# endernewton/tf-faster-rcnn

Hardware: AMD Instinct MI355X
Metric: images/sec (600×1000) ResNet-101 Faster R-CNN at 1/2/4/8 MI355X (higher is better)
Workload: dtype f32 (operands, accumulators, results; GEMMs with Cin, Cout % 128 == 0 form each f32 product from two-piece fp16 operands with an exact power-of-two scale per 128-k block on the fp16 matrix pipe -- 3 MFMAs / product, dropped terms <= 3 * 2^-22, measured error vs float64 below the f32-MFMA kernel's; o

## Files before the change

### include/frcnn_hip.h

```cpp
#ifndef FRCNN_HIP_H_
#define FRCNN_HIP_H_
#include <stddef.h>
#include <stdint.h>

#ifdef __cplusplus
extern "C" {
#endif

#define FRCNN_OK 0
#define FRCNN_E_ARG (-1)
#define FRCNN_E_WS (-2)
#define FRCNN_E_UNSUPPORTED (-3)
#define FRCNN_E_HIP(e) (-(1000 + (int)(e)))

#define FRCNN_NMS_RULE_CPU 0
#define FRCNN_NMS_RULE_GPU 1

#define FRCNN_ACT_NONE 0
#define FRCNN_ACT_RELU 1
#define FRCNN_ACT_RELU6 2

#define FRCNN_ABI_VERSION 6
int frcnn_abi_version(void);
const char* frcnn_build_info(void);
// ... 61 lines not shown
                      int* out_count_d, int max_out, void* ws, size_t ws_bytes, void* stream);
size_t frcnn_detect_post_batched_workspace_bytes(int B, int R, int C);
int frcnn_detect_post_batched(const float* cls_prob_d, const float* bbox_pred_d, const float* rois_d, const int* num_rois_d,
                              int B, int R, int C, double im_scale, int im_h, int im_w, double nms_thresh, int rule,
                              float score_thresh, int max_per_image, float* out_dets_d, int* out_count_d, int max_out,
                              long long out_stride, void* ws, size_t ws_bytes, void* stream);

int frcnn_im_detect_boxes(const float* rois_d, const float* bbox_pred_d, int R, int C, double im_scale,
                          int im_h, int im_w, float* boxes_d, void* stream);

int frcnn_bbox_transform_inv(const float* boxes_d, const float* deltas_d, int N, int k, float* out_d, void* stream);
int frcnn_clip_boxes(float* boxes_d, int N, int k, float im_h, float im_w, void* stream);
int frcnn_bbox_transform(const float* ex_rois_d, const float* gt_rois_d, int N, float* targets_d, void* stream);

int frcnn_bbox_overlaps(const double* boxes_d, int n, const double* query_d, int k, double* out_d, void* stream);

size_t frcnn_coco_match_workspace_bytes(int n_groups, long long n_det, long long n_gt, long long n_pairs);
int frcnn_coco_match(const double* det_xywh_d, const long long* det_off_d, const double* gt_xywh_d, const double* gt_area_d,
                     const unsigned char* gt_crowd_d, const long long* gt_off_d, int n_groups, const double* iou_thrs_d, int T,
                     const double* area_rng_d, int A, unsigned char* det_matched_d, unsigned char* det_ignored_d,
                     unsigned char* gt_ignored_d, double* iou_out_d, void* ws, size_t ws_bytes, void* stream);

int frcnn_conv2d_nhwc(const float* x_d, int N, int H, int W, int Cin, const float* w_d, const float* bias_d,
                      const float* residual_d, int RH, int RW, int res_stride, float* y_d, int OH, int OW,
                      int Cout, int KH, int KW, int stride, int pad_top, int pad_left, int act, int fold_w,
                      void* stream);
size_t frcnn_conv2d_workspace_bytes(int N, int OH, int OW, int Cout, int KH, int KW, int Cin, int fold_w);
int frcnn_conv2d_nhwc_ws(const float* x_d, int N, int H, int W, int Cin, const float* w_d, const float* bias_d,
                         const float* residual_d, int RH, int RW, int res_stride, float* y_d, int OH, int OW, int Cout, int KH,
                         int KW, int stride, int pad_top, int pad_left, int act, int fold_w, void* ws, size_t ws_bytes,
                         void* stream);

int frcnn_set_tuning(int key, int value);
unsigned int frcnn_crc32c(const void* data, size_t n, unsigned int crc);

long long frcnn_snappy_uncompress(const unsigned char* src, size_t n, unsigned char* dst, size_t cap);

int frcnn_prep_image_shape(int h, int w, int target_size, int max_size, double* im_scale, int* out_h, int* out_w);
int frcnn_prep_image(const void* src_d, int src_is_float, int h, int w, const double* pixel_means, double im_scale, float* out_d,
                     int OH, int OW, int out_c, void* stream);
int frcnn_prep_image_batched(const void* src_d, int src_is_float, int B, int h, int w, const double* pixel_means, double im_scale,
                             float* out_d, int OH, int OW, int out_c, void* stream);
int frcnn_prep_train_image(const void* src_d, int src_is_float, int h, int w, int flipped, const double* pixel_means, double im_scale,
                           float* out_d, int OH, int OW, int out_c, const unsigned short* boxes_d, const int* classes_d, int G,
                           float* gt_d, void* stream);

int frcnn_jpeg_info(const unsigned char* data, size_t n, int* out8);
size_t frcnn_jpeg_coef_bytes(int width, int height, int ncomp, int hs, int vs);
int frcnn_jpeg_entropy_decode(const unsigned char* data, size_t n, void* coef_h, size_t coef_bytes);
int frcnn_jpeg_pixels_host(const void* coef_h, int width, int height, int ncomp, int hs, int vs, unsigned char* bgr_h);
size_t frcnn_jpeg_workspace_bytes(int width, int height, int ncomp, int hs, int vs);
int frcnn_jpeg_pixels(const void* coef_d, int width, int height, int ncomp, int hs, int vs, unsigned char* bgr_d, void* ws,
                      size_t ws_bytes, void* stream);

int frcnn_gemm_batched_nt(const float* x_d, const float* w_d, float* y_d, int G, int M, int N, int K, void* stream);
size_t frcnn_gemm_x3_pack_bytes(int G, int N, int K);
int frcnn_gemm_x3_pack(const float* w_d, int G, int N, int K, void* planes_d, void* stream);
int frcnn_gemm_x3(const float* x_d, const void* planes_d, const float* bias_d, const float* res_d, float* y_d, int G, int M, int N,
                  int K, int act, int cfg, int terms, void* stream);
size_t frcnn_h2_planes_bytes(long long rows, int K);
int frcnn_h2_pack_w(const float* w_d, int G, int N, int K, void* planes_d, float* w_inv_d, void* stream);
int frcnn_h2_split(const float* x_d, long long M, int K, void* planes_d, float* inv_d, void* stream);
int frcnn_gemm_h2(const void* x_planes_d, const float* x_inv_d, const void* w_planes_d, const float* w_inv_d, const float* bias_d,
                  const float* res_d, const void* res_planes_d, const float* res_inv_d, float* y_d, void* y_planes_d, float* y_inv_d,
                  int G, int M, int N, int K, int act, int cfg, void* stream);
size_t frcnn_gemm_h2_mean_workspace_bytes(int G, int M, int N);
int frcnn_gemm_h2_mean(const void* x_planes_d, const float* x_inv_d, const void* w_planes_d, const float* w_inv_d, const float* bias_d,
                       const float* res_d, const void* res_planes_d, const float* res_inv_d, int G, int M, int N, int K, int act, int rows,
                       float* mean_out_d, void* ws, size_t ws_bytes, int cfg, void* stream);
int frcnn_winograd_filter_transform(const float* w_hwio, int Cin, int Cout, const float* scale, int m, float* u_out);
int frcnn_winograd_filter_transform_device(const float* w_packed_d, int Cout, int Cin, int m, int transpose_flip, float* u_d,
                                           void* stream);
int frcnn_winograd_input_transform(const float* x_d, int N, int H, int W, int C, int m, float* v_d, void* stream);
int frcnn_winograd_output_transform(const float* m_d, int N, int H, int W, int C, int m, const float* bias_d, int act, float* y_d,
                                    void* stream);
int frcnn_winograd7_filter_transform(const float* w_hwio, int Cin, int Cout, const float* scale, float* u_out);
int frcnn_winograd7_filter_transform_device(const float* w_packed_d, int Cout, int Cin, int transpose_flip, float* u_d, void* stream);
int frcnn_winograd7_input_transform(const float* x_d, int R, int C, float* v_d, void* stream);
int frcnn_winograd7_output_transform(const float* m_d, int R, int C, const float* bias_d, int act, float* y_d, void* stream);
int frcnn_winograd_input_transform_h2(const float* x_d, int N, int H, int W, int C, int m, void* v_planes_d, float* v_inv_d, void* stream);
int frcnn_winograd_output_transform_h2(const float* m_d, int N, int H, int W, int C, int m, const float* bias_d, int act, float* y_d,
                                       void* y_planes_d, float* y_inv_d, void* stream);
int frcnn_winograd7_input_transform_h2(const float* x_d, int R, int C, void* v_planes_d, float* v_inv_d, void* stream);
int frcnn_winograd7_output_transform_h2(const float* m_d, int R, int C, const float* bias_d, int act, float* y_d, void* y_planes_d,
                                        float* y_inv_d, void* stream);
int frcnn_pack_filter_hwio(const float* w_hwio, int KH, int KW, int Cin, int Cout, const float* scale, float* out);
int frcnn_maxpool_nhwc(const float* x_d, int N, int H, int W, int C, int k, int stride, int pad_top,
                       int pad_left, float* y_d, int OH, int OW, void* stream);
int frcnn_dwconv3x3_nhwc(const float* x_d, int N, int H, int W, int C, const float* w_d, const float* bias_d,
                         float* y_d, int OH, int OW, int stride, int pad_top, int pad_left, int act, void* stream);
int frcnn_dwconv3x3_nhwc_h2(const float* x_d, int N, int H, int W, int C, const float* w_d, const float* bias_d, float* y_d,
                            void* y_planes_d, float* y_inv_d, int OH, int OW, int stride, int pad_top, int pad_left, int act, void* stream);
int frcnn_spatial_mean(const float* x_d, int N, int HW, int C, float* y_d, void* stream);
int frcnn_softmax_rows(const float* x_d, int R, int C, int ld, float* y_d, void* stream);
int frcnn_rpn_softmax(const float* score_d, int HW, int A, int ld, float* prob_d, void* stream);
int frcnn_copy_cols(const float* src_d, int R, int ld_src, int col0, int cols, float* dst_d, int ld_dst, void* stream);

size_t frcnn_anchor_target_workspace_bytes(int H, int W, int A, int max_gt);
int frcnn_anchor_target_layer(const float* gt_boxes_d, int G, float im_h, float im_w, int H, int W, int A,
                              int feat_stride, const double* base_d, int rpn_batchsize, double fg_fraction,
                              double pos_overlap, double neg_overlap, long long seed, const double* opts, float* labels_d,
                              float* bbox_targets_d, float* inside_w_d, float* outside_w_d, void* ws,
                              size_t ws_bytes, void* stream);
int frcnn_anchor_target_layer_inject(const float* gt_boxes_d, int G, float im_h, float im_w, int H, int W, int A, int feat_stride,
                                     const double* base_d, int rpn_batchsize, double fg_fraction, double pos_overlap,
                                     double neg_overlap, const int* disable_d, int n_disable, const double* opts, float* labels_d,
                                     float* bbox_targets_d, float* inside_w_d, float* outside_w_d, void* ws, size_t ws_bytes,
                                     void* stream);
int frcnn_proposal_target_layer(const float* rpn_rois_d, const float* rpn_scores_d, int N, const float* gt_boxes_d,
                                int G, int num_classes, int batch_size, double fg_fraction, double fg_thresh,
                                double bg_thresh_hi, double bg_thresh_lo, const double* means4, const double* stds4,
                                long long seed, const double* opts, float* rois_d, float* roi_scores_d, float* labels_d,
                                float* bbox_targets_d, float* inside_w_d, float* outside_w_d, int* counts_d,
                                void* stream);
int frcnn_proposal_target_layer_dn(const float* rpn_rois_d, const float* rpn_scores_d, int max_rois, const int* num_rois_d,
                                   const float* gt_boxes_d, int G, int num_classes, int batch_size, double fg_fraction,
                                   double fg_thresh, double bg_thresh_hi, double bg_thresh_lo, const double* means4,
                                   const double* stds4, long long seed, const double* opts, float* rois_d, float* roi_scores_d,
                                   float* labels_d, float* bbox_targets_d, float* inside_w_d, float* outside_w_d, int* counts_d,
                                   void* stream);
int frcnn_proposal_target_layer_inject(const float* rpn_rois_d, const float* rpn_scores_d, int N, const float* gt_boxes_d, int G,
                                       int num_classes, int batch_size, const int* keep_inds_d, int n_fg, const double* means4,
                                       const double* stds4, const double* opts, float* rois_d, float* roi_scores_d, float* labels_d,
                                       float* bbox_targets_d, float* inside_w_d, float* outside_w_d, void* stream);
size_t frcnn_loss_workspace_bytes(long long elements);
int frcnn_softmax_ce_loss(const float* logits_d, const float* labels_d, int R, int C, int rpn_A, int rpn_H, int rpn_W,
                          float* loss_d, float* dlogits_d, void* ws, size_t ws_bytes, void* stream);
int frcnn_smooth_l1_loss(const float* pred_d, const float* targets_d, const float* inside_w_d, const float* outside_w_d,
                         long long n, float sigma, float mean_divisor, float* loss_d, float* dpred_d, void* ws,
                         size_t ws_bytes, void* stream);

int frcnn_transpose_pad(const float* in_d, int M, int C, float* out_d, int Mp, void* stream);
int frcnn_im2col_t(const float* x_d, int N, int H, int W, int Cin, int OH, int OW, int KH, int KW, int stride,
                   int pad_top, int pad_left, float* out_d, int Mp, void* stream);
int frcnn_flip_transpose_filter(const float* w_d, int Cout, int KH, int KW, int Cin, float* out_d, void* stream);
int frcnn_conv2d_dgrad_strided(const float* dy_d, int N, int OH, int OW, int Cout, const float* w_d, int KH, int KW,
                               int Cin, int stride, int pad_top, int pad_left, float* dx_d, int H, int W,
                               int accumulate, void* stream);
int frcnn_conv2d_wgrad_supported(int Cin, int Cout);
size_t frcnn_conv2d_wgrad_workspace_bytes(int N, int OH, int OW, int Cin, int Cout, int KH, int KW);
int frcnn_conv2d_wgrad(const float* dy_d, const float* x_d, int N, int H, int W, int Cin, int OH, int OW, int Cout, int KH, int KW,
                       int stride, int pad_top, int pad_left, float* dw_d, void* ws, size_t ws_bytes, void* stream);
void frcnn_conv2d_wgrad_set_plan(int tile, int min_workgroups);
size_t frcnn_conv2d_wgrad_h2_workspace_bytes(int N, int OH, int OW, int Cin, int Cout, int KH, int KW);
int frcnn_conv2d_wgrad_h2(const float* dy_d, const float* x_d, int N, int H, int W, int Cin, int OH, int OW, int Cout, int KH, int KW,
                          int stride, int pad_top, int pad_left, float* dw_d, void* ws, size_t ws_bytes, void* stream);
void frcnn_conv2d_wgrad_h2_set_plan(int tile, int min_workgroups);
int frcnn_relu_bwd(float* grad_d, const float* y_d, long long n, void* stream);
int frcnn_conv2d_nhwc_masked_ws(const float* x_d, int N, int H, int W, int Cin, const float* w_d, const float* bias_d,
                                const float* residual_d, int RH, int RW, int res_stride, float* y_d, int OH, int OW,
                                int Cout, int KH, int KW, int stride, int pad_top, int pad_left, int act, const float* mask_d,
                                void* ws, size_t ws_bytes, void* stream);
int frcnn_gemm_h2_masked(const void* x_planes_d, const float* x_inv_d, const void* w_planes_d, const float* w_inv_d, const float* bias_d,
                         const float* res_d, const float* mask_d, float* y_d, void* y_planes_d, float* y_inv_d, int G, int M, int N, int K,
                         int act, int cfg, void* stream);
int frcnn_winograd_output_transform_masked(const float* m_d, int N, int H, int W, int C, int m, const float* mask_d, float* y_d,
                                           void* y_planes_d, float* y_inv_d, void* stream);
int frcnn_winograd7_output_transform_masked(const float* m_d, int R, int C, const float* mask_d, float* y_d, void* y_planes_d,
                                            float* y_inv_d, void* stream);
int frcnn_relu6_bwd(float* grad_d, const float* y_d, long long n, void* stream);
int frcnn_maxpool_bwd(const float* x_d, int N, int H, int W, int C, int k, int stride, const float* y_d, const float* dy_d,
                      int OH, int OW, float* dx_d, void* stream);
int frcnn_dropout(const float* x_d, long long n, unsigned long long seed, float keep_prob, float* y_d, void* stream);
int frcnn_dwconv3x3_dgrad(const float* g_d, int N, int OH, int OW, int C, const float* w_d, float* dx_d, int H, int W, int stride,
                          int pad_top, int pad_left, int accumulate, void* stream);
size_t frcnn_dwconv3x3_wgrad_workspace_bytes(int N, int OH, int OW, int C);
// ... 30 lines not shown
```

### scratch/wino_bench.py

```python
import os, sys
ROOT = os.path.dirname(os.path.dirname(os.path.abspath(__file__)))
sys.path[:0] = [os.path.join(ROOT, "tf-faster-rcnn_amd")]
import numpy as np, torch
import frcnn_hip
from frcnn_hip import ops
dev = torch.device("cuda:0")
ths = [int(a) for a in (sys.argv[1] if (len(sys.argv) > 1 and "=" not in sys.argv[1]) else "256,100000000").split(",")]
shapes = {
    "block3 conv2 x8": (8, 38, 63, 256, 4),
    "block3 conv2 x1": (1, 38, 63, 256, 4),
    "rpn 3x3 x8": (8, 38, 63, 1024, 4),
    "block2 conv2 x8 (F2)": (8, 75, 125, 128, 2),
    "tail conv2 7x7 x8": (2400, 7, 7, 512, 7),
}
single = [a for a in sys.argv[1:] if a.startswith("single=")]
if single:
    nm, which, n = single[0][7:].split(":")
    N, H, W, C, m = shapes[nm]
    x = torch.randn(N, H, W, C, device=dev).clamp(min=0)
    G, T = ops.winograd_points(m), ops.winograd_tiles(N, H, W, m)
    mm = torch.randn(G, T, C, device=dev)
    bias = torch.randn(C, device=dev)
    v, yp = ops.H2.empty(G * T, C, dev), ops.H2.empty(N * H * W, C, dev)
    for _ in range(int(n)):
        if which == "input":
            ops.winograd_input_transform_h2(x, v, m)
        else:
            ops.winograd_output_transform_h2(mm, bias, 1, (N, H, W, C), m, yp)
    torch.cuda.synchronize()
    print("algorithmic bytes per launch: %d" % (4 * (N * H * W * C + G * T * C)))
    sys.exit(0)
print("%-24s %-10s %-6s %9s %9s %8s  %s" % ("shape", "transform", "rows<", "med_us", "min_us", "GB/s", "bits vs first"))
for name, (N, H, W, C, m) in shapes.items():
    torch.manual_seed(1)
    x = torch.randn(N, H, W, C, device=dev).clamp(min=0)
    G, T = ops.winograd_points(m), ops.winograd_tiles(N, H, W, m)
    mm = torch.randn(G, T, C, device=dev)
    bias = torch.randn(C, device=dev)
    for which in ("input", "output"):
        ref = None
        for th in ths:
            frcnn_hip.lib().frcnn_set_tuning(9, th)
            v = ops.H2.empty(G * T, C, dev)
            yp = ops.H2.empty(N * H * W, C, dev)
            v.planes.zero_(); v.inv.zero_(); yp.planes.zero_(); yp.inv.zero_()

            def run():
                if which == "input":
                    ops.winograd_input_transform_h2(x, v, m)
                else:
                    ops.winograd_output_transform_h2(mm, bias, 1, (N, H, W, C), m, yp)
            run(); torch.cuda.synchronize()
            o = v if which == "input" else yp
            pv = o.planes.view(torch.int16).to(torch.int64).view(-1)
            dig = (int(pv.sum()), int((pv * (torch.arange(pv.numel(), device=dev) % 8191 + 1)).sum()), int(o.inv.view(torch.int32).to(torch.int64).sum()))
            del pv
            ref = dig if ref is None else ref
            ts = []
            for r in range(6):
                e0, e1 = torch.cuda.Event(enable_timing=True), torch.cuda.Event(enable_timing=True)
                e0.record()
                for _ in range(10): run()
                e1.record(); torch.cuda.synchronize()
                if r: ts.append(e0.elapsed_time(e1) * 100)
            nbytes = 4.0 * (N * H * W * C + G * T * C)
            print("%-24s %-10s %-6s %9.1f %9.1f %8.0f  %s" % (name, which, th if th < 10**8 else "all", float(np.median(ts)), min(ts), nbytes / np.median(ts) / 1e3,
                                                             "identical" if dig == ref else "DIFFERENT"), flush=True)
            if m != 4:
                break
frcnn_hip.lib().frcnn_set_tuning(9, 0)
```

### tf-faster-rcnn_amd/csrc/conv_igemm.hip

```cpp
#include "common.h"
#include "mfma_f32.h"
#include <mutex>
#include <type_traits>

__device__ float4 g_zero_page[4];

struct ConvParams {
  const float* x; const float* w; const float* bias; const float* res; float* y;
  const float* mask;
  int N, H, W, Cin, OH, OW, Cout, KH, KW, stride, pad_top, pad_left, act;
  int RH, RW, res_stride;
  int M, Ktot, nsteps;
  int mtiles, ntiles;
  int batch;
  long long gx, gw, gy;
  int reserved;
  int splits, kchunk;
  long long gz;
  int stagger, stagger_slots;
};

__device__ __forceinline__ size_t res_offset_strided(int m, int n, int Cout, int res_stride, int ohow, int OW, int RH, int RW) {
  const int img = m / ohow, rem = m % ohow, oh = rem / OW, ow = rem % OW;
  return ((size_t)(img * RH + oh * res_stride) * RW + ow * res_stride) * Cout + n;
// ... 448 lines not shown
    int next = tile;
    if (last) {
      next = __builtin_amdgcn_readfirstlane(tile + W8);
      set_tile(next < t_end ? next : tile);
      prefetch_res();
    }
    slab_body(cur);
    cur ^= 1;
    if (!last) { ++step; continue; }
    if (p.res) finish(std::true_type{}); else finish(std::false_type{});
    if (next >= t_end) break;
    zero_acc();
    step = 0; tile = next; c_bm0 = i_bm0; c_bn0 = i_bn0; c_g = i_g;
  }
  wait_vmcnt<0>();
}

template <int BM, int BN, int WM, int WN, bool ILV, bool RF, bool RESPF>
static int launch_stream(const ConvParams& c, hipStream_t st) {
  constexpr int NT = (BM / WM) * (BN / WN) * 64;
  constexpr size_t lds = sizeof(float) * 2 * (BM + BN) * 32;
  auto kern = k_gemm_stream<BM, BN, WM, WN, ILV, RF, RESPF>;
  static KernelOnce once;
  int slots = 0;
  HIP_TRY(kernel_once(once, (const void*)kern, NT, lds, &slots));
  const bool plain = c.KH == 1 && c.KW == 1 && c.stride == 1 && c.pad_top == 0 && c.pad_left == 0 && c.OH == c.H && c.OW == c.W;
  if (slots < 8 || !plain || c.mask || c.Cout % BN || c.splits != 1 || (c.res && c.res_stride != 1) || (long long)c.M * c.Cout >= (1ll << 31) ||
      (long long)c.M * c.Cin >= (1ll << 31) || (long long)c.Cout * c.Cin >= (1ll << 31))
    return FRCNN_E_UNSUPPORTED;
  GemmParams p;
  p.x = c.x; p.w = c.w; p.bias = c.bias; p.res = c.res; p.y = c.y;
  p.mtiles = cdiv(c.M, BM); p.M = c.M; p.N = c.Cout; p.K = c.Cin; p.nsteps = c.Cin / 32;
  p.ntiles = c.Cout / BN; p.batch = c.batch; p.act = c.act;
  p.gx = c.gx; p.gw = c.gw; p.gy = c.gy;
  const long long T = (long long)p.mtiles * p.ntiles * p.batch;
  if (T >= (1ll << 30)) return FRCNN_E_UNSUPPORTED;
  const int grid = (int)min((long long)(slots / 8) * 8, ((T + 7) / 8) * 8);
  hipLaunchKernelGGL(kern, dim3(grid), dim3(NT), lds, st, p);
  LAUNCH_CHECK();
  return FRCNN_OK;
}

enum : int {
  IGEMM_64x32_NS4 = 4,
  IGEMM_64x64_ILV = 15,
  IGEMM_128_RF = 20,
  IGEMM_128_8W_RF = 21,
  STREAM_64x64 = 100, STREAM_64x64_RESPF = 101,
  STREAM_128_RF = 102,
  STREAM_128_8W_RF = 104, STREAM_128_8W_RF_RESPF = 105,
  STREAM_128x64 = 106, STREAM_128x64_RESPF = 107,
  STREAM_64x128 = 108, STREAM_64x128_RESPF = 109,
  STREAM_128x64_4W_RESPF = 110, STREAM_64x128_4W_RESPF = 111,
  STREAM_32x64 = 112,
  STREAM_32x128 = 114,
};

static int launch_cfg(int id, const ConvParams& p, hipStream_t st) {
  switch (id) {
    case IGEMM_64x32_NS4: return launch_conv<64, 32, 32, 32, 4, false>(p, st);
    case IGEMM_64x64_ILV: return launch_conv<64, 64, 32, 32, 2, false, true>(p, st);
    case IGEMM_128_RF: return launch_conv<128, 128, 64, 64, 2, false, false, true>(p, st);
    case IGEMM_128_8W_RF: return launch_conv<128, 128, 32, 64, 2, false, false, true>(p, st);
    case STREAM_64x64: return launch_stream<64, 64, 32, 32, true, false, false>(p, st);
    case STREAM_64x64_RESPF: return launch_stream<64, 64, 32, 32, true, false, true>(p, st);
    case STREAM_128_RF: return launch_stream<128, 128, 64, 64, false, true, false>(p, st);
    case STREAM_128_8W_RF: return launch_stream<128, 128, 32, 64, false, true, false>(p, st);
    case STREAM_128_8W_RF_RESPF: return launch_stream<128, 128, 32, 64, false, true, true>(p, st);
    case STREAM_128x64: return launch_stream<128, 64, 32, 32, true, false, false>(p, st);
    case STREAM_128x64_RESPF: return launch_stream<128, 64, 32, 32, true, false, true>(p, st);
    case STREAM_64x128: return launch_stream<64, 128, 32, 32, true, false, false>(p, st);
    case STREAM_64x128_RESPF: return launch_stream<64, 128, 32, 32, true, false, true>(p, st);
    case STREAM_128x64_4W_RESPF: return launch_stream<128, 64, 64, 32, false, true, true>(p, st);
    case STREAM_64x128_4W_RESPF: return launch_stream<64, 128, 32, 64, false, true, true>(p, st);
    case STREAM_32x64: return launch_stream<32, 64, 32, 32, true, false, false>(p, st);
    case STREAM_32x128: return launch_stream<32, 128, 32, 32, true, false, false>(p, st);
    default: return FRCNN_E_ARG;
  }
}

static thread_local int g_force_cfg = -1, g_stagger = 0, g_stream = 1, g_split_target = 640;
static thread_local int g_plan_images = 0;
static constexpr int PLAN_IMAGES = 4;
extern thread_local int g_wino_rows_below;
extern "C" int frcnn_set_tuning(int key, int value) {
  if (key == 9) { g_wino_rows_below = value > 0 ? value : 256; return FRCNN_OK; }
  if (key == 0) { g_force_cfg = value; return FRCNN_OK; }
  if (key == 5) { g_stagger = value; return FRCNN_OK; }
  if (key == 6) { g_stream = value; return FRCNN_OK; }
  if (key == 7) { g_split_target = value > 0 ? value : 640; return FRCNN_OK; }
  if (key == 8) { g_plan_images = value > 0 ? value : 0; return FRCNN_OK; }
  return FRCNN_E_ARG;
}

static long long plan_rows(long long M) {
  return (g_plan_images > 0 && M % g_plan_images == 0) ? M / g_plan_images * PLAN_IMAGES : M;
}

static long long tiles_128(long long rows, int Cout, int groups) { return (rows + 127) / 128 * cdiv(Cout, 128) * groups; }

static int tile_cfg_64(int Cout) { return Cout > 32 ? IGEMM_64x64_ILV : IGEMM_64x32_NS4; }
static int tile_cfg(long long rows, int Cout, int nsteps, int groups) {
  if (Cout >= 96 && tiles_128(rows, Cout, groups) >= 384 && nsteps >= 8) return Cout >= 1024 ? IGEMM_128_8W_RF : IGEMM_128_RF;
  return tile_cfg_64(Cout);
}

static bool short_k_stream(long long rows, int Cout, int nsteps, int groups) {
  return g_stream && nsteps <= 8 && Cout % 128 == 0 && (rows + 63) / 64 * (Cout / 128) * groups >= 512;
}

static int plan_splits(int M, int Cout, int nsteps) {
  if (g_force_cfg >= 0) return 1;
  M = (int)min(plan_rows(M), (long long)0x7fffffff);
  if (tile_cfg(M, Cout, nsteps, 1) != tile_cfg_64(Cout)) return 1;
  const long long tiles = (long long)cdiv(M, 64) * cdiv(Cout, Cout > 32 ? 64 : 32);
  if (tiles >= 384 || nsteps < 16) return 1;
  int S = (int)min((long long)8, (g_split_target + tiles - 1) / tiles);
  S = min(S, nsteps / 8);
  if (S < 2) return 1;
  const int kchunk = cdiv(nsteps, S);
  return cdiv(nsteps, kchunk);
}

extern "C" size_t frcnn_conv2d_workspace_bytes(int N, int OH, int OW, int Cout, int KH, int KW, int Cin, int fold_w) {
  if (fold_w || N <= 0 || OH <= 0 || OW <= 0 || Cout <= 0 || KH <= 0 || KW <= 0 || Cin <= 0 || Cin % 32) return 0;
  const long long M = (long long)N * OH * OW;
  if (M >= (1ll << 29)) return 0;
  const int S = plan_splits((int)M, Cout, KH * KW * (Cin / 32));
  return S > 1 ? (size_t)S * (size_t)M * (size_t)Cout * sizeof(float) : 0;
}

__global__ void k_splitk_finish(const float* __restrict__ part, int S, int M, int Cout, const float* __restrict__ bias,
                                const float* res, int res_stride, int OH, int OW, int RH, int RW, int act, const float* __restrict__ mask,
                                float* y) {
  const long long total = (long long)M * Cout;
  const int ohow = OH * OW;
  for (long long i = (long long)blockIdx.x * blockDim.x + threadIdx.x; i < total; i += (long long)gridDim.x * blockDim.x) {
    float v = part[i];
    for (int s = 1; s < S; ++s) v += part[(size_t)s * total + i];
    const int m = (int)(i / Cout), n = (int)(i - (long long)m * Cout);
    if (bias) v += bias[n];
    if (res) {
      size_t ro;
      if (res_stride == 1) ro = (size_t)i;
      else ro = res_offset_strided(m, n, Cout, res_stride, ohow, OW, RH, RW);
      v += res[ro];
    }
    if (act == FRCNN_ACT_RELU) v = act_relu(v);
    else if (act == FRCNN_ACT_RELU6) v = act_relu6(v);
    if (mask) v = mask[i] > 0.f ? v : 0.f;
    y[i] = v;
  }
}

static ConvParams conv_params() {
  ConvParams p = {};
  p.KH = p.KW = p.stride = p.res_stride = p.batch = p.splits = 1;
  p.act = FRCNN_ACT_NONE;
  return p;
}

static int conv2d_impl(const float* x_d, int N, int H, int W, int Cin, const float* w_d, const float* bias_d,
                       const float* residual_d, int RH, int RW, int res_stride, float* y_d, int OH, int OW, int Cout, int KH, int KW,
                       int stride, int pad_top, int pad_left, int act, int fold_w, void* ws, size_t ws_bytes, const float* mask_d,
                       void* stream) {
  if (!x_d || !w_d || !y_d) return FRCNN_E_ARG;
  if (N <= 0 || H <= 0 || W <= 0 || Cin <= 0 || OH <= 0 || OW <= 0 || Cout <= 0 || KH <= 0 || KW <= 0 || stride <= 0)
    return FRCNN_E_ARG;
  if (act < 0 || act > 2) return FRCNN_E_ARG;
// ... 110 lines not shown
```

### tf-faster-rcnn_amd/csrc/detect_kernels.hip

```cpp
#include "common.h"

extern "C" int frcnn_generate_anchors(int base_size, const double* ratios, int n_ratios, const double* scales,
                                      int n_scales, double* out_base) {
  if (!ratios || !scales || !out_base || n_ratios <= 0 || n_scales <= 0 || base_size <= 0) return FRCNN_E_ARG;
  const double w = (double)base_size, h = (double)base_size;
  const double cx = 0.5 * (w - 1), cy = 0.5 * (h - 1);
  for (int r = 0; r < n_ratios; ++r) {
    const double ws = nearbyint(sqrt(w * h / ratios[r]));
    const double hs = nearbyint(ws * ratios[r]);
    const double x1 = cx - 0.5 * (ws - 1), y1 = cy - 0.5 * (hs - 1);
    const double x2 = cx + 0.5 * (ws - 1), y2 = cy + 0.5 * (hs - 1);
    const double aw = x2 - x1 + 1, ah = y2 - y1 + 1;
    const double acx = x1 + 0.5 * (aw - 1), acy = y1 + 0.5 * (ah - 1);
    for (int s = 0; s < n_scales; ++s) {
      const double sw = aw * scales[s], sh = ah * scales[s];
      double* o = out_base + 4 * ((size_t)r * n_scales + s);
      o[0] = acx - 0.5 * (sw - 1);
      o[1] = acy - 0.5 * (sh - 1);
      o[2] = acx + 0.5 * (sw - 1);
      o[3] = acy + 0.5 * (sh - 1);
    }
  }
  return FRCNN_OK;
}

__device__ __forceinline__ float4 anchor_at(const double* __restrict__ base, int n, int A, int W, int stride) {
  const int a = n % A, pix = n / A;
  const double sx = (double)((pix % W) * stride), sy = (double)((pix / W) * stride);
  const double* b = base + 4 * a;
  return make_float4((float)(b[0] + sx), (float)(b[1] + sy), (float)(b[2] + sx), (float)(b[3] + sy));
}

__global__ void k_anchors(const double* __restrict__ base, int A, int W, int stride, int N, float4* __restrict__ out) {
  const int n = blockIdx.x * blockDim.x + threadIdx.x;
  if (n < N) out[n] = anchor_at(base, n, A, W, stride);
}

extern "C" int frcnn_generate_anchors_pre(int height, int width, int feat_stride, const double* base_d, int A,
                                          float* anchors_d, void* stream) {
  if (!base_d || !anchors_d || height <= 0 || width <= 0 || A <= 0) return FRCNN_E_ARG;
  const int N = height * width * A;
  hipLaunchKernelGGL(k_anchors, dim3(cdiv(N, 256)), dim3(256), 0, (hipStream_t)stream, base_d, A, width,
                     feat_stride, N, (float4*)anchors_d);
  LAUNCH_CHECK();
  return FRCNN_OK;
}

#define NMS_RULE_CPU FRCNN_NMS_RULE_CPU
#define NMS_RULE_GPU FRCNN_NMS_RULE_GPU
#define NMS_RULE_TF 2

__global__ void k_decode_clip_key(const float* __restrict__ prob, const float4* __restrict__ deltas,
                                  const double* __restrict__ base, int A, int W, int stride, int N, float hi_x,
                                  float hi_y, float4* __restrict__ boxes, u64* __restrict__ keys, size_t img) {
  const int n = blockIdx.x * blockDim.x + threadIdx.x;
  if (n >= N) return;
  const int b = blockIdx.y;
  prob += (size_t)b * 2 * N;
  deltas += (size_t)b * N;
  const int a = n % A, pix = n / A;
  const float score = prob[(size_t)pix * 2 * A + A + a];
  float4 bx = decode_box(anchor_at(base, n, A, W, stride), deltas[n]);
  bx.x = rmax(rmin(bx.x, hi_x), 0.0f);
  bx.y = rmax(rmin(bx.y, hi_y), 0.0f);
  bx.z = rmax(rmin(bx.z, hi_x), 0.0f);
  bx.w = rmax(rmin(bx.w, hi_y), 0.0f);
  img_ptr(boxes, img, b)[n] = bx;
  img_ptr(keys, img, b)[n] = make_key(score, (u32)n);
}

__global__ void k_dets_key(const float* __restrict__ dets, int k, float4* __restrict__ boxes, u64* __restrict__ keys) {
  const int n = blockIdx.x * blockDim.x + threadIdx.x;
  if (n >= k) return;
  const float* d = dets + 5 * (size_t)n;
  boxes[n] = make_float4(d[0], d[1], d[2], d[3]);
  keys[n] = make_key(d[4], (u32)n);
}

__global__ void k_boxes_scores_key(const float4* __restrict__ in_boxes, const float* __restrict__ in_scores, int k,
                                   float4* __restrict__ boxes, u64* __restrict__ keys) {
  const int n = blockIdx.x * blockDim.x + threadIdx.x;
  if (n >= k) return;
  boxes[n] = in_boxes[n];
// ... 652 lines not shown
  if (!rpn_cls_prob_d || !rpn_bbox_pred_d || !base_d || !rois_d || !scores_d || !ws) return FRCNN_E_ARG;
  if (H <= 0 || W <= 0 || A <= 0 || rpn_top_n <= 0) return FRCNN_E_ARG;
  const int N = H * W * A;
  if (N < rpn_top_n) return FRCNN_E_UNSUPPORTED;
  hipStream_t st = (hipStream_t)stream;
  SortWs s = carve(ws, N, rpn_top_n);
  if (s.bytes > ws_bytes) return FRCNN_E_WS;
  int rc = launch_decode(s, rpn_cls_prob_d, rpn_bbox_pred_d, 1, im_h, im_w, W, A, feat_stride, base_d, N, st);
  if (rc) return rc;
  rc = launch_topk_sort(s, N, rpn_top_n, 1, st);
  if (rc) return rc;
  hipLaunchKernelGGL(k_top_rois, dim3(cdiv(rpn_top_n, 256)), dim3(256), 0, st, s.sboxes, s.sscores, rpn_top_n, rois_d,
                     scores_d);
  LAUNCH_CHECK();
  return FRCNN_OK;
}

extern "C" int frcnn_proposal_top_layer_inds(const float* rpn_cls_prob_d, const float* rpn_bbox_pred_d, float im_h, float im_w,
                                             int H, int W, int A, int feat_stride, const double* base_d, const int* top_inds_d,
                                             int n_inds, float* rois_d, float* scores_d, void* stream) {
  if (!rpn_cls_prob_d || !rpn_bbox_pred_d || !base_d || !rois_d || !scores_d || !top_inds_d) return FRCNN_E_ARG;
  if (H <= 0 || W <= 0 || A <= 0 || n_inds <= 0) return FRCNN_E_ARG;
  hipLaunchKernelGGL(k_decode_gather, dim3(cdiv(n_inds, 256)), dim3(256), 0, (hipStream_t)stream, rpn_cls_prob_d,
                     (const float4*)rpn_bbox_pred_d, base_d, A, W, feat_stride, H * W * A, im_w - 1.0f, im_h - 1.0f, top_inds_d, n_inds,
                     rois_d, scores_d);
  LAUNCH_CHECK();
  return FRCNN_OK;
}

extern "C" int frcnn_non_max_suppression(const float* boxes_d, const float* scores_d, int k, int max_output_size,
                                         float iou_threshold, int* selected_d, int* num_d, void* ws, size_t ws_bytes,
                                         void* stream) {
  if (!num_d || k < 0 || max_output_size < 0) return FRCNN_E_ARG;
  hipStream_t st = (hipStream_t)stream;
  if (k == 0 || max_output_size == 0) {
    HIP_TRY(hipMemsetAsync(num_d, 0, sizeof(int), st));
    return FRCNN_OK;
  }
  if (!boxes_d || !scores_d || !selected_d || !ws) return FRCNN_E_ARG;
  if (k > NMS_MAX_BOXES) return FRCNN_E_UNSUPPORTED;
  SortWs s = carve(ws, k, k);
  if (s.bytes > ws_bytes) return FRCNN_E_WS;
  hipLaunchKernelGGL(k_boxes_scores_key, dim3(cdiv(k, 256)), dim3(256), 0, st, (const float4*)boxes_d, scores_d, k, s.boxes,
                     s.keys);
  LAUNCH_CHECK();
  int rc = launch_topk_sort(s, k, k, 1, st);
  if (rc) return rc;
  rc = launch_mask(s, k, 1, iou_threshold, NMS_RULE_TF, st);
  if (rc) return rc;
  ReduceOut o = {s.sboxes, s.sscores, s.sidx, nullptr, nullptr, selected_d, num_d, 0};
  return launch_reduce(s, k, 1, min(max_output_size, k), o, st);
}

extern "C" int frcnn_proposal_layer_tf_batched(const float* rpn_cls_prob_d, const float* rpn_bbox_pred_d, int B, float im_h,
                                               float im_w, int H, int W, int A, int feat_stride, const double* base_d,
                                               int post_nms_topn, float nms_thresh, float* rois_d, float* scores_d, int* num_d,
                                               void* ws, size_t ws_bytes, void* stream) {
  if (!rpn_cls_prob_d || !rpn_bbox_pred_d || !base_d || !rois_d || !scores_d || !num_d || !ws) return FRCNN_E_ARG;
  if (B <= 0 || H <= 0 || W <= 0 || A <= 0 || post_nms_topn <= 0) return FRCNN_E_ARG;
  const long long NN = (long long)H * W * A;
  if (NN > NMS_MAX_BOXES) return FRCNN_E_UNSUPPORTED;
  const int N = (int)NN;
  hipStream_t st = (hipStream_t)stream;
  SortWs s = carve(ws, N, N);
  if (s.bytes * (size_t)B > ws_bytes) return FRCNN_E_WS;
  int rc = launch_decode(s, rpn_cls_prob_d, rpn_bbox_pred_d, B, im_h, im_w, W, A, feat_stride, base_d, N, st);
  if (rc) return rc;
  rc = launch_topk_sort(s, N, N, B, st);
  if (rc) return rc;
  rc = launch_mask(s, N, B, nms_thresh, NMS_RULE_TF, st);
  if (rc) return rc;
  ReduceOut o = {s.sboxes, s.sscores, s.sidx, rois_d, scores_d, nullptr, num_d, 1};
  return launch_reduce(s, N, B, post_nms_topn, o, st);
}

extern "C" int frcnn_proposal_layer_tf(const float* rpn_cls_prob_d, const float* rpn_bbox_pred_d, float im_h, float im_w,
                                       int H, int W, int A, int feat_stride, const double* base_d, int post_nms_topn,
                                       float nms_thresh, float* rois_d, float* scores_d, int* num_d, void* ws,
                                       size_t ws_bytes, void* stream) {
  return frcnn_proposal_layer_tf_batched(rpn_cls_prob_d, rpn_bbox_pred_d, 1, im_h, im_w, H, W, A, feat_stride, base_d, post_nms_topn,
                                         nms_thresh, rois_d, scores_d, num_d, ws, ws_bytes, stream);
}

__device__ __forceinline__ float4 lerp4(const float4 a, const float4 b, float t) {
  return make_float4(a.x + (b.x - a.x) * t, a.y + (b.y - a.y) * t, a.z + (b.z - a.z) * t, a.w + (b.w - a.w) * t);
}
__device__ __forceinline__ float4 max4(const float4 a, const float4 b) {
  return make_float4(fmaxf(a.x, b.x), fmaxf(a.y, b.y), fmaxf(a.z, b.z), fmaxf(a.w, b.w));
}

__device__ __forceinline__ float4 crop_sample(const float4* __restrict__ feat, int H, int W, int C4, int c4, float y1,
                                              float x1, float hs, float ws, int gy, int gx) {
  const float in_y = y1 * (float)(H - 1) + (float)gy * hs;
  const float in_x = x1 * (float)(W - 1) + (float)gx * ws;
  if (in_y < 0 || in_y > (float)(H - 1) || in_x < 0 || in_x > (float)(W - 1)) return make_float4(0, 0, 0, 0);
  const int top = (int)floorf(in_y), bot = (int)ceilf(in_y);
  const int left = (int)floorf(in_x), right = (int)ceilf(in_x);
  const float ly = in_y - (float)top, lx = in_x - (float)left;
  const float4 tl = feat[((size_t)top * W + left) * C4 + c4], tr = feat[((size_t)top * W + right) * C4 + c4];
  const float4 bl = feat[((size_t)bot * W + left) * C4 + c4], br = feat[((size_t)bot * W + right) * C4 + c4];
  return lerp4(lerp4(tl, tr, lx), lerp4(bl, br, lx), ly);
}

template <bool MAX2>
__global__ __launch_bounds__(256) void k_crop_and_resize(const float4* __restrict__ feat_all, int NIMG, int H, int W, int C4,
                                                         int nslab, const float* __restrict__ rois, float stride, int pool,
                                                         const float4* __restrict__ bias, int act, float4* __restrict__ out) {
  const int slab = blockIdx.x % nslab, rp = blockIdx.x / nslab;
  const int r = rp / pool, py = rp % pool;
  const int SC4 = C4 / nslab, c40 = slab * SC4;
  const float height = ((float)H - 1.0f) * stride, width = ((float)W - 1.0f) * stride;
  const float* roi = rois + 5 * (size_t)r;
  const int img = (int)roi[0];
  float4* orow = out + ((size_t)r * pool + py) * pool * C4;
  if (img < 0 || img >= NIMG) {
    for (int t = threadIdx.x; t < pool * SC4; t += 256) orow[(size_t)(t / SC4) * C4 + c40 + t % SC4] = make_float4(0, 0, 0, 0);
    return;
  }
  const float4* feat = feat_all + (size_t)img * H * W * C4;
  const float x1 = roi[1] / width, y1 = roi[2] / height, x2 = roi[3] / width, y2 = roi[4] / height;
  const int P = MAX2 ? 2 * pool : pool;
  const float hs = (y2 - y1) * (float)(H - 1) / (float)(P - 1);
  const float ws = (x2 - x1) * (float)(W - 1) / (float)(P - 1);
  for (int t = threadIdx.x; t < pool * SC4; t += 256) {
    const int px = t / SC4, c4 = c40 + t % SC4;
    float4 v;
    if (MAX2) {
      v = crop_sample(feat, H, W, C4, c4, y1, x1, hs, ws, 2 * py, 2 * px);
      v = max4(v, crop_sample(feat, H, W, C4, c4, y1, x1, hs, ws, 2 * py, 2 * px + 1));
      v = max4(v, crop_sample(feat, H, W, C4, c4, y1, x1, hs, ws, 2 * py + 1, 2 * px));
      v = max4(v, crop_sample(feat, H, W, C4, c4, y1, x1, hs, ws, 2 * py + 1, 2 * px + 1));
    } else {
      v = crop_sample(feat, H, W, C4, c4, y1, x1, hs, ws, py, px);
    }
    if (bias) {
      const float4 bv = bias[c4];
      v.x += bv.x; v.y += bv.y; v.z += bv.z; v.w += bv.w;
    }
    if (act == FRCNN_ACT_RELU) v = act_relu(v);
    orow[(size_t)px * C4 + c4] = v;
  }
}

template <bool MAX2, int ITEMS>
__global__ __launch_bounds__(256) void k_crop_and_resize_roi(const float4* __restrict__ feat_all, int NIMG, int H, int W, int C4,
                                                             int nslab, const float* __restrict__ rois, float stride, int pool,
                                                             const float4* __restrict__ bias, int act, float4* __restrict__ out) {
  const int slab = blockIdx.x % nslab, r = blockIdx.x / nslab;
  const int SC4 = C4 / nslab, c40 = slab * SC4;
  const float height = ((float)H - 1.0f) * stride, width = ((float)W - 1.0f) * stride;
  const float* roi = rois + 5 * (size_t)r;
  const int img = (int)roi[0];
  float4* obase = out + (size_t)r * pool * pool * C4;
  const int total = pool * pool * SC4;
  if (img < 0 || img >= NIMG) {
    for (int t = threadIdx.x; t < total; t += 256) obase[(size_t)(t / SC4) * C4 + c40 + t % SC4] = make_float4(0, 0, 0, 0);
    return;
  }
  const float4* feat = feat_all + (size_t)img * H * W * C4;
  const float x1 = roi[1] / width, y1 = roi[2] / height, x2 = roi[3] / width, y2 = roi[4] / height;
  const int P = MAX2 ? 2 * pool : pool;
  const float hs = (y2 - y1) * (float)(H - 1) / (float)(P - 1);
  const float ws = (x2 - x1) * (float)(W - 1) / (float)(P - 1);
  for (int t0 = threadIdx.x; t0 < total; t0 += 256 * ITEMS) {
    float4 v[ITEMS];
#pragma unroll
    for (int k = 0; k < ITEMS; ++k) {
      const int t = t0 + k * 256;
      if (t >= total) { v[k] = make_float4(0, 0, 0, 0); continue; }
      const int pix = t / SC4, c4 = c40 + t % SC4;
      const int py = pix / pool, px = pix - py * pool;
      if (MAX2) {
        v[k] = crop_sample(feat, H, W, C4, c4, y1, x1, hs, ws, 2 * py, 2 * px);
        v[k] = max4(v[k], crop_sample(feat, H, W, C4, c4, y1, x1, hs, ws, 2 * py, 2 * px + 1));
        v[k] = max4(v[k], crop_sample(feat, H, W, C4, c4, y1, x1, hs, ws, 2 * py + 1, 2 * px));
        v[k] = max4(v[k], crop_sample(feat, H, W, C4, c4, y1, x1, hs, ws, 2 * py + 1, 2 * px + 1));
      } else {
        v[k] = crop_sample(feat, H, W, C4, c4, y1, x1, hs, ws, py, px);
      }
    }
#pragma unroll
    for (int k = 0; k < ITEMS; ++k) {
      const int t = t0 + k * 256;
      if (t >= total) continue;
      const int pix = t / SC4, c4 = c40 + t % SC4;
      float4 o = v[k];
      if (bias) {
        const float4 bv = bias[c4];
        o.x += bv.x; o.y += bv.y; o.z += bv.z; o.w += bv.w;
      }
      if (act == FRCNN_ACT_RELU) o = act_relu(o);
      obase[(size_t)pix * C4 + c4] = o;
    }
  }
}

static thread_local int g_crop_slabs = -1;
static thread_local int g_crop_form = 0;

static int launch_crop(const float* feat_d, int NIMG, int H, int W, int C, const float* rois_d, int R, float feat_stride, int pool,
                       int fuse_max2x2, const float* bias_d, int act, float* out_d, void* stream) {
  if (R == 0) return FRCNN_OK;
  if (!feat_d || !rois_d || !out_d || NIMG <= 0 || H < 2 || W < 2 || C <= 0 || R < 0 || pool < 2) return FRCNN_E_ARG;
  if (C % 4) return FRCNN_E_UNSUPPORTED;
  hipStream_t st = (hipStream_t)stream;
  const int C4 = C / 4;
  int nslab = (C4 % 8 == 0 && C4 / 8 >= 16) ? 8 : 1;
  if (g_crop_form == 0 && nslab == 8 && C4 / 8 < 32) nslab = 4;
  if (g_crop_slabs > 0 && C4 % g_crop_slabs == 0) nslab = g_crop_slabs;
  const long long blocks = (long long)R * pool * nslab;
  if (blocks >= (1ll << 31)) return FRCNN_E_UNSUPPORTED;
  if (g_crop_form == 0) {
    const unsigned grid = (unsigned)((long long)R * nslab);
    if (fuse_max2x2)
      hipLaunchKernelGGL((k_crop_and_resize_roi<true, 2>), dim3(grid), dim3(256), 0, st, (const float4*)feat_d, NIMG, H, W, C4, nslab, rois_d,
                         feat_stride, pool, (const float4*)bias_d, act, (float4*)out_d);
    else
      hipLaunchKernelGGL((k_crop_and_resize_roi<false, 4>), dim3(grid), dim3(256), 0, st, (const float4*)feat_d, NIMG, H, W, C4, nslab, rois_d,
                         feat_stride, pool, (const float4*)bias_d, act, (float4*)out_d);
    LAUNCH_CHECK();
    return FRCNN_OK;
  }
  if (fuse_max2x2)
    hipLaunchKernelGGL(k_crop_and_resize<true>, dim3((unsigned)blocks), dim3(256), 0, st, (const float4*)feat_d, NIMG, H, W, C4, nslab,
                       rois_d, feat_stride, pool, (const float4*)bias_d, act, (float4*)out_d);
  else
    hipLaunchKernelGGL(k_crop_and_resize<false>, dim3((unsigned)blocks), dim3(256), 0, st, (const float4*)feat_d, NIMG, H, W, C4, nslab,
                       rois_d, feat_stride, pool, (const float4*)bias_d, act, (float4*)out_d);
  LAUNCH_CHECK();
  return FRCNN_OK;
}

extern "C" int frcnn_detect_set_tuning(int key, int value) {
  if (key == 4) { g_crop_slabs = value; return FRCNN_OK; }
  if (key == 5) { g_crop_form = value; return FRCNN_OK; }
  return FRCNN_E_ARG;
}

extern "C" int frcnn_crop_and_resize(const float* feat_d, int H, int W, int C, const float* rois_d, int R,
                                     float feat_stride, int pool, int fuse_max2x2, float* out_d, void* stream) {
  return launch_crop(feat_d, 1, H, W, C, rois_d, R, feat_stride, pool, fuse_max2x2, nullptr, FRCNN_ACT_NONE, out_d, stream);
}

extern "C" int frcnn_crop_and_resize_batched(const float* feat_d, int N, int H, int W, int C, const float* rois_d, int R,
                                             float feat_stride, int pool, int fuse_max2x2, float* out_d, void* stream) {
  return launch_crop(feat_d, N, H, W, C, rois_d, R, feat_stride, pool, fuse_max2x2, nullptr, FRCNN_ACT_NONE, out_d, stream);
}

extern "C" int frcnn_crop_and_resize_bias_act(const float* feat_d, int N, int H, int W, int C, const float* rois_d, int R,
                                              float feat_stride, int pool, const float* bias_d, int act, float* out_d,
                                              void* stream) {
  if (act != FRCNN_ACT_NONE && act != FRCNN_ACT_RELU) return FRCNN_E_ARG;
  return launch_crop(feat_d, N, H, W, C, rois_d, R, feat_stride, pool, 0, bias_d, act, out_d, stream);
}

__global__ void k_bbox_transform_inv(const float4* __restrict__ boxes, const float4* __restrict__ deltas, int N, int k,
                                     float4* __restrict__ out) {
  const long long t = (long long)blockIdx.x * blockDim.x + threadIdx.x;
  if (t >= (long long)N * k) return;
  out[t] = decode_box(boxes[t / k], deltas[t]);
}
__global__ void k_clip_boxes(float4* __restrict__ boxes, long long n, float hi_x, float hi_y) {
  const long long t = (long long)blockIdx.x * blockDim.x + threadIdx.x;
  if (t >= n) return;
  float4 b = boxes[t];
  b.x = rmax(rmin(b.x, hi_x), 0.0f); b.y = rmax(rmin(b.y, hi_y), 0.0f);
  b.z = rmax(rmin(b.z, hi_x), 0.0f); b.w = rmax(rmin(b.w, hi_y), 0.0f);
  boxes[t] = b;
}
__global__ void k_bbox_transform(const float4* __restrict__ ex, const float4* __restrict__ gt, int N, float4* __restrict__ out) {
  const int t = blockIdx.x * blockDim.x + threadIdx.x;
  if (t >= N) return;
  const float4 e = ex[t], g = gt[t];
  const float ew = (e.z - e.x) + 1.0f, eh = (e.w - e.y) + 1.0f;
  const float ecx = e.x + 0.5f * ew, ecy = e.y + 0.5f * eh;
// ... 315 lines not shown
```

### tf-faster-rcnn_amd/csrc/gemm_h2.hip

```cpp
#include "h2_common.h"
#include <mutex>
#include <type_traits>

typedef float f32x16 __attribute__((ext_vector_type(16)));
typedef _Float16 h8 __attribute__((ext_vector_type(8)));

#define LDS_AS __attribute__((address_space(3)))

struct GemmH2Params {
  const unsigned short* x; const float* x_inv; const unsigned short* w; const float* w_inv;
  const float* bias; const float* res; const unsigned short* resp; const float* resp_inv; float* y; unsigned short* yp; float* y_inv;
  int M, N, K, batch, act, nsteps, mtiles, ntiles;
  long long Mtot;
  int wshare;
  const float* mask;
  float* mean_part; int mean_rows;
};

__device__ __forceinline__ void h2_glds16(unsigned voff, const void* sbase, unsigned lds_base) {
  unsigned keep;
  asm volatile(
      "s_mov_b32 %0, m0\n\t"
      "s_mov_b32 m0, %3\n\t"
      "s_nop 0\n\t"
// ... 1028 lines not shown
  return FRCNN_OK;
}

template <int MASK>
static int h2_dispatch(const GemmH2Params& p, int cfg, hipStream_t st) {
  switch (cfg) {
    case 9: return launch_h2<128, 128, 64, 64, 2, 2, H2_SCALES_ONCE + MASK>(p, st);
    case 12: return launch_h2<64, 128, 32, 64, 2, 2, MASK>(p, st);
    case 21: return launch_h2<256, 128, 64, 64, 3, 2, H2_SCALES_ONCE + H2_PINGPONG + MASK>(p, st);
    case 30: return launch_h2<128, 128, 64, 64, 2, 2, H2_SCALES_ONCE + H2_LIGHT_BOUNDARY + MASK>(p, st);
    case 31: return launch_h2<128, 128, 64, 64, 2, 2, H2_SCALES_ONCE + H2_LIGHT_BOUNDARY + H2_STORE16 + MASK>(p, st);
    case 32: return launch_h2<128, 128, 64, 64, 2, 2, H2_SCALES_ONCE + H2_STORE16 + MASK>(p, st);
    case 33: return launch_h2<64, 128, 32, 64, 2, 2, H2_LIGHT_BOUNDARY + H2_STORE16 + MASK>(p, st);
    case 34: return launch_h2<256, 128, 64, 64, 3, 2, H2_SCALES_ONCE + H2_PINGPONG + H2_STORE16 + MASK>(p, st);
    case 40: return launch_h2<128, 128, 64, 64, 2, 2, H2_SCALES_ONCE + H2_LIGHT_BOUNDARY + H2_STORE16 + H2_DEFERRED + MASK>(p, st);
    case 41: return launch_h2<64, 128, 32, 64, 2, 2, H2_LIGHT_BOUNDARY + H2_STORE16 + H2_DEFERRED + MASK>(p, st);
  }
#ifdef FRCNN_ABLATION
  constexpr int CFG31 = H2_SCALES_ONCE + H2_LIGHT_BOUNDARY + H2_STORE16;
  if constexpr (MASK == 0) switch (cfg) {
    case 50: return launch_h2<128, 128, 64, 64, 2, 2, CFG31 + H2_NO_MFMA>(p, st);
    case 51: return launch_h2<128, 128, 64, 64, 2, 2, CFG31 + H2_NO_FRAG>(p, st);
    case 52: return launch_h2<128, 128, 64, 64, 2, 2, CFG31 + H2_NO_LOAD>(p, st);
    case 53: return launch_h2<128, 128, 64, 64, 2, 2, CFG31 + H2_NO_MFMA + H2_NO_FRAG>(p, st);
    case 54: return launch_h2<128, 128, 64, 64, 2, 2, CFG31 + H2_NO_FRAG + H2_NO_LOAD>(p, st);
    case 55: return launch_h2<128, 128, 64, 64, 2, 2, CFG31 + H2_NO_MFMA + H2_NO_FRAG + H2_NO_LOAD>(p, st);
  }
#endif
  return FRCNN_E_ARG;
}

static int run_h2(GemmH2Params& p, int cfg, hipStream_t st);

static GemmH2Params h2_params(const void* x_planes_d, const float* x_inv_d, const void* w_planes_d, const float* w_inv_d, const float* bias_d,
                              const float* res_d, const void* res_planes_d, const float* res_inv_d, float* y_d, void* y_planes_d, float* y_inv_d,
                              int G, int M, int N, int K, int act) {
  GemmH2Params p;
  p.x = (const unsigned short*)x_planes_d; p.x_inv = x_inv_d; p.w = (const unsigned short*)w_planes_d; p.w_inv = w_inv_d;
  p.bias = bias_d; p.res = res_d; p.resp = (const unsigned short*)res_planes_d; p.resp_inv = res_inv_d; p.y = y_d; p.yp = (unsigned short*)y_planes_d; p.y_inv = y_inv_d;
  p.M = M; p.N = N; p.K = K; p.batch = G; p.act = act; p.Mtot = (long long)G * M;
  p.nsteps = p.mtiles = p.ntiles = 0;
  p.mean_part = nullptr; p.mean_rows = 0; p.wshare = 0; p.mask = nullptr;
  return p;
}

extern "C" int frcnn_gemm_h2(const void* x_planes_d, const float* x_inv_d, const void* w_planes_d, const float* w_inv_d, const float* bias_d,
                             const float* res_d, const void* res_planes_d, const float* res_inv_d, float* y_d, void* y_planes_d, float* y_inv_d,
                             int G, int M, int N, int K, int act, int cfg, void* stream) {
  if (!x_planes_d || !x_inv_d || !w_planes_d || !w_inv_d || (!y_d && !y_planes_d) || (y_planes_d && !y_inv_d) || G <= 0 || M <= 0 || N <= 0 ||
      K <= 0 || act < 0 || act > 2 || (res_d && res_planes_d) || (res_planes_d && !res_inv_d))
    return FRCNN_E_ARG;
  const long long Mtot = (long long)G * M;
  if (K % H2_KB || N % 128 || 4ll * Mtot * K >= (1ll << 32) || 4ll * N * K >= (1ll << 32) ||
      (long long)M * N >= (1ll << 29))
    return FRCNN_E_UNSUPPORTED;
  GemmH2Params p = h2_params(x_planes_d, x_inv_d, w_planes_d, w_inv_d, bias_d, res_d, res_planes_d, res_inv_d, y_d, y_planes_d, y_inv_d, G, M, N, K, act);
  return run_h2(p, cfg, (hipStream_t)stream);
}

extern "C" int frcnn_gemm_h2_masked(const void* x_planes_d, const float* x_inv_d, const void* w_planes_d, const float* w_inv_d, const float* bias_d,
                                    const float* res_d, const float* mask_d, float* y_d, void* y_planes_d, float* y_inv_d, int G, int M, int N, int K,
                                    int act, int cfg, void* stream) {
  if (!x_planes_d || !x_inv_d || !w_planes_d || !w_inv_d || !mask_d || (!y_d && !y_planes_d) || (y_planes_d && !y_inv_d) || G <= 0 || M <= 0 ||
      N <= 0 || K <= 0 || act < 0 || act > 2)
    return FRCNN_E_ARG;
  const long long Mtot = (long long)G * M;
  if (K % H2_KB || N % 128 || 4ll * Mtot * K >= (1ll << 32) || 4ll * N * K >= (1ll << 32) || (long long)M * N >= (1ll << 29)) return FRCNN_E_UNSUPPORTED;
  GemmH2Params p = h2_params(x_planes_d, x_inv_d, w_planes_d, w_inv_d, bias_d, res_d, nullptr, nullptr, y_d, y_planes_d, y_inv_d, G, M, N, K, act);
  p.mask = mask_d;
  return run_h2(p, cfg, (hipStream_t)stream);
}

static int run_h2(GemmH2Params& p, int cfg, hipStream_t st) {
  const int G = p.batch, M = p.M, N = p.N, K = p.K;
  if (cfg < 0) {
    const long long mt256 = (M + 255) / 256;
#ifndef FRCNN_H2_PP_MIN_K
#define FRCNN_H2_PP_MIN_K 1024
#endif
    const int pp_min_k = ((cfg == -4 || cfg == -5 || cfg == -6) && !p.mean_part) ? 512 : FRCNN_H2_PP_MIN_K;
    const int pp_cfg = (cfg == -3 || cfg == -4 || (cfg == -6 && K < FRCNN_H2_PP_MIN_K)) ? 34 : 21;
    const bool pp = K >= pp_min_k && mt256 * 256 * 100 <= (long long)M * 104 && mt256 * (N / 128) * G >= 256;
    const bool tiny = (long long)((M + 127) / 128) * (N / 128) * G < 150;
    const bool de = cfg != -2 && cfg != -7 && !p.mean_part && !p.mask && ((p.resp && p.yp && !p.y) || cfg == -8);
    cfg = pp ? pp_cfg : tiny ? (cfg == -2 ? 12 : (de && cfg == -8) ? 41 : 33) : (cfg == -2 ? 9 : de ? 40 : 31);
  }
  if (p.mean_part && (cfg == 40 || cfg == 41)) cfg = cfg == 40 ? 31 : 33;
  return p.mask ? h2_dispatch<H2_MASKED>(p, cfg, st) : h2_dispatch<0>(p, cfg, st);
}

__global__ __launch_bounds__(256) void k_h2_mean_finish(const float* __restrict__ part, int G, int M, int N4, int rows, float4* __restrict__ out) {
  const long long t = (long long)blockIdx.x * blockDim.x + threadIdx.x;
  const int per = M / rows;
  if (t >= (long long)G * per * N4) return;
  const int n4 = (int)(t % N4);
  const long long gr = t / N4;
  const int g = (int)(gr / per), r = (int)(gr % per);
  const int nblk = (M + 31) >> 5;
  const int row0 = r * rows, row1 = row0 + rows - 1;
  float4 s = make_float4(0.f, 0.f, 0.f, 0.f);
  for (int b = row0 >> 5; b <= (row1 >> 5); ++b) {
    const int which = ((b << 5) / rows == r) ? 0 : 1;
    const float4 v = *(const float4*)(part + (((size_t)g * nblk + b) * 2 + which) * (size_t)N4 * 4 + (size_t)n4 * 4);
    s.x += v.x; s.y += v.y; s.z += v.z; s.w += v.w;
  }
  const float inv = 1.0f / (float)rows;
  out[t] = make_float4(s.x * inv, s.y * inv, s.z * inv, s.w * inv);
}

extern "C" size_t frcnn_gemm_h2_mean_workspace_bytes(int G, int M, int N) {
  if (G <= 0 || M <= 0 || N <= 0) return 256;
  return (size_t)G * (size_t)((M + 31) / 32) * 2 * (size_t)N * sizeof(float);
}

extern "C" int frcnn_gemm_h2_mean(const void* x_planes_d, const float* x_inv_d, const void* w_planes_d, const float* w_inv_d, const float* bias_d,
                                  const float* res_d, const void* res_planes_d, const float* res_inv_d, int G, int M, int N, int K, int act, int rows,
                                  float* mean_out_d, void* ws, size_t ws_bytes, int cfg, void* stream) {
  if (!x_planes_d || !x_inv_d || !w_planes_d || !w_inv_d || !mean_out_d || !ws || G <= 0 || M <= 0 || N <= 0 || K <= 0 || act < 0 || act > 2 ||
      rows <= 0 || (res_d && res_planes_d) || (res_planes_d && !res_inv_d))
    return FRCNN_E_ARG;
  const long long Mtot = (long long)G * M;
  if (K % H2_KB || N % 128 || M % rows || rows < 32 || 4ll * Mtot * K >= (1ll << 32) || 4ll * N * K >= (1ll << 32) || (long long)M * N >= (1ll << 29))
    return FRCNN_E_UNSUPPORTED;
  if (frcnn_gemm_h2_mean_workspace_bytes(G, M, N) > ws_bytes) return FRCNN_E_WS;
  GemmH2Params p = h2_params(x_planes_d, x_inv_d, w_planes_d, w_inv_d, bias_d, res_d, res_planes_d, res_inv_d, nullptr, nullptr, nullptr, G, M, N, K, act);
  p.mean_part = (float*)ws; p.mean_rows = rows; p.wshare = 1;
  hipStream_t st = (hipStream_t)stream;
  const int rc = run_h2(p, cfg, st);
  if (rc) return rc;
  const long long tot = (long long)G * (M / rows) * (N / 4);
  hipLaunchKernelGGL(k_h2_mean_finish, dim3((unsigned)((tot + 255) / 256)), dim3(256), 0, st, (const float*)ws, G, M, N / 4, rows, (float4*)mean_out_d);
  LAUNCH_CHECK();
  return FRCNN_OK;
}
```

### tf-faster-rcnn_amd/csrc/winograd.hip

```cpp
#include "h2_common.h"


extern "C" int frcnn_winograd_filter_transform(const float* w_hwio, int Cin, int Cout, const float* scale, int m, float* u_out) {
  if (!w_hwio || !u_out || Cin <= 0 || Cout <= 0) return FRCNN_E_ARG;
  if (m != 2 && m != 4) return FRCNN_E_UNSUPPORTED;
  static const double G2[4][3] = {{1, 0, 0}, {0.5, 0.5, 0.5}, {0.5, -0.5, 0.5}, {0, 0, 1}};
  static const double G4[6][3] = {{1.0 / 4, 0, 0},           {-1.0 / 6, -1.0 / 6, -1.0 / 6}, {-1.0 / 6, 1.0 / 6, -1.0 / 6},
                                  {1.0 / 24, 1.0 / 12, 1.0 / 6}, {1.0 / 24, -1.0 / 12, 1.0 / 6}, {0, 0, 1}};
  const int a = m + 2;
  const double(*G)[3] = m == 2 ? G2 : G4;
  for (int c = 0; c < Cin; ++c)
    for (int o = 0; o < Cout; ++o) {
      double g[3][3], t[6][3];
      const double sc = scale ? (double)scale[o] : 1.0;
      for (int i = 0; i < 3; ++i)
        for (int j = 0; j < 3; ++j) g[i][j] = (double)w_hwio[((size_t)(i * 3 + j) * Cin + c) * Cout + o] * sc;
      for (int i = 0; i < a; ++i)
        for (int j = 0; j < 3; ++j) t[i][j] = G[i][0] * g[0][j] + G[i][1] * g[1][j] + G[i][2] * g[2][j];
      for (int i = 0; i < a; ++i)
        for (int j = 0; j < a; ++j) {
          const double u = t[i][0] * G[j][0] + t[i][1] * G[j][1] + t[i][2] * G[j][2];
          u_out[((size_t)(i * a + j) * Cout + o) * Cin + c] = (float)u;
        }
    }
// ... 196 lines not shown
    if (oh >= H) continue;
    float4 o[4];
    WINO4_AT(s[a][0], s[a][1], s[a][2], s[a][3], s[a][4], s[a][5], o[0], o[1], o[2], o[3]);
    const size_t row = (size_t)(img * H + oh) * W;
    size_t r[4];
    unsigned valid = 0;
#pragma unroll
    for (int b = 0; b < 4; ++b) {
      const int ow = 4 * tx + b;
      r[b] = row + ow;
      valid |= (ow < W ? 1u : 0u) << b;
      float4 v = f4add(o[b], bv);
      if (act == FRCNN_ACT_RELU) v = act_relu(v);
      if (MASK && ow < W) {
        const float4 k = mask[r[b] * C4 + c4];
        v.x = k.x > 0.f ? v.x : 0.f; v.y = k.y > 0.f ? v.y : 0.f; v.z = k.z > 0.f ? v.z : 0.f; v.w = k.w > 0.f ? v.w : 0.f;
      }
      o[b] = v;
    }
    y.template putn<4>(r, o, valid, c4, C4);
  }
}

template <int A, bool H2, bool MASK>
__device__ __forceinline__ void wino4_output_row(const float4* __restrict__ in, size_t plane, int H, int W, int C4, int img, int ty, int tx, int c4,
                                                 const float4* __restrict__ bias, int act, const float4* __restrict__ mask,
                                                 const WinoSink<H2>& y) {
  const int oh = 4 * ty + A;
  if (oh >= H) return;
  float4 sa[6];
#pragma unroll
  for (int j = 0; j < 6; ++j) {
    const float4 z = make_float4(0.f, 0.f, 0.f, 0.f);
    const float4 m0 = A == 0 ? in[(size_t)(0 * 6 + j) * plane] : z, m1 = in[(size_t)(1 * 6 + j) * plane], m2 = in[(size_t)(2 * 6 + j) * plane];
    const float4 m3 = in[(size_t)(3 * 6 + j) * plane], m4 = in[(size_t)(4 * 6 + j) * plane], m5 = A == 3 ? in[(size_t)(5 * 6 + j) * plane] : z;
    float4 sv[4];
    WINO4_AT(m0, m1, m2, m3, m4, m5, sv[0], sv[1], sv[2], sv[3]);
    sa[j] = sv[A];
  }
  const float4 bv = bias ? bias[c4] : make_float4(0.f, 0.f, 0.f, 0.f);
  float4 o[4];
  WINO4_AT(sa[0], sa[1], sa[2], sa[3], sa[4], sa[5], o[0], o[1], o[2], o[3]);
  const size_t row = (size_t)(img * H + oh) * W;
  size_t r[4];
  unsigned valid = 0;
#pragma unroll
  for (int b = 0; b < 4; ++b) {
    const int ow = 4 * tx + b;
    r[b] = row + ow;
    valid |= (ow < W ? 1u : 0u) << b;
    float4 v = f4add(o[b], bv);
    if (act == FRCNN_ACT_RELU) v = act_relu(v);
    if (MASK && ow < W) {
      const float4 k = mask[r[b] * C4 + c4];
      v.x = k.x > 0.f ? v.x : 0.f; v.y = k.y > 0.f ? v.y : 0.f; v.z = k.z > 0.f ? v.z : 0.f; v.w = k.w > 0.f ? v.w : 0.f;
    }
    o[b] = v;
  }
  y.template putn<4>(r, o, valid, c4, C4);
}

template <bool H2, bool MASK = false>
__global__ void __launch_bounds__(256) k_wino4_output_rows(const float4* __restrict__ Mx, int N, int H, int W, int C4, int TH, int TW,
                                                            const float4* __restrict__ bias, int act, const float4* __restrict__ mask,
                                                            const WinoSink<H2> y) {
  const long long id = (long long)blockIdx.x * blockDim.x + threadIdx.x;
  const long long T = (long long)N * TH * TW;
  if (id >= T * C4 * 4) return;
  const int c4 = (int)(id % C4);
  const int a = (int)((id / C4) & 3);
  const long long t = id / ((long long)C4 * 4);
  const int tx = (int)(t % TW), ty = (int)((t / TW) % TH), img = (int)(t / ((long long)TW * TH));
  const size_t plane = (size_t)T * C4;
  const float4* in = Mx + (size_t)t * C4 + c4;
  switch (a) {
    case 0: wino4_output_row<0, H2, MASK>(in, plane, H, W, C4, img, ty, tx, c4, bias, act, mask, y); break;
    case 1: wino4_output_row<1, H2, MASK>(in, plane, H, W, C4, img, ty, tx, c4, bias, act, mask, y); break;
    case 2: wino4_output_row<2, H2, MASK>(in, plane, H, W, C4, img, ty, tx, c4, bias, act, mask, y); break;
    default: wino4_output_row<3, H2, MASK>(in, plane, H, W, C4, img, ty, tx, c4, bias, act, mask, y); break;
  }
}

thread_local int g_wino_rows_below = 256;
#define WINO_ROWS_BELOW g_wino_rows_below

template <bool H2>
static int wino_input_launch(const float* x_d, int N, int H, int W, int C, int m, const WinoSink<H2>& sink, hipStream_t st) {
  const int TH = (H + m - 1) / m, TW = (W + m - 1) / m;
  const long long tot = (long long)N * TH * TW * (C / 4);
  if (m == 4 && (tot + 255) / 256 < WINO_ROWS_BELOW)
    hipLaunchKernelGGL(k_wino4_input_rows<H2>, dim3((unsigned)((tot * 6 + 255) / 256)), dim3(256), 0, st, (const float4*)x_d, N, H, W, C / 4, TH, TW,
                       sink);
  else if (m == 4)
    hipLaunchKernelGGL(k_wino4_input<H2>, dim3((unsigned)((tot + 255) / 256)), dim3(256), 0, st, (const float4*)x_d, N, H, W, C / 4, TH, TW, sink);
  else
    hipLaunchKernelGGL(k_wino_input<H2>, dim3((unsigned)((tot + 255) / 256)), dim3(256), 0, st, (const float4*)x_d, N, H, W, C / 4, TH, TW, sink);
  LAUNCH_CHECK();
  return FRCNN_OK;
}

extern "C" int frcnn_winograd_input_transform(const float* x_d, int N, int H, int W, int C, int m, float* v_d, void* stream) {
  if (!x_d || !v_d || N <= 0 || H <= 0 || W <= 0 || C <= 0) return FRCNN_E_ARG;
  if (C % 4 || (m != 2 && m != 4)) return FRCNN_E_UNSUPPORTED;
  const WinoSink<false> sink{(float4*)v_d, nullptr, nullptr, 0};
  return wino_input_launch<false>(x_d, N, H, W, C, m, sink, (hipStream_t)stream);
}

extern "C" int frcnn_winograd_input_transform_h2(const float* x_d, int N, int H, int W, int C, int m, void* v_planes_d, float* v_inv_d,
                                                 void* stream) {
  if (!x_d || !v_planes_d || !v_inv_d || N <= 0 || H <= 0 || W <= 0 || C <= 0) return FRCNN_E_ARG;
  if (C % H2_KB || (m != 2 && m != 4)) return FRCNN_E_UNSUPPORTED;
  const int TH = (H + m - 1) / m, TW = (W + m - 1) / m;
  const WinoSink<true> sink{nullptr, (unsigned short*)v_planes_d, v_inv_d, (size_t)(m + 2) * (m + 2) * N * TH * TW};
  return wino_input_launch<true>(x_d, N, H, W, C, m, sink, (hipStream_t)stream);
}

template <bool H2>
__global__ void k_wino_output(const float4* __restrict__ Mx, int N, int H, int W, int C4, int TH, int TW,
                              const float4* __restrict__ bias, int act, const WinoSink<H2> y) {
  const long long id = (long long)blockIdx.x * blockDim.x + threadIdx.x;
  const long long T = (long long)N * TH * TW;
  if (id >= T * C4) return;
  const int c4 = (int)(id % C4);
  const long long t = id / C4;
  const int tx = (int)(t % TW), ty = (int)((t / TW) % TH), img = (int)(t / ((long long)TW * TH));
  const size_t plane = (size_t)T * C4;
  const float4* in = Mx + (size_t)t * C4 + c4;
  float4 m[4][4];
#pragma unroll
  for (int i = 0; i < 4; ++i)
#pragma unroll
    for (int j = 0; j < 4; ++j) m[i][j] = in[(size_t)(i * 4 + j) * plane];
  float4 s[2][4];
#pragma unroll
  for (int j = 0; j < 4; ++j) {
    s[0][j] = f4add(f4add(m[0][j], m[1][j]), m[2][j]);
    s[1][j] = f4sub(f4sub(m[1][j], m[2][j]), m[3][j]);
  }
  const float4 bv = bias ? bias[c4] : make_float4(0.f, 0.f, 0.f, 0.f);
#pragma unroll
  for (int a = 0; a < 2; ++a) {
    const int oh = 2 * ty + a;
    if (oh >= H) continue;
    float4 o0 = f4add(f4add(f4add(s[a][0], s[a][1]), s[a][2]), bv);
    float4 o1 = f4add(f4sub(f4sub(s[a][1], s[a][2]), s[a][3]), bv);
    if (act == FRCNN_ACT_RELU) {
      o0 = act_relu(o0);
      o1 = act_relu(o1);
    }
    const size_t row = (size_t)(img * H + oh) * W;
    const float4 o[2] = {o0, o1};
    const size_t r[2] = {row + 2 * tx, row + 2 * tx + 1};
    y.template putn<2>(r, o, (2 * tx < W ? 1u : 0u) | (2 * tx + 1 < W ? 2u : 0u), c4, C4);
  }
}

template <bool H2>
static int wino_output_launch(const float* m_d, int N, int H, int W, int C, int m, const float* bias_d, int act, const WinoSink<H2>& sink,
                              hipStream_t st, const float* mask_d = nullptr) {
  const int TH = (H + m - 1) / m, TW = (W + m - 1) / m;
  const long long tot = (long long)N * TH * TW * (C / 4);
  const bool rows = (tot + 255) / 256 < WINO_ROWS_BELOW;
  if (m == 4 && mask_d && rows)
    hipLaunchKernelGGL((k_wino4_output_rows<H2, true>), dim3((unsigned)((tot * 4 + 255) / 256)), dim3(256), 0, st, (const float4*)m_d, N, H, W,
                       C / 4, TH, TW, (const float4*)bias_d, act, (const float4*)mask_d, sink);
  else if (m == 4 && mask_d)
    hipLaunchKernelGGL((k_wino4_output<H2, true>), dim3((unsigned)((tot + 255) / 256)), dim3(256), 0, st, (const float4*)m_d, N, H, W, C / 4, TH,
                       TW, (const float4*)bias_d, act, (const float4*)mask_d, sink);
  else if (mask_d)
    return FRCNN_E_UNSUPPORTED;
  else if (m == 4 && rows)
    hipLaunchKernelGGL((k_wino4_output_rows<H2, false>), dim3((unsigned)((tot * 4 + 255) / 256)), dim3(256), 0, st, (const float4*)m_d, N, H, W,
                       C / 4, TH, TW, (const float4*)bias_d, act, (const float4*)nullptr, sink);
  else if (m == 4)
    hipLaunchKernelGGL((k_wino4_output<H2, false>), dim3((unsigned)((tot + 255) / 256)), dim3(256), 0, st, (const float4*)m_d, N, H, W, C / 4, TH,
                       TW, (const float4*)bias_d, act, (const float4*)nullptr, sink);
  else
    hipLaunchKernelGGL(k_wino_output<H2>, dim3((unsigned)((tot + 255) / 256)), dim3(256), 0, st, (const float4*)m_d, N, H, W, C / 4, TH, TW,
                       (const float4*)bias_d, act, sink);
  LAUNCH_CHECK();
  return FRCNN_OK;
}

extern "C" int frcnn_winograd_output_transform(const float* m_d, int N, int H, int W, int C, int m, const float* bias_d, int act,
                                               float* y_d, void* stream) {
  if (!m_d || !y_d || N <= 0 || H <= 0 || W <= 0 || C <= 0) return FRCNN_E_ARG;
  if (C % 4 || (m != 2 && m != 4) || (act != FRCNN_ACT_NONE && act != FRCNN_ACT_RELU)) return FRCNN_E_UNSUPPORTED;
  const WinoSink<false> sink{(float4*)y_d, nullptr, nullptr, 0};
  return wino_output_launch<false>(m_d, N, H, W, C, m, bias_d, act, sink, (hipStream_t)stream);
}

extern "C" int frcnn_winograd_output_transform_h2(const float* m_d, int N, int H, int W, int C, int m, const float* bias_d, int act,
                                                  float* y_d, void* y_planes_d, float* y_inv_d, void* stream) {
  if (!m_d || !y_planes_d || !y_inv_d || N <= 0 || H <= 0 || W <= 0 || C <= 0) return FRCNN_E_ARG;
  if (C % H2_KB || (m != 2 && m != 4) || (act != FRCNN_ACT_NONE && act != FRCNN_ACT_RELU)) return FRCNN_E_UNSUPPORTED;
  const WinoSink<true> sink{(float4*)y_d, (unsigned short*)y_planes_d, y_inv_d, (size_t)N * H * W};
  return wino_output_launch<true>(m_d, N, H, W, C, m, bias_d, act, sink, (hipStream_t)stream);
}

extern "C" int frcnn_winograd_output_transform_masked(const float* m_d, int N, int H, int W, int C, int m, const float* mask_d, float* y_d,
                                                      void* y_planes_d, float* y_inv_d, void* stream) {
  if (!m_d || !mask_d || (!y_d && !y_planes_d) || (y_planes_d && !y_inv_d) || N <= 0 || H <= 0 || W <= 0 || C <= 0) return FRCNN_E_ARG;
  if (C % 4 || m != 4 || (y_planes_d && C % H2_KB)) return FRCNN_E_UNSUPPORTED;
  if (y_planes_d) {
    const WinoSink<true> sink{(float4*)y_d, (unsigned short*)y_planes_d, y_inv_d, (size_t)N * H * W};
    return wino_output_launch<true>(m_d, N, H, W, C, m, nullptr, FRCNN_ACT_NONE, sink, (hipStream_t)stream, mask_d);
  }
  const WinoSink<false> sink{(float4*)y_d, nullptr, nullptr, 0};
  return wino_output_launch<false>(m_d, N, H, W, C, m, nullptr, FRCNN_ACT_NONE, sink, (hipStream_t)stream, mask_d);
}

template <int M>
__global__ void k_wino_filter(const float* __restrict__ w, int O, int C, int transpose_flip, float* __restrict__ U) {
  const long long id = (long long)blockIdx.x * blockDim.x + threadIdx.x;
  if (id >= (long long)O * C) return;
  int o, c;
  if (transpose_flip) { o = (int)(id % O); c = (int)(id / O); }
  else { c = (int)(id % C); o = (int)(id / C); }
  float g[3][3];
#pragma unroll
  for (int i = 0; i < 3; ++i)
#pragma unroll
    for (int j = 0; j < 3; ++j) {
      const int kh = transpose_flip ? 2 - i : i, kw = transpose_flip ? 2 - j : j;
      g[i][j] = w[(((size_t)o * 3 + kh) * 3 + kw) * C + c];
    }
  constexpr int A = M + 2;
  float t[A][3];
#pragma unroll
  for (int j = 0; j < 3; ++j) {
    const float g0 = g[0][j], g1 = g[1][j], g2 = g[2][j];
    if (M == 2) {
      t[0][j] = g0;
      t[1][j] = 0.5f * (g0 + g1 + g2);
      t[2][j] = 0.5f * (g0 - g1 + g2);
      t[3][j] = g2;
    } else {
      t[0][j] = 0.25f * g0;
      t[1][j] = (-1.0f / 6.0f) * (g0 + g1 + g2);
      t[2][j] = (-1.0f / 6.0f) * (g0 - g1 + g2);
      t[3][j] = (1.0f / 24.0f) * g0 + (1.0f / 12.0f) * g1 + (1.0f / 6.0f) * g2;
      t[4][j] = (1.0f / 24.0f) * g0 - (1.0f / 12.0f) * g1 + (1.0f / 6.0f) * g2;
      t[A - 1][j] = g2;
    }
  }
// ... 33 lines not shown
```

### tf-faster-rcnn_amd/csrc/winograd7.hip

```cpp
#include "h2_common.h"

namespace w7 {
constexpr float BT[11][9] = {
    {4.f, 0.f, -5.f, 0.f, 1.f, 0.f, 0.f, 0.f, 0.f},  {0.f, -4.f, -4.f, 1.f, 1.f, 0.f, 0.f, 0.f, 0.f}, {0.f, 4.f, -4.f, -1.f, 1.f, 0.f, 0.f, 0.f, 0.f},
    {0.f, -2.f, -1.f, 2.f, 1.f, 0.f, 0.f, 0.f, 0.f}, {0.f, 2.f, -1.f, -2.f, 1.f, 0.f, 0.f, 0.f, 0.f}, {0.f, 4.f, 0.f, -5.f, 0.f, 1.f, 0.f, 0.f, 0.f},
    {0.f, 0.f, 0.f, 0.f, 2.f, -1.f, -2.f, 1.f, 0.f}, {0.f, 0.f, 0.f, 0.f, 0.f, -2.f, -1.f, 1.f, 0.f}, {0.f, 0.f, 0.f, 0.f, 0.f, 2.f, -3.f, 1.f, 0.f},
    {0.f, 0.f, 0.f, 0.f, 0.f, -1.f, 0.f, 1.f, 0.f},  {0.f, 0.f, 0.f, 0.f, 0.f, 2.f, -1.f, -2.f, 1.f}};
constexpr float AT[7][11] = {
    {1.f, 1.f, 1.f, 1.f, 1.f, 0.f, 0.f, 0.f, 0.f, 0.f, 0.f},  {0.f, 1.f, -1.f, 2.f, -2.f, 0.f, 0.f, 0.f, 0.f, 0.f, 0.f},
    {0.f, 1.f, 1.f, 4.f, 4.f, 0.f, 0.f, 0.f, 0.f, 0.f, 0.f},  {0.f, 1.f, -1.f, 8.f, -8.f, 1.f, 0.f, 0.f, 0.f, 0.f, 0.f},
    {0.f, 0.f, 0.f, 0.f, 0.f, 0.f, 1.f, 1.f, 1.f, 1.f, 0.f},  {0.f, 0.f, 0.f, 0.f, 0.f, 0.f, 0.f, 1.f, -1.f, 2.f, 0.f},
    {0.f, 0.f, 0.f, 0.f, 0.f, 0.f, 0.f, 1.f, 1.f, 4.f, 1.f}};
constexpr double G[11][3] = {{1.0 / 4, 0, 0},          {-1.0 / 6, -1.0 / 6, -1.0 / 6}, {-1.0 / 6, 1.0 / 6, -1.0 / 6}, {1.0 / 24, 1.0 / 12, 1.0 / 6},
                             {1.0 / 24, -1.0 / 12, 1.0 / 6}, {0, 0, 1},                {1.0 / 2, 0, 0},               {-1.0 / 2, -1.0 / 2, -1.0 / 2},
                             {-1.0 / 6, 1.0 / 6, -1.0 / 6},  {1.0 / 6, 1.0 / 3, 2.0 / 3}, {0, 0, 1}};
}

__device__ __forceinline__ float2 f2mad(float a, float2 x, float2 y) { return make_float2(a * x.x + y.x, a * x.y + y.y); }

__device__ __forceinline__ void acc_term(float2& acc, bool& first, float coef, const float2 x) {
  if (coef == 0.f) return;
  if (first) {
    acc = coef == 1.f ? x : (coef == -1.f ? make_float2(-x.x, -x.y) : make_float2(coef * x.x, coef * x.y));
    first = false;
  } else if (coef == 1.f) {
    acc = make_float2(acc.x + x.x, acc.y + x.y);
  } else if (coef == -1.f) {
    acc = make_float2(acc.x - x.x, acc.y - x.y);
  } else {
    acc = f2mad(coef, x, acc);
  }
}

template <bool H2>
struct Wino7Sink {
  float2* f; unsigned short* planes; float* inv; size_t rows;
  template <int NR>
  __device__ __forceinline__ void putn(const size_t* row, const float2* v, int c2, int C2) const {
    if (!H2 || f) {
#pragma unroll
      for (int n = 0; n < NR; ++n) f[row[n] * C2 + c2] = v[n];
    }
    if (H2) {
      size_t e[NR];
      float* slot[NR];
#pragma unroll
      for (int n = 0; n < NR; ++n) {
        e[n] = (row[n] * C2 + c2) * 2;
        slot[n] = inv + (size_t)(c2 >> 6) * rows + row[n];
      }
      h2_emit_rows64<NR>(v, e, slot, (1u << NR) - 1u, planes, rows * (size_t)C2 * 2, c2 & 63);
    }
  }
};

template <bool H2>
__global__ void __launch_bounds__(256) k_wino7_input(const float2* __restrict__ x, int R, int C2, const Wino7Sink<H2> V) {
  const long long id = (long long)blockIdx.x * blockDim.x + threadIdx.x;
  if (id >= (long long)R * C2) return;
  const int c2 = (int)(id % C2);
  const int r = (int)(id / C2);
  float2 d[7][7];
  const float2* src = x + (size_t)r * 49 * C2 + c2;
#pragma unroll
  for (int i = 0; i < 7; ++i)
#pragma unroll
    for (int j = 0; j < 7; ++j) d[i][j] = src[(size_t)(i * 7 + j) * C2];
#pragma unroll
  for (int xi = 0; xi < 11; ++xi) {
    float2 t[7];
#pragma unroll
    for (int j = 0; j < 7; ++j) {
      bool first = true;
      t[j] = make_float2(0.f, 0.f);
#pragma unroll
      for (int i = 0; i < 7; ++i) acc_term(t[j], first, w7::BT[xi][i + 1], d[i][j]);
    }
    float2 o[11];
    size_t rw[11];
#pragma unroll
    for (int nu = 0; nu < 11; ++nu) {
      bool first = true;
      float2 v = make_float2(0.f, 0.f);
#pragma unroll
      for (int j = 0; j < 7; ++j) acc_term(v, first, w7::BT[nu][j + 1], t[j]);
      o[nu] = v;
      rw[nu] = (size_t)(xi * 11 + nu) * R + r;
    }
    V.template putn<11>(rw, o, c2, C2);
  }
}

template <int XI0, int NXI, int I0, int NI, bool H2, bool MASK>
__device__ __forceinline__ void wino7_out_segment(const float2* __restrict__ in, size_t plane, float2 bv, int act, const Wino7Sink<H2>& y,
                                                  size_t row0, int c2, int C2, const float2* __restrict__ mask) {
  float2 m[NXI][11];
#pragma unroll
  for (int a = 0; a < NXI; ++a)
#pragma unroll
    for (int nu = 0; nu < 11; ++nu) m[a][nu] = in[(size_t)((XI0 + a) * 11 + nu) * plane];
#pragma unroll
  for (int i = 0; i < NI; ++i) {
    float2 s[11];
#pragma unroll
    for (int nu = 0; nu < 11; ++nu) {
      bool first = true;
      s[nu] = make_float2(0.f, 0.f);
#pragma unroll
      for (int a = 0; a < NXI; ++a) acc_term(s[nu], first, w7::AT[I0 + i][XI0 + a], m[a][nu]);
    }
    float2 o[7];
    size_t rw[7];
#pragma unroll
    for (int j = 0; j < 7; ++j) {
      bool first = true;
      float2 v = make_float2(0.f, 0.f);
#pragma unroll
      for (int nu = 0; nu < 11; ++nu) acc_term(v, first, w7::AT[j][nu], s[nu]);
      v = make_float2(v.x + bv.x, v.y + bv.y);
      if (act == FRCNN_ACT_RELU) v = act_relu(v);
      rw[j] = row0 + (I0 + i) * 7 + j;
      if (MASK) {
        const float2 k = mask[rw[j] * C2 + c2];
        v.x = k.x > 0.f ? v.x : 0.f; v.y = k.y > 0.f ? v.y : 0.f;
      }
      o[j] = v;
    }
    y.template putn<7>(rw, o, c2, C2);
  }
}

template <bool H2, bool MASK = false>
__global__ void __launch_bounds__(256) k_wino7_output(const float2* __restrict__ Mx, int R, int C2, const float2* __restrict__ bias, int act,
                                                       const float2* __restrict__ mask, const Wino7Sink<H2> y) {
  const long long id = (long long)blockIdx.x * blockDim.x + threadIdx.x;
  if (id >= (long long)R * C2) return;
  const int c2 = (int)(id % C2);
  const int r = (int)(id / C2);
  const size_t plane = (size_t)R * C2;
  const float2* in = Mx + (size_t)r * C2 + c2;
  const float2 bv = bias ? bias[c2] : make_float2(0.f, 0.f);
  wino7_out_segment<0, 6, 0, 4, H2, MASK>(in, plane, bv, act, y, (size_t)r * 49, c2, C2, mask);
  wino7_out_segment<6, 5, 4, 3, H2, MASK>(in, plane, bv, act, y, (size_t)r * 49, c2, C2, mask);
}

__global__ void k_wino7_filter(const float* __restrict__ w, int O, int C, int transpose_flip, float* __restrict__ U) {
  const long long id = (long long)blockIdx.x * blockDim.x + threadIdx.x;
  if (id >= (long long)O * C) return;
  int o, c;
  if (transpose_flip) { o = (int)(id % O); c = (int)(id / O); }
  else { c = (int)(id % C); o = (int)(id / C); }
  float g[3][3];
#pragma unroll
  for (int i = 0; i < 3; ++i)
#pragma unroll
    for (int j = 0; j < 3; ++j) {
      const int kh = transpose_flip ? 2 - i : i, kw = transpose_flip ? 2 - j : j;
      g[i][j] = w[(((size_t)o * 3 + kh) * 3 + kw) * C + c];
    }
  float t[11][3];
#pragma unroll
  for (int a = 0; a < 11; ++a)
#pragma unroll
    for (int j = 0; j < 3; ++j) t[a][j] = (float)w7::G[a][0] * g[0][j] + (float)w7::G[a][1] * g[1][j] + (float)w7::G[a][2] * g[2][j];
  const size_t plane = (size_t)O * C;
  float* out = U + (transpose_flip ? (size_t)c * O + o : (size_t)o * C + c);
#pragma unroll
  for (int a = 0; a < 11; ++a)
#pragma unroll
    for (int b = 0; b < 11; ++b)
      out[(size_t)(a * 11 + b) * plane] = t[a][0] * (float)w7::G[b][0] + t[a][1] * (float)w7::G[b][1] + t[a][2] * (float)w7::G[b][2];
}

extern "C" int frcnn_winograd7_filter_transform(const float* w_hwio, int Cin, int Cout, const float* scale, float* u_out) {
  if (!w_hwio || !u_out || Cin <= 0 || Cout <= 0) return FRCNN_E_ARG;
  for (int c = 0; c < Cin; ++c)
    for (int o = 0; o < Cout; ++o) {
      double g[3][3], t[11][3];
      const double sc = scale ? (double)scale[o] : 1.0;
      for (int i = 0; i < 3; ++i)
        for (int j = 0; j < 3; ++j) g[i][j] = (double)w_hwio[((size_t)(i * 3 + j) * Cin + c) * Cout + o] * sc;
      for (int a = 0; a < 11; ++a)
        for (int j = 0; j < 3; ++j) t[a][j] = w7::G[a][0] * g[0][j] + w7::G[a][1] * g[1][j] + w7::G[a][2] * g[2][j];
      for (int a = 0; a < 11; ++a)
        for (int b = 0; b < 11; ++b)
          u_out[((size_t)(a * 11 + b) * Cout + o) * Cin + c] = (float)(t[a][0] * w7::G[b][0] + t[a][1] * w7::G[b][1] + t[a][2] * w7::G[b][2]);
    }
  return FRCNN_OK;
}

extern "C" int frcnn_winograd7_filter_transform_device(const float* w_packed_d, int Cout, int Cin, int transpose_flip, float* u_d,
                                                       void* stream) {
  if (!w_packed_d || !u_d || Cout <= 0 || Cin <= 0) return FRCNN_E_ARG;
  const long long tot = (long long)Cout * Cin;
  hipLaunchKernelGGL(k_wino7_filter, dim3((unsigned)((tot + 255) / 256)), dim3(256), 0, (hipStream_t)stream, w_packed_d, Cout, Cin,
                     transpose_flip ? 1 : 0, u_d);
  LAUNCH_CHECK();
  return FRCNN_OK;
}

extern "C" int frcnn_winograd7_input_transform(const float* x_d, int R, int C, float* v_d, void* stream) {
  if (!x_d || !v_d || R <= 0 || C <= 0) return FRCNN_E_ARG;
  if (C % 2) return FRCNN_E_UNSUPPORTED;
  const long long tot = (long long)R * (C / 2);
  const Wino7Sink<false> sink{(float2*)v_d, nullptr, nullptr, 0};
  hipLaunchKernelGGL(k_wino7_input<false>, dim3((unsigned)((tot + 255) / 256)), dim3(256), 0, (hipStream_t)stream, (const float2*)x_d, R, C / 2, sink);
  LAUNCH_CHECK();
  return FRCNN_OK;
}

extern "C" int frcnn_winograd7_input_transform_h2(const float* x_d, int R, int C, void* v_planes_d, float* v_inv_d, void* stream) {
  if (!x_d || !v_planes_d || !v_inv_d || R <= 0 || C <= 0) return FRCNN_E_ARG;
  if (C % H2_KB) return FRCNN_E_UNSUPPORTED;
  const long long tot = (long long)R * (C / 2);
  const Wino7Sink<true> sink{nullptr, (unsigned short*)v_planes_d, v_inv_d, (size_t)121 * R};
  hipLaunchKernelGGL(k_wino7_input<true>, dim3((unsigned)((tot + 255) / 256)), dim3(256), 0, (hipStream_t)stream, (const float2*)x_d, R, C / 2, sink);
  LAUNCH_CHECK();
  return FRCNN_OK;
}

extern "C" int frcnn_winograd7_output_transform(const float* m_d, int R, int C, const float* bias_d, int act, float* y_d, void* stream) {
  if (!m_d || !y_d || R <= 0 || C <= 0) return FRCNN_E_ARG;
  if (C % 2 || (act != FRCNN_ACT_NONE && act != FRCNN_ACT_RELU)) return FRCNN_E_UNSUPPORTED;
  const long long tot = (long long)R * (C / 2);
  const Wino7Sink<false> sink{(float2*)y_d, nullptr, nullptr, 0};
  hipLaunchKernelGGL((k_wino7_output<false, false>), dim3((unsigned)((tot + 255) / 256)), dim3(256), 0, (hipStream_t)stream, (const float2*)m_d, R,
                     C / 2, (const float2*)bias_d, act, (const float2*)nullptr, sink);
  LAUNCH_CHECK();
  return FRCNN_OK;
}

extern "C" int frcnn_winograd7_output_transform_h2(const float* m_d, int R, int C, const float* bias_d, int act, float* y_d, void* y_planes_d,
                                                   float* y_inv_d, void* stream) {
  if (!m_d || !y_planes_d || !y_inv_d || R <= 0 || C <= 0) return FRCNN_E_ARG;
  if (C % H2_KB || (act != FRCNN_ACT_NONE && act != FRCNN_ACT_RELU)) return FRCNN_E_UNSUPPORTED;
  const long long tot = (long long)R * (C / 2);
  const Wino7Sink<true> sink{(float2*)y_d, (unsigned short*)y_planes_d, y_inv_d, (size_t)R * 49};
  hipLaunchKernelGGL((k_wino7_output<true, false>), dim3((unsigned)((tot + 255) / 256)), dim3(256), 0, (hipStream_t)stream, (const float2*)m_d, R,
                     C / 2, (const float2*)bias_d, act, (const float2*)nullptr, sink);
  LAUNCH_CHECK();
  return FRCNN_OK;
}

extern "C" int frcnn_winograd7_output_transform_masked(const float* m_d, int R, int C, const float* mask_d, float* y_d, void* y_planes_d,
                                                       float* y_inv_d, void* stream) {
  if (!m_d || !mask_d || (!y_d && !y_planes_d) || (y_planes_d && !y_inv_d) || R <= 0 || C <= 0) return FRCNN_E_ARG;
  if (C % 2 || (y_planes_d && C % H2_KB)) return FRCNN_E_UNSUPPORTED;
  const long long tot = (long long)R * (C / 2);
  if (y_planes_d) {
    const Wino7Sink<true> sink{(float2*)y_d, (unsigned short*)y_planes_d, y_inv_d, (size_t)R * 49};
    hipLaunchKernelGGL((k_wino7_output<true, true>), dim3((unsigned)((tot + 255) / 256)), dim3(256), 0, (hipStream_t)stream, (const float2*)m_d, R,
                       C / 2, (const float2*)nullptr, FRCNN_ACT_NONE, (const float2*)mask_d, sink);
  } else {
    const Wino7Sink<false> sink{(float2*)y_d, nullptr, nullptr, 0};
    hipLaunchKernelGGL((k_wino7_output<false, true>), dim3((unsigned)((tot + 255) / 256)), dim3(256), 0, (hipStream_t)stream, (const float2*)m_d, R,
                       C / 2, (const float2*)nullptr, FRCNN_ACT_NONE, (const float2*)mask_d, sink);
  }
  LAUNCH_CHECK();
  return FRCNN_OK;
}
```

### tf-faster-rcnn_amd/frcnn_hip/__init__.py

```python
import ctypes
import os
from ctypes import c_double, c_float, c_int, c_longlong, c_size_t, c_ulonglong, c_void_p

_PKG = os.path.dirname(os.path.abspath(__file__))
LIB_PATH = os.path.join(_PKG, "libfrcnn_hip.so")
_lib = None

ABI_VERSION = 6
ACT_NONE, ACT_RELU, ACT_RELU6 = 0, 1, 2
NMS_RULE_CPU, NMS_RULE_GPU = 0, 1

_P = c_void_p
SIGNATURES = {
    "frcnn_abi_version": (c_int, []),
    "frcnn_build_info": (ctypes.c_char_p, []),
    "_nms": (None, [_P, _P, _P, c_int, c_int, c_float, c_int]),
    "frcnn_nms_workspace_bytes": (c_size_t, [c_int]),
    "frcnn_nms": (c_int, [_P, c_int, c_double, c_int, _P, _P, _P, c_size_t, _P]),
    "frcnn_nms_sorted": (c_int, [_P, c_int, c_int, c_double, c_int, _P, _P, _P, c_size_t, _P]),
    "frcnn_nms_rule": (c_int, [_P, c_int, c_double, c_int, c_int, _P, _P, _P, c_size_t, _P]),
    "frcnn_nms_sorted_rule": (c_int, [_P, c_int, c_int, c_double, c_int, c_int, _P, _P, _P, c_size_t, _P]),
    "frcnn_generate_anchors": (c_int, [c_int, _P, c_int, _P, c_int, _P]),
    "frcnn_generate_anchors_pre": (c_int, [c_int, c_int, c_int, _P, c_int, _P, _P]),
    "frcnn_proposal_workspace_bytes": (c_size_t, [c_int, c_int, c_int, c_int]),
    "frcnn_proposal_layer": (c_int, [_P, _P, c_float, c_float, c_int, c_int, c_int, c_int, _P, c_int, c_int, c_double,
                                     _P, _P, _P, _P, c_size_t, _P]),
    "frcnn_proposal_batched_workspace_bytes": (c_size_t, [c_int, c_int, c_int, c_int, c_int]),
    "frcnn_proposal_layer_batched": (c_int, [_P, _P, c_int, c_float, c_float, c_int, c_int, c_int, c_int, _P, c_int, c_int, c_double,
                                             c_int, _P, _P, _P, _P, c_size_t, _P]),
    "frcnn_proposal_top_layer_inds": (c_int, [_P, _P, c_float, c_float, c_int, c_int, c_int, c_int, _P, _P, c_int, _P, _P, _P]),
    "frcnn_proposal_layer_tf_batched": (c_int, [_P, _P, c_int, c_float, c_float, c_int, c_int, c_int, c_int, _P, c_int, c_float, _P, _P,
                                                _P, _P, c_size_t, _P]),
    "frcnn_proposal_top_layer": (c_int, [_P, _P, c_float, c_float, c_int, c_int, c_int, c_int, _P, c_int, _P, _P, _P,
                                         c_size_t, _P]),
    "frcnn_non_max_suppression": (c_int, [_P, _P, c_int, c_int, c_float, _P, _P, _P, c_size_t, _P]),
    "frcnn_proposal_layer_tf": (c_int, [_P, _P, c_float, c_float, c_int, c_int, c_int, c_int, _P, c_int, c_float, _P, _P, _P,
                                        _P, c_size_t, _P]),
    "frcnn_crop_and_resize": (c_int, [_P, c_int, c_int, c_int, _P, c_int, c_float, c_int, c_int, _P, _P]),
    "frcnn_crop_and_resize_batched": (c_int, [_P, c_int, c_int, c_int, c_int, _P, c_int, c_float, c_int, c_int, _P, _P]),
    "frcnn_crop_and_resize_bias_act": (c_int, [_P, c_int, c_int, c_int, c_int, _P, c_int, c_float, c_int, _P, c_int, _P, _P]),
    "frcnn_detect_set_tuning": (c_int, [c_int, c_int]),
    "frcnn_detect_post_batched_workspace_bytes": (c_size_t, [c_int, c_int, c_int]),
    "frcnn_detect_post_batched": (c_int, [_P, _P, _P, _P, c_int, c_int, c_int, c_double, c_int, c_int, c_double, c_int, c_float, c_int,
                                          _P, _P, c_int, c_longlong, _P, c_size_t, _P]),
    "frcnn_detect_post_workspace_bytes": (c_size_t, [c_int, c_int]),
    "frcnn_detect_post": (c_int, [_P, _P, _P, _P, c_int, c_int, c_double, c_int, c_int, c_double, c_float, c_int, _P, _P,
                                  c_int, _P, c_size_t, _P]),
    "frcnn_im_detect_boxes": (c_int, [_P, _P, c_int, c_int, c_double, c_int, c_int, _P, _P]),
    "frcnn_bbox_overlaps": (c_int, [_P, c_int, _P, c_int, _P, _P]),
    "frcnn_coco_match_workspace_bytes": (c_size_t, [c_int, c_longlong, c_longlong, c_longlong]),
    "frcnn_coco_match": (c_int, [_P, _P, _P, _P, _P, _P, c_int, _P, c_int, _P, c_int, _P, _P, _P, _P, _P, c_size_t, _P]),
    "frcnn_bbox_transform_inv": (c_int, [_P, _P, c_int, c_int, _P, _P]),
    "frcnn_clip_boxes": (c_int, [_P, c_int, c_int, c_float, c_float, _P]),
    "frcnn_bbox_transform": (c_int, [_P, _P, c_int, _P, _P]),
    "frcnn_conv2d_nhwc": (c_int, [_P, c_int, c_int, c_int, c_int, _P, _P, _P, c_int, c_int, c_int, _P, c_int, c_int,
                                  c_int, c_int, c_int, c_int, c_int, c_int, c_int, c_int, _P]),
    "frcnn_conv2d_workspace_bytes": (c_size_t, [c_int, c_int, c_int, c_int, c_int, c_int, c_int, c_int]),
    "frcnn_conv2d_nhwc_ws": (c_int, [_P, c_int, c_int, c_int, c_int, _P, _P, _P, c_int, c_int, c_int, _P, c_int, c_int,
                                     c_int, c_int, c_int, c_int, c_int, c_int, c_int, c_int, _P, c_size_t, _P]),
    "frcnn_conv2d_nhwc_masked_ws": (c_int, [_P, c_int, c_int, c_int, c_int, _P, _P, _P, c_int, c_int, c_int, _P, c_int, c_int,
                                            c_int, c_int, c_int, c_int, c_int, c_int, c_int, _P, _P, c_size_t, _P]),
    "frcnn_gemm_h2_masked": (c_int, [_P, _P, _P, _P, _P, _P, _P, _P, _P, _P, c_int, c_int, c_int, c_int, c_int, c_int, _P]),
    "frcnn_winograd_output_transform_masked": (c_int, [_P, c_int, c_int, c_int, c_int, c_int, _P, _P, _P, _P, _P]),
    "frcnn_winograd7_output_transform_masked": (c_int, [_P, c_int, c_int, _P, _P, _P, _P, _P]),
    "frcnn_crc32c": (ctypes.c_uint32, [_P, c_size_t, ctypes.c_uint32]),
    "frcnn_snappy_uncompress": (c_longlong, [_P, c_size_t, _P, c_size_t]),
    "frcnn_prep_image_shape": (c_int, [c_int, c_int, c_int, c_int, _P, _P, _P]),
    "frcnn_prep_image": (c_int, [_P, c_int, c_int, c_int, _P, c_double, _P, c_int, c_int, c_int, _P]),
    "frcnn_prep_image_batched": (c_int, [_P, c_int, c_int, c_int, c_int, _P, c_double, _P, c_int, c_int, c_int, _P]),
    "frcnn_prep_train_image": (c_int, [_P, c_int, c_int, c_int, c_int, _P, c_double, _P, c_int, c_int, c_int, _P, _P, c_int, _P, _P]),
    "frcnn_jpeg_info": (c_int, [_P, c_size_t, _P]),
    "frcnn_jpeg_coef_bytes": (c_size_t, [c_int, c_int, c_int, c_int, c_int]),
    "frcnn_jpeg_entropy_decode": (c_int, [_P, c_size_t, _P, c_size_t]),
    "frcnn_jpeg_pixels_host": (c_int, [_P, c_int, c_int, c_int, c_int, c_int, _P]),
    "frcnn_jpeg_workspace_bytes": (c_size_t, [c_int, c_int, c_int, c_int, c_int]),
    "frcnn_jpeg_pixels": (c_int, [_P, c_int, c_int, c_int, c_int, c_int, _P, _P, c_size_t, _P]),
    "frcnn_gemm_batched_nt": (c_int, [_P, _P, _P, c_int, c_int, c_int, c_int, _P]),
    "frcnn_winograd_filter_transform": (c_int, [_P, c_int, c_int, _P, c_int, _P]),
    "frcnn_winograd_filter_transform_device": (c_int, [_P, c_int, c_int, c_int, c_int, _P, _P]),
    "frcnn_winograd_input_transform": (c_int, [_P, c_int, c_int, c_int, c_int, c_int, _P, _P]),
    "frcnn_winograd_output_transform": (c_int, [_P, c_int, c_int, c_int, c_int, c_int, _P, c_int, _P, _P]),
    "frcnn_winograd7_filter_transform": (c_int, [_P, c_int, c_int, _P, _P]),
    "frcnn_winograd7_filter_transform_device": (c_int, [_P, c_int, c_int, c_int, _P, _P]),
    "frcnn_winograd7_input_transform": (c_int, [_P, c_int, c_int, _P, _P]),
    "frcnn_winograd7_output_transform": (c_int, [_P, c_int, c_int, _P, c_int, _P, _P]),
    "frcnn_winograd_input_transform_h2": (c_int, [_P, c_int, c_int, c_int, c_int, c_int, _P, _P, _P]),
    "frcnn_winograd_output_transform_h2": (c_int, [_P, c_int, c_int, c_int, c_int, c_int, _P, c_int, _P, _P, _P, _P]),
    "frcnn_winograd7_input_transform_h2": (c_int, [_P, c_int, c_int, _P, _P, _P]),
    "frcnn_winograd7_output_transform_h2": (c_int, [_P, c_int, c_int, _P, c_int, _P, _P, _P, _P]),
    "frcnn_set_tuning": (c_int, [c_int, c_int]),
    "frcnn_pack_filter_hwio": (c_int, [_P, c_int, c_int, c_int, c_int, _P, _P]),
    "frcnn_maxpool_nhwc": (c_int, [_P, c_int, c_int, c_int, c_int, c_int, c_int, c_int, c_int, _P, c_int, c_int, _P]),
    "frcnn_dwconv3x3_nhwc": (c_int, [_P, c_int, c_int, c_int, c_int, _P, _P, _P, c_int, c_int, c_int, c_int, c_int, c_int, _P]),
    "frcnn_dwconv3x3_nhwc_h2": (c_int, [_P, c_int, c_int, c_int, c_int, _P, _P, _P, _P, _P, c_int, c_int, c_int, c_int, c_int, c_int, _P]),
    "frcnn_spatial_mean": (c_int, [_P, c_int, c_int, c_int, _P, _P]),
    "frcnn_softmax_rows": (c_int, [_P, c_int, c_int, c_int, _P, _P]),
    "frcnn_rpn_softmax": (c_int, [_P, c_int, c_int, c_int, _P, _P]),
    "frcnn_copy_cols": (c_int, [_P, c_int, c_int, c_int, c_int, _P, c_int, _P]),
    "frcnn_anchor_target_workspace_bytes": (c_size_t, [c_int, c_int, c_int, c_int]),
    "frcnn_anchor_target_layer": (c_int, [_P, c_int, c_float, c_float, c_int, c_int, c_int, c_int, _P, c_int, c_double, c_double,
                                          c_double, c_longlong, _P, _P, _P, _P, _P, _P, c_size_t, _P]),
    "frcnn_anchor_target_layer_inject": (c_int, [_P, c_int, c_float, c_float, c_int, c_int, c_int, c_int, _P, c_int, c_double, c_double,
                                                 c_double, _P, c_int, _P, _P, _P, _P, _P, _P, c_size_t, _P]),
    "frcnn_proposal_target_layer_inject": (c_int, [_P, _P, c_int, _P, c_int, c_int, c_int, _P, c_int, _P, _P, _P, _P, _P, _P, _P, _P, _P, _P]),
    "frcnn_proposal_target_layer": (c_int, [_P, _P, c_int, _P, c_int, c_int, c_int, c_double, c_double, c_double, c_double, _P, _P,
                                            c_longlong, _P, _P, _P, _P, _P, _P, _P, _P, _P]),
    "frcnn_proposal_target_layer_dn": (c_int, [_P, _P, c_int, _P, _P, c_int, c_int, c_int, c_double, c_double, c_double, c_double, _P, _P,
                                               c_longlong, _P, _P, _P, _P, _P, _P, _P, _P, _P]),
    "frcnn_loss_workspace_bytes": (c_size_t, [c_longlong]),
    "frcnn_softmax_ce_loss": (c_int, [_P, _P, c_int, c_int, c_int, c_int, c_int, _P, _P, _P, c_size_t, _P]),
    "frcnn_smooth_l1_loss": (c_int, [_P, _P, _P, _P, c_longlong, c_float, c_float, _P, _P, _P, c_size_t, _P]),
    "frcnn_transpose_pad": (c_int, [_P, c_int, c_int, _P, c_int, _P]),
    "frcnn_im2col_t": (c_int, [_P, c_int, c_int, c_int, c_int, c_int, c_int, c_int, c_int, c_int, c_int, c_int, _P, c_int, _P]),
    "frcnn_flip_transpose_filter": (c_int, [_P, c_int, c_int, c_int, c_int, _P, _P]),
    "frcnn_conv2d_dgrad_strided": (c_int, [_P, c_int, c_int, c_int, c_int, _P, c_int, c_int, c_int, c_int, c_int, c_int, _P, c_int,
                                           c_int, c_int, _P]),
    "frcnn_conv2d_wgrad_supported": (c_int, [c_int, c_int]),
    "frcnn_conv2d_wgrad_workspace_bytes": (c_size_t, [c_int, c_int, c_int, c_int, c_int, c_int, c_int]),
    "frcnn_conv2d_wgrad": (c_int, [_P, _P, c_int, c_int, c_int, c_int, c_int, c_int, c_int, c_int, c_int, c_int, c_int, c_int, _P, _P,
                                   c_size_t, _P]),
    "frcnn_conv2d_wgrad_set_plan": (None, [c_int, c_int]),
    "frcnn_conv2d_wgrad_h2_workspace_bytes": (c_size_t, [c_int, c_int, c_int, c_int, c_int, c_int, c_int]),
    "frcnn_conv2d_wgrad_h2": (c_int, [_P, _P, c_int, c_int, c_int, c_int, c_int, c_int, c_int, c_int, c_int, c_int, c_int, c_int, _P, _P,
                                      c_size_t, _P]),
    "frcnn_conv2d_wgrad_h2_set_plan": (None, [c_int, c_int]),
    "frcnn_relu_bwd": (c_int, [_P, _P, c_longlong, _P]),
    "frcnn_gemm_x3_pack_bytes": (c_size_t, [c_int, c_int, c_int]),
    "frcnn_gemm_x3_pack": (c_int, [_P, c_int, c_int, c_int, _P, _P]),
    "frcnn_gemm_x3": (c_int, [_P, _P, _P, _P, _P, c_int, c_int, c_int, c_int, c_int, c_int, c_int, _P]),
    "frcnn_h2_planes_bytes": (c_size_t, [c_longlong, c_int]),
    "frcnn_h2_pack_w": (c_int, [_P, c_int, c_int, c_int, _P, _P, _P]),
    "frcnn_h2_split": (c_int, [_P, c_longlong, c_int, _P, _P, _P]),
    "frcnn_gemm_h2": (c_int, [_P, _P, _P, _P, _P, _P, _P, _P, _P, _P, _P, c_int, c_int, c_int, c_int, c_int, c_int, _P]),
    "frcnn_gemm_h2_mean_workspace_bytes": (c_size_t, [c_int, c_int, c_int]),
    "frcnn_gemm_h2_mean": (c_int, [_P, _P, _P, _P, _P, _P, _P, _P, c_int, c_int, c_int, c_int, c_int, c_int, _P, _P, c_size_t, c_int, _P]),
    "frcnn_relu6_bwd": (c_int, [_P, _P, c_longlong, _P]),
    "frcnn_maxpool_bwd": (c_int, [_P, c_int, c_int, c_int, c_int, c_int, c_int, _P, _P, c_int, c_int, _P, _P]),
    "frcnn_dropout": (c_int, [_P, c_longlong, c_ulonglong, c_float, _P, _P]),
    "frcnn_dwconv3x3_dgrad": (c_int, [_P, c_int, c_int, c_int, c_int, _P, _P, c_int, c_int, c_int, c_int, c_int, c_int, _P]),
    "frcnn_dwconv3x3_wgrad_workspace_bytes": (c_size_t, [c_int, c_int, c_int, c_int]),
    "frcnn_dwconv3x3_wgrad": (c_int, [_P, _P, c_int, c_int, c_int, c_int, c_int, c_int, c_int, c_int, c_int, _P, _P, _P, c_size_t, _P]),
    "frcnn_dwconv3x3_refold": (c_int, [_P, _P, c_int, _P, _P]),
    "frcnn_add_strided": (c_int, [_P, c_int, c_int, c_int, c_int, _P, c_int, c_int, c_int, c_int, _P]),
    "frcnn_spatial_mean_bwd": (c_int, [_P, c_int, c_int, c_int, _P, _P]),
    "frcnn_colsum": (c_int, [_P, c_int, c_int, _P, _P]),
    "frcnn_crop_and_resize_bwd": (c_int, [_P, c_int, c_int, c_int, _P, c_int, c_float, c_int, _P, _P]),
    "frcnn_crop_and_resize_bwd_plan": (c_int, [_P, c_int, c_int, c_int, _P, c_int, c_float, c_int, _P, c_size_t, _P]),
    "frcnn_sgd_momentum": (c_int, [_P, _P, _P, _P, _P, c_longlong, c_int, c_float, c_float, c_float, c_float, _P]),
    "frcnn_sgd_desc_bytes": (c_size_t, []),
    "frcnn_sgd_momentum_multi": (c_int, [_P, c_int, c_float, c_float, c_float, _P]),
    "frcnn_sgd_momentum_range": (c_int, [_P, c_int, c_int, c_float, c_float, c_float, _P]),
    "frcnn_sumsq": (c_int, [_P, c_longlong, c_double, _P, c_int, _P, c_size_t, _P]),
    "frcnn_sumsq_multi": (c_int, [_P, _P, c_int, c_double, _P, c_int, _P, c_size_t, _P]),
    "frcnn_graph_begin": (c_int, [_P]),
    "frcnn_graph_end": (c_int, [_P, ctypes.POINTER(c_void_p)]),
    "frcnn_graph_launch": (c_int, [_P, _P]),
    "frcnn_graph_destroy": (c_int, [_P]),
}


class FrcnnHipError(RuntimeError):
    pass


def lib():
    global _lib
    if _lib is None:
        if not os.path.exists(LIB_PATH):
            raise ImportError("libfrcnn_hip.so not built: run `python -c 'import __graft_entry__ as g; g.build()'` "
                              "(or python tf-faster-rcnn_amd/frcnn_hip/build.py); there is no CPU fallback")
        L = ctypes.CDLL(LIB_PATH)
# ... 28 lines not shown
```

### tf-faster-rcnn_amd/frcnn_hip/ops.py

```python
import ctypes

import numpy as np
import torch

import frcnn_hip as _binding
from . import ACT_NONE, NMS_RULE_CPU, call, lib

_ws_cache = {}
ws_scope = "default"

_scope_stack = [(None, None, None)]


def active_store(owner, default=None):
    o, _, store = _scope_stack[-1]
    return store if store is not None and (owner is None or o is owner) else default


def scope_depth():
    return len(_scope_stack) - 1


class unscoped(object):

# ... 897 lines not shown
    __slots__ = ("planes", "inv", "rows", "K")

    def __init__(self, planes, inv, rows, K):
        self.planes, self.inv, self.rows, self.K = planes, inv, int(rows), int(K)

    @staticmethod
    def empty(rows, K, device):
        assert K % 128 == 0
        return H2(torch.empty(lib().frcnn_h2_planes_bytes(int(rows), int(K)), dtype=torch.uint8, device=device),
                  torch.empty((K // 128, rows), dtype=torch.float32, device=device), rows, K)

    def to_float(self):
        hl = self.planes.view(torch.float16).view(2, self.rows, self.K).float()
        inv = self.inv.t().repeat_interleave(128, dim=1)
        return (hl[0] + hl[1]) * inv


def h2_split(x, out=None):
    _chk(x)
    K = x.shape[-1]
    rows = x.numel() // K
    out = H2.empty(rows, K, x.device) if out is None else out
    assert out.rows == rows and out.K == K
    call("frcnn_h2_split", _ptr(x), rows, K, _ptr(out.planes), _ptr(out.inv), _stream())
    return out


def h2_pack_w(w, out=None):
    _chk(w)
    G, N, K = (w.shape[0], w.shape[1], w.shape[2]) if w.dim() == 3 else (1, w.shape[0], w[0].numel())
    if out is None:
        out = (torch.empty(lib().frcnn_h2_planes_bytes(G * N, K), dtype=torch.uint8, device=w.device),
               torch.empty((G, N), dtype=torch.float32, device=w.device))
    call("frcnn_h2_pack_w", _ptr(w), G, N, K, _ptr(out[0]), _ptr(out[1]), _stream())
    return out


def gemm_h2(x, wp, G, M, N, K, bias=None, residual=None, act=ACT_NONE, out=None, out_planes=None, want_f32=True, cfg=-1, mask=None):
    assert isinstance(x, H2) and x.rows == G * M and x.K == K
    if out is None and want_f32:
        out = _empty((G * M, N), dtype=torch.float32, device=x.planes.device)
    if out_planes is not None:
        assert out_planes.rows == G * M and out_planes.K == N
    rp = residual if isinstance(residual, H2) else None
    if rp is not None:
        assert rp.rows == G * M and rp.K == N
    if mask is not None:
        _chk(mask)
        assert rp is None and mask.numel() == G * M * N
        call("frcnn_gemm_h2_masked", _ptr(x.planes), _ptr(x.inv), _ptr(wp[0]), _ptr(wp[1]), _ptr(bias), _ptr(residual), _ptr(mask), _ptr(out),
             _ptr(None if out_planes is None else out_planes.planes), _ptr(None if out_planes is None else out_planes.inv),
             int(G), int(M), int(N), int(K), int(act), int(cfg), _stream())
        return out, out_planes
    call("frcnn_gemm_h2", _ptr(x.planes), _ptr(x.inv), _ptr(wp[0]), _ptr(wp[1]), _ptr(bias), _ptr(None if rp is not None else residual),
         _ptr(None if rp is None else rp.planes), _ptr(None if rp is None else rp.inv), _ptr(out),
         _ptr(None if out_planes is None else out_planes.planes), _ptr(None if out_planes is None else out_planes.inv),
         int(G), int(M), int(N), int(K), int(act), int(cfg), _stream())
    return out, out_planes


def gemm_h2_mean(x, wp, G, M, N, K, bias, residual, act, rows, out=None, cfg=-1):
    assert isinstance(x, H2) and x.rows == G * M and x.K == K and M % rows == 0
    if out is None:
        out = _empty((G * (M // rows), N), dtype=torch.float32, device=x.planes.device)
    rp = residual if isinstance(residual, H2) else None
    ws = workspace(lib().frcnn_gemm_h2_mean_workspace_bytes(int(G), int(M), int(N)), x.planes.device, "h2_mean")
    call("frcnn_gemm_h2_mean", _ptr(x.planes), _ptr(x.inv), _ptr(wp[0]), _ptr(wp[1]), _ptr(bias), _ptr(None if rp is not None else residual),
         _ptr(None if rp is None else rp.planes), _ptr(None if rp is None else rp.inv), int(G), int(M), int(N), int(K), int(act), int(rows),
         _ptr(out), _ptr(ws), ws.numel() * ws.element_size(), int(cfg), _stream())
    return out


def winograd_input_transform_h2(x, v, m):
    _chk(x)
    N, H, W, C = x.shape
    assert isinstance(v, H2) and v.K == C and v.rows == winograd_points(m) * winograd_tiles(N, H, W, m)
    if m == 7:
        call("frcnn_winograd7_input_transform_h2", _ptr(x), N, C, _ptr(v.planes), _ptr(v.inv), _stream())
    else:
        call("frcnn_winograd_input_transform_h2", _ptr(x), N, H, W, C, int(m), _ptr(v.planes), _ptr(v.inv), _stream())
    return v


def winograd_output_transform_h2(mm, bias, act, shape, m, out_planes, out=None):
    _chk(mm)
    N, H, W, C = shape
    assert isinstance(out_planes, H2) and out_planes.rows == N * H * W and out_planes.K == C
    assert mm.numel() == winograd_points(m) * winograd_tiles(N, H, W, m) * C
    if out is not None:
        _chk(out)
        assert tuple(out.shape) == tuple(shape)
    if m == 7:
        call("frcnn_winograd7_output_transform_h2", _ptr(mm), N, C, _ptr(bias), int(act), _ptr(out), _ptr(out_planes.planes),
             _ptr(out_planes.inv), _stream())
    else:
        call("frcnn_winograd_output_transform_h2", _ptr(mm), N, H, W, C, int(m), _ptr(bias), int(act), _ptr(out), _ptr(out_planes.planes),
             _ptr(out_planes.inv), _stream())
    return out_planes


def relu6_bwd(grad, y):
    _chk(grad), _chk(y)
    call("frcnn_relu6_bwd", _ptr(grad), _ptr(y), grad.numel(), _stream())
    return grad


def maxpool_bwd(x, y, dy, k, stride, dx):
    _chk(x), _chk(y), _chk(dy), _chk(dx)
    N, H, W, C = x.shape
    call("frcnn_maxpool_bwd", _ptr(x), N, H, W, C, int(k), int(stride), _ptr(y), _ptr(dy), y.shape[1], y.shape[2], _ptr(dx), _stream())
    return dx


def dropout(x, seed, keep_prob, out=None, step_mult=0):
    _chk(x)
    out = _empty(tuple(x.shape), dtype=x.dtype, device=x.device) if out is None else out
    call("frcnn_dropout", _ptr(x), x.numel(), int(seed) & 0xFFFFFFFFFFFFFFFF, float(keep_prob), _ptr(out), _stream())
    if _binding.recorder is not None and step_mult:
        _binding.recorder.patch_last(2, step_mult)
    return out


def dwconv3x3_dgrad(g, w, stride, pad, dx, accumulate=False):
    _chk(g), _chk(w), _chk(dx)
    N, OH, OW, C = g.shape
    call("frcnn_dwconv3x3_dgrad", _ptr(g), N, OH, OW, C, _ptr(w), _ptr(dx), dx.shape[1], dx.shape[2], int(stride), int(pad[0]), int(pad[2]),
         1 if accumulate else 0, _stream())
    return dx


def dwconv3x3_wgrad(g, x, stride, pad, scale, dw):
    _chk(g), _chk(x), _chk(dw)
    N, OH, OW, C = g.shape
    ws = workspace(lib().frcnn_dwconv3x3_wgrad_workspace_bytes(N, OH, OW, C), g.device, "dw_wgrad")
    call("frcnn_dwconv3x3_wgrad", _ptr(g), _ptr(x), N, x.shape[1], x.shape[2], C, OH, OW, int(stride), int(pad[0]), int(pad[2]), _ptr(scale),
         _ptr(dw), _ptr(ws), ws.numel(), _stream())
    return dw


def dwconv3x3_refold(w, scale, wf):
    _chk(w), _chk(scale), _chk(wf)
    call("frcnn_dwconv3x3_refold", _ptr(w), _ptr(scale), w.shape[-1], _ptr(wf), _stream())
    return wf


def add_strided(src, dst, stride, accumulate):
    _chk(src), _chk(dst)
    N, OH, OW, C = src.shape
    call("frcnn_add_strided", _ptr(src), N, OH, OW, C, _ptr(dst), dst.shape[1], dst.shape[2], int(stride), 1 if accumulate else 0, _stream())
    return dst


def spatial_mean_bwd(dy, HW, out):
    _chk(dy), _chk(out)
    call("frcnn_spatial_mean_bwd", _ptr(dy), dy.shape[0], int(HW), dy.shape[1], _ptr(out), _stream())
    return out


def colsum(dy2d, out):
    _chk(dy2d), _chk(out)
    call("frcnn_colsum", _ptr(dy2d), dy2d.shape[0], dy2d.shape[1], _ptr(out), _stream())
    return out


def crop_and_resize_bwd(dout, rois, feat_stride, dfeat, max_lds=0):
    _chk(dout), _chk(rois), _chk(dfeat)
# ... 74 lines not shown
```

### tf-faster-rcnn_amd/lib/model/config.py

```python
import ast
import os
import os.path as osp

import numpy as np


class AttrDict(dict):

    def __init__(self, d=None, **kw):
        super().__init__()
        for k, v in dict(d or {}, **kw).items():
            self[k] = v

    def __setitem__(self, k, v):
        if isinstance(v, dict) and not isinstance(v, AttrDict):
            v = AttrDict(v)
        super().__setitem__(k, v)

    def __getattr__(self, k):
        try:
            return self[k]
        except KeyError:
            raise AttributeError(k)

    __setattr__ = __setitem__


_TRAIN = dict(
    LEARNING_RATE=0.001, MOMENTUM=0.9, WEIGHT_DECAY=0.0001, GAMMA=0.1, STEPSIZE=[30000], DISPLAY=10,
    DOUBLE_BIAS=True, TRUNCATED=False, BIAS_DECAY=False, USE_GT=False, ASPECT_GROUPING=False,
    SNAPSHOT_KEPT=3, SUMMARY_INTERVAL=180, SCALES=(600,), MAX_SIZE=1000, IMS_PER_BATCH=1, BATCH_SIZE=128,
    FG_FRACTION=0.25, FG_THRESH=0.5, BG_THRESH_HI=0.5, BG_THRESH_LO=0.1, USE_FLIPPED=True, BBOX_REG=True,
    BBOX_THRESH=0.5, SNAPSHOT_ITERS=5000, SNAPSHOT_PREFIX='res101_faster_rcnn', BBOX_NORMALIZE_TARGETS=True,
    BBOX_INSIDE_WEIGHTS=(1.0, 1.0, 1.0, 1.0), BBOX_NORMALIZE_TARGETS_PRECOMPUTED=True,
    BBOX_NORMALIZE_MEANS=(0.0, 0.0, 0.0, 0.0), BBOX_NORMALIZE_STDS=(0.1, 0.1, 0.2, 0.2), PROPOSAL_METHOD='gt',
    HAS_RPN=True, RPN_POSITIVE_OVERLAP=0.7, RPN_NEGATIVE_OVERLAP=0.3, RPN_CLOBBER_POSITIVES=False,
    RPN_FG_FRACTION=0.5, RPN_BATCHSIZE=256, RPN_NMS_THRESH=0.7, RPN_PRE_NMS_TOP_N=12000,
    RPN_POST_NMS_TOP_N=2000, RPN_BBOX_INSIDE_WEIGHTS=(1.0, 1.0, 1.0, 1.0), RPN_POSITIVE_WEIGHT=-1.0,
    USE_ALL_GT=True)

_TEST = dict(
    SCALES=(600,), MAX_SIZE=1000, NMS=0.3, SVM=False, BBOX_REG=True, HAS_RPN=False, PROPOSAL_METHOD='gt',
    RPN_NMS_THRESH=0.7, RPN_PRE_NMS_TOP_N=6000, RPN_POST_NMS_TOP_N=300, MODE='nms', RPN_TOP_N=5000)

__C = AttrDict(
    TRAIN=_TRAIN, TEST=_TEST,
    RESNET=dict(MAX_POOL=False, FIXED_BLOCKS=1),
    MOBILENET=dict(REGU_DEPTH=False, FIXED_LAYERS=5, WEIGHT_DECAY=0.00004, DEPTH_MULTIPLIER=1.),
    PIXEL_MEANS=np.array([[[102.9801, 115.9465, 122.7717]]]), RNG_SEED=3,
    ROOT_DIR=osp.abspath(osp.join(osp.dirname(__file__), '..', '..')),
    MATLAB='matlab', EXP_DIR='default', USE_GPU_NMS=True, USE_E2E_TF=False, POOLING_MODE='crop', POOLING_SIZE=7,
    ANCHOR_SCALES=[8, 16, 32], ANCHOR_RATIOS=[0.5, 1, 2], RPN_CHANNELS=512,
    HIP=dict(WINOGRAD=True, WINOGRAD_MIN_CIN=64, WINOGRAD_M=4, WINOGRAD_F2_SCOPES=("block1", "block2"), WINOGRAD_DIRECT_SCOPES=(),
             WINOGRAD_TRAIN=True, WINOGRAD_DGRAD=True,
             WINOGRAD_7X7=True, FUSE_TAIL_MEAN=True, MFMA_X3=True,
             MFMA_H2=True, H2_LAZY_SPLIT=True, H2_MIN_TILES=150, H2_TRAIN_MIN_TILES=320, H2_TRUNK_PLANES=True, H2_TILE_CFG=-1,
             X3_TILE_CFG=-1, H2_TRAIN=True, WGRAD_STREAM=2, WGRAD_TN=True, WGRAD_H2=True, PREP_STREAM=True, TRAIN_REPLAY=True, TRAIN_PICK_STREAMS=6,
             GRAPH_CACHE_SHAPES=4, TRAIN_CACHE_SHAPES=16, JPEG_DEVICE=False, TEST_BATCH_IMAGES=1))
__C.DATA_DIR = osp.abspath(osp.join(__C.ROOT_DIR, 'data'))
cfg = __C


def get_output_dir(imdb, weights_filename):
    outdir = osp.abspath(osp.join(__C.ROOT_DIR, 'output', __C.EXP_DIR, imdb.name))
    outdir = osp.join(outdir, 'default' if weights_filename is None else weights_filename)
    os.makedirs(outdir, exist_ok=True)
    return outdir


def get_output_tb_dir(imdb, weights_filename):
    outdir = osp.abspath(osp.join(__C.ROOT_DIR, 'tensorboard', __C.EXP_DIR, imdb.name))
    outdir = osp.join(outdir, 'default' if weights_filename is None else weights_filename)
    os.makedirs(outdir, exist_ok=True)
    return outdir


_NULLABLE_KEYS = ("H2_TRAIN_MIN_TILES",)


def _merge_a_into_b(a, b):
    if not isinstance(a, dict):
        return
    for k, v in a.items():
        if k not in b:
            raise KeyError('{} is not a valid config key'.format(k))
        old = b[k]
        if type(old) is not type(v) and not (isinstance(old, dict) and isinstance(v, dict)):
            if isinstance(old, np.ndarray):
                v = np.array(v, dtype=old.dtype)
            elif isinstance(old, tuple) and isinstance(v, list):
                v = tuple(v)
            elif isinstance(old, list) and isinstance(v, tuple):
                v = list(v)
            elif k in _NULLABLE_KEYS and (v is None or old is None) and isinstance(old if v is None else v, int):
                pass
            else:
                raise ValueError('Type mismatch ({} vs. {}) for config key: {}'.format(type(old), type(v), k))
        if isinstance(v, dict):
            try:
                _merge_a_into_b(v, b[k])
            except Exception:
                print('Error under config key: {}'.format(k))
                raise
        else:
            b[k] = v


def cfg_from_file(filename):
    import yaml
    with open(filename, 'r') as f:
        _merge_a_into_b(AttrDict(yaml.safe_load(f) or {}), __C)


def cfg_from_list(cfg_list):
    assert len(cfg_list) % 2 == 0
    for k, v in zip(cfg_list[0::2], cfg_list[1::2]):
        path = k.split('.')
        d = __C
        for sub in path[:-1]:
            assert sub in d
            d = d[sub]
        leaf = path[-1]
        assert leaf in d
        try:
            value = ast.literal_eval(v)
        except Exception:
            value = v
        old = d[leaf]
        if isinstance(old, tuple) and isinstance(value, list):
            value = tuple(value)
        if isinstance(old, list) and isinstance(value, tuple):
            value = list(value)
        nullable = leaf in _NULLABLE_KEYS and (value is None or old is None) and isinstance(old if value is None else value, int)
        assert nullable or type(value) == type(old), 'type {} does not match original type {}'.format(type(value), type(old))
        d[leaf] = value
```

### tf-faster-rcnn_amd/lib/nets/network.py

```python
import collections

import numpy as np
import torch

from frcnn_hip import ACT_NONE, ACT_RELU, NMS_RULE_CPU, NMS_RULE_GPU, ops
from frcnn_hip.runtime import VarSpec
from model.config import cfg


class Network(object):
    def __init__(self):
        self._predictions = {}
        self._losses = {}
        self._anchor_targets = {}
        self._proposal_targets = {}
        self._layers = {}
        self._act_summaries = []
        self._variables_to_fix = {}
        self._feat_stride = [16, ]
        self._scope = "network"
        self._sess = None
        self._image = None
        self._im_info = None
        self._var_specs = collections.OrderedDict()
# ... 79 lines not shown
            if residual is not None and residual.data_ptr() in self._f32_missing:
                res = self._h2_of[residual.data_ptr()]
            tcfg = int(cfg.HIP.H2_TILE_CFG)
            sess.mark("conv:h2:" + scope, flops, lambda: ops.gemm_h2(xp, wp, 1, M, Cout, Cin, b, res, act, out=y, out_planes=yp,
                                                                      want_f32=False, cfg=tcfg),
                      nbytes=4 * M * Cin + 4 * w.numel() + (4 * out.numel() if y is not None else 0)
                      + (4 * out.numel() if yp is not None else 0) + (4 * out.numel() if residual is not None else 0))
            self._wrote(out, yp, y is not None)
        elif plain and self._x3_eligible(M, Cout, Cin, 1):
            self._need_f32(x), self._need_f32(residual)
            planes = sess.x3_planes(w)
            xc = int(cfg.HIP.X3_TILE_CFG)
            sess.mark("conv:x3:" + scope, flops, lambda: ops.gemm_x3(x, planes, 1, M, Cout, Cin, b, residual, act, out=out, cfg=xc),
                      nbytes=4 * (x.numel() + out.numel() + (out.numel() if residual is not None else 0)) + 6 * w.numel())
            self._wrote(out)
        else:
            self._need_f32(x), self._need_f32(residual)
            sess.mark("conv:" + scope, flops,
                      lambda: ops.conv2d(x, w, b, k, k, stride, pad, act, residual, res_stride, fold_w, out=out),
                      nbytes=4 * (x.numel() + w.numel() + out.numel() + (out.numel() if residual is not None else 0)))
            self._wrote(out)
        if self._mode == "TRAIN":
            self._tape.append(dict(kind="conv", scope=scope, x=x, y=out, k=k, stride=stride, pad=tuple(pad), act=act,
                                   residual=residual, res_stride=res_stride))
            if self.trainable_scope(scope) or x.data_ptr() in self._requires_grad:
                self._requires_grad.add(out.data_ptr())
            if residual is not None and residual.data_ptr() in self._requires_grad:
                self._requires_grad.add(out.data_ptr())
        return out

    H2_MIN_CHANNEL_RATIO = 2.0 ** -18

    def _h2_eligible(self, M, N, K, G, scope=None):
        rows = G * M
        if scope is not None and self._mode == "TEST" and self._sess.h2_channel_spread(scope) < self.H2_MIN_CHANNEL_RATIO:
            return False
        return (bool(cfg.HIP.MFMA_H2) and (self._mode == "TEST" or bool(cfg.HIP.H2_TRAIN)) and K % 128 == 0 and N % 128 == 0
                and ((self._plan_rows(M) + 127) // 128) * (N // 128) * G >= self._h2_min_tiles()
                and 4 * rows * K < (1 << 32) and 4 * N * K < (1 << 32) and M * N < (1 << 29))

    @staticmethod
    def h2_min_tiles(mode):
        if mode == "TRAIN" and cfg.HIP.H2_TRAIN_MIN_TILES is not None:
            return int(cfg.HIP.H2_TRAIN_MIN_TILES)
        return int(cfg.HIP.H2_MIN_TILES)

    def _h2_min_tiles(self):
        return self.h2_min_tiles(self._mode)

    def _h2_input(self, x):
        xp = self._h2_of.get(x.data_ptr())
        if xp is None and cfg.HIP.H2_LAZY_SPLIT:
            self._need_f32(x)
            K = x.shape[-1]
            xp = self._sess.h2_buf(self._tag + "/split@%x" % x.data_ptr(), x.numel() // K, K)
            self._sess.mark("op:h2_split", 0, lambda: ops.h2_split(x, out=xp), nbytes=8 * x.numel())
            self._h2_of[x.data_ptr()] = xp
        return xp

    def _wrote(self, t, planes=None, f32=True):
        k = t.data_ptr()
        if planes is None:
            self._h2_of.pop(k, None)
        else:
            self._h2_of[k] = planes
        (self._f32_missing.discard if f32 else self._f32_missing.add)(k)
        return t

    def _need_f32(self, x):
        if x is not None and x.data_ptr() in self._f32_missing:
            raise RuntimeError("graph construction error: a float32 consumer reads a tensor that was emitted as operand planes only")

    def _x3_eligible(self, M, N, K, G):
        return (bool(cfg.HIP.MFMA_X3) and self._mode == "TEST" and N % 64 == 0 and K % 32 == 0
                and ((self._plan_rows(M) + 127) // 128) * ((N + 127) // 128) * G >= 150 and M * N < (1 << 31) and N * K < (1 << 28))

    @staticmethod
    def _winograd_scheme(scope, H, W):
        if any(tok in scope for tok in cfg.HIP.WINOGRAD_F2_SCOPES):
            return 2
        m = int(cfg.HIP.WINOGRAD_M)
        return 7 if (m == 4 and H == 7 and W == 7 and cfg.HIP.WINOGRAD_7X7) else m

    def _conv_winograd(self, x, scope, act, bn_eps, emit_h2=False, want_f32=True):
        sess = self._sess
        self._need_f32(x)
        N, H, W, Cin = x.shape
        m = self._winograd_scheme(scope, H, W)
        u, b = sess.winograd_params(scope, bn_eps=bn_eps, m=m)
        G, Cout = u.shape[0], u.shape[1]
        T = ops.winograd_tiles(N, H, W, m)
        mm = sess.buf(self._tag + "/wino_m", (G, T, Cout))
        out = sess.buf(self._tag + "/" + scope, (N, H, W, Cout))
        flops = 2 * G * T * Cout * Cin
        if self._h2_eligible(T, Cout, Cin, G, scope):
            vp, wp = sess.h2_buf(self._tag + "/wino_v", G * T, Cin), sess.h2_planes(u)
            sess.mark("op:wino_in", 0, lambda: ops.winograd_input_transform_h2(x, vp, m), nbytes=4 * (x.numel() + G * T * Cin))
            tcfg = int(cfg.HIP.H2_TILE_CFG)
            sess.mark("conv:h2:" + scope, flops, lambda: ops.gemm_h2(vp, wp, G, T, Cout, Cin, out=mm, cfg=tcfg),
                      nbytes=4 * (G * T * Cin + mm.numel()) + 4 * u.numel())
        else:
            v = sess.buf(self._tag + "/wino_v", (G, T, Cin))
            sess.mark("op:wino_in", 0, lambda: ops.winograd_input_transform(x, v, m), nbytes=4 * (x.numel() + v.numel()))
            if self._x3_eligible(T, Cout, Cin, G):
                planes = sess.x3_planes(u)
                xc = int(cfg.HIP.X3_TILE_CFG)
                sess.mark("conv:x3:" + scope, flops, lambda: ops.gemm_x3(v, planes, G, T, Cout, Cin, out=mm, cfg=xc),
                          nbytes=4 * (v.numel() + mm.numel()) + 6 * u.numel())
            else:
                sess.mark("conv:" + scope, flops, lambda: ops.gemm_batched_nt(v, u, mm), nbytes=4 * (v.numel() + u.numel() + mm.numel()))
        if emit_h2 and cfg.HIP.MFMA_H2 and Cout % 128 == 0:
            yp = sess.h2_buf(self._tag + "/" + scope, N * H * W, Cout)
            y = out if want_f32 else None
            sess.mark("op:wino_out", 0, lambda: ops.winograd_output_transform_h2(mm, b, act, (N, H, W, Cout), m, yp, y),
                      nbytes=4 * (mm.numel() + out.numel() * (2 if want_f32 else 1)))
            self._wrote(out, yp, y is not None)
        else:
            sess.mark("op:wino_out", 0, lambda: ops.winograd_output_transform(mm, b, act, out, m), nbytes=4 * (mm.numel() + out.numel()))
            self._wrote(out)
        return out

    def _conv1x1_mean(self, x, scope, group_rows, act=ACT_RELU, bn_eps=None, residual=None, name="fc7"):
        sess = self._sess
        w, b = sess.conv_params(scope, bn_eps=bn_eps)
        Cin, Cout = x.shape[-1], w.shape[0]
        rows = x.numel() // Cin
        G = max(1, self._plan_batch)
        assert rows % G == 0 and (rows // G) % group_rows == 0
        M = rows // G
        out = sess.buf(self._tag + "/" + name, (rows // group_rows, Cout))
        xp, wp = self._h2_of[x.data_ptr()], sess.h2_planes(w)
        res = residual
        if residual is not None and residual.data_ptr() in self._f32_missing:
            res = self._h2_of[residual.data_ptr()]
        tcfg = int(cfg.HIP.H2_TILE_CFG)
        sess.mark("conv:h2:" + scope, 2 * rows * Cout * Cin, lambda: ops.gemm_h2_mean(xp, wp, G, M, Cout, Cin, b, res, act, group_rows, out=out, cfg=tcfg),
                  nbytes=4 * (rows * Cin + w.numel() + out.numel() + (rows * Cout if residual is not None else 0)))
        return self._wrote(out)

    def _mean_fusable(self, rows, cout, cin, scope, group_rows=1):
        G = max(1, self._plan_batch)
        return (bool(cfg.HIP.FUSE_TAIL_MEAN) and self._mode == "TEST" and rows % G == 0 and (rows // G) % max(1, int(group_rows)) == 0
                and self._h2_eligible(rows, cout, cin, 1, scope)
                and bool(cfg.HIP.H2_LAZY_SPLIT or cfg.HIP.WINOGRAD))

    _rgb_first_conv = None

    def get_variables_to_restore(self, variables, var_keep_dic):
        skip = set(self._variables_to_fix_names())
        self._variables_to_fix = {}
        keep = []
        for name in variables:
            if name in skip:
                self._variables_to_fix[name] = True
                continue
            if name in var_keep_dic:
                keep.append(name)
        return keep

    def _variables_to_fix_names(self):
        return [] if self._rgb_first_conv is None else [self._scope + self._rgb_first_conv + "/weights"]

    def fix_variables(self, sess, pretrained_model):
        from frcnn_hip.tensor_bundle import open_checkpoint
        reader = open_checkpoint(pretrained_model)
        fixed = {}
        for name in self._variables_to_fix_names():
            fixed[name] = self._fix_one(name, reader.get_tensor(name))
        sess.load_variables(fixed)
        sess.conv_info.clear()
        return sorted(fixed)

    def _fix_one(self, name, value):
        return np.ascontiguousarray(value[:, :, ::-1, :])

    def trainable_scope(self, scope):
        return True

    def _reshape_layer(self, bottom, num_dim, name):
        raise NotImplementedError("folded into frcnn_rpn_softmax (network.py:68-78 only served the pair softmax)")

    def _softmax_layer(self, bottom, name):
        if name.startswith("rpn_cls_prob"):
            A = self._num_anchors
# ... 206 lines not shown

    def _build_network(self, is_training=True):
        with self._plan_context(self, is_training):
            return self._build_network_impl(is_training)

    def _build_network_impl(self, is_training=True):
        self._tape = []
        self._requires_grad = set()
        self._h2_of, self._f32_missing = {}, set()
        net_conv = self._image_to_head(is_training)
        self._anchor_component()
        fused = self._fuse_tail_entry and not is_training and hasattr(self, "_fused_tail_entry")
        rois = self._region_proposal(net_conv, is_training)
        if cfg.POOLING_MODE != "crop":
            raise NotImplementedError
        if fused:
            fc7 = self._fused_tail_entry(net_conv, rois)
        else:
            pool5 = self._crop_pool_layer(net_conv, rois, "pool5")
            self._layers["pool5"] = pool5
            fc7 = self._head_to_tail(pool5, is_training)
        self._layers["fc7"] = fc7
        cls_prob, bbox_pred = self._region_classification(fc7, is_training)
        return rois, cls_prob, bbox_pred

    _trainable_on_device = False

    @staticmethod
    def _check_supported_cfg(mode):
        t = cfg.TRAIN
        fixed = [("POOLING_MODE", cfg.POOLING_MODE, "crop")]
        bad = ["%s = %r (only %r is implemented)" % (k, v, want) for k, v, want in fixed if v != want]
        if float(t.RPN_POSITIVE_WEIGHT) >= 0 and not (0.0 < float(t.RPN_POSITIVE_WEIGHT) < 1.0):
            bad.append("TRAIN.RPN_POSITIVE_WEIGHT = %r (the reference asserts 0 < p < 1, anchor_target_layer.py:103-104)" % (t.RPN_POSITIVE_WEIGHT,))
        if bad:
            raise NotImplementedError("unsupported configuration for the HIP path: " + "; ".join(bad))

    def create_architecture(self, mode, num_classes, tag=None, anchor_scales=(8, 16, 32), anchor_ratios=(0.5, 1, 2)):
        assert tag is not None
        self._check_supported_cfg(mode)
        if mode == "TRAIN" and not self._trainable_on_device:
            raise NotImplementedError("%s: no reverse sweep for this network's TRAIN graph; TEST mode works" % type(self).__name__)
        self._tag = tag
        self._num_classes = num_classes
        self._mode = mode
        self._anchor_scales = tuple(anchor_scales)
        self._num_scales = len(anchor_scales)
        self._anchor_ratios = tuple(anchor_ratios)
        self._num_ratios = len(anchor_ratios)
        self._num_anchors = self._num_scales * self._num_ratios
        A = self._num_anchors
        self._var_specs.clear()
        self._declare_backbone()
        hc = self._head_channels()
        self._declare_conv_bias(self._scope + "/rpn_conv/3x3", 3, 3, hc, cfg.RPN_CHANNELS, 0.01)
        self._declare_conv_bias(self._scope + "/rpn_cls_score", 1, 1, cfg.RPN_CHANNELS, 2 * A, 0.01)
        self._declare_conv_bias(self._scope + "/rpn_bbox_pred", 1, 1, cfg.RPN_CHANNELS, 4 * A, 0.01)
        tc = self._tail_channels()
        self._var(self._scope + "/cls_score/weights", (tc, num_classes), "normal", 0.01)
        self._var(self._scope + "/cls_score/biases", (num_classes,), "zeros")
        self._var(self._scope + "/bbox_pred/weights", (tc, 4 * num_classes), "normal", 0.001)
        self._var(self._scope + "/bbox_pred/biases", (4 * num_classes,), "zeros")
        names = ["rois", "rpn_cls_score", "rpn_cls_prob", "rpn_bbox_pred", "cls_score", "cls_prob", "bbox_pred"]
        return {k: k for k in names}

    def _stage_image(self, sess, image, im_info=None):
        if isinstance(image, np.ndarray):
            image = torch.from_numpy(np.ascontiguousarray(image, dtype=np.float32))
        B, H, W, C = image.shape
        if im_info is None:
            buf = sess.buf(self._tag + "/image", (B, H, W, 4), zero=True)
        else:
            with self.shape_scope(sess, (B, H, W, 4), im_info):
                buf = sess.buf(self._tag + "/image", (B, H, W, 4), zero=True)
        buf[..., :C].copy_(image, non_blocking=True)
        return buf

    def graph_key(self, image_shape, im_info):
        c = cfg[self._mode]
        return (self._tag, self._scope, self._num_classes, self._anchor_scales, self._anchor_ratios, bool(cfg.RESNET.MAX_POOL),
                bool(cfg.USE_GPU_NMS), tuple(int(v) for v in image_shape), (float(im_info[0]), float(im_info[1])), self._mode, cfg.TEST.MODE, self._fuse_tail_entry,
                c.RPN_PRE_NMS_TOP_N, c.RPN_POST_NMS_TOP_N, c.RPN_NMS_THRESH, cfg.TEST.RPN_TOP_N, cfg.POOLING_SIZE,
                bool(cfg.HIP.WINOGRAD), int(cfg.HIP.WINOGRAD_MIN_CIN), int(cfg.HIP.WINOGRAD_M), tuple(cfg.HIP.WINOGRAD_F2_SCOPES),
                tuple(cfg.HIP.WINOGRAD_DIRECT_SCOPES), bool(cfg.HIP.WINOGRAD_7X7), bool(cfg.HIP.FUSE_TAIL_MEAN), bool(cfg.HIP.MFMA_X3), bool(cfg.USE_E2E_TF),
                bool(cfg.HIP.MFMA_H2), bool(cfg.HIP.H2_LAZY_SPLIT), int(cfg.HIP.H2_MIN_TILES), bool(cfg.HIP.H2_TRUNK_PLANES), int(cfg.HIP.H2_TILE_CFG), int(cfg.HIP.X3_TILE_CFG), bool(cfg.HIP.H2_TRAIN))

    def shape_scope(self, sess, image_shape, im_info):
        return sess.shape_scope(self.graph_key(image_shape, im_info), group=("graphs", self._tag), cap=int(cfg.HIP.GRAPH_CACHE_SHAPES))

    def forward_device(self, sess, image_d, im_info, use_graph=True):
        self._sess = sess
        self._image = image_d
        self._im_info = (float(im_info[0]), float(im_info[1]), float(im_info[2]))
        sess.prepared.wait_planes()
        ops.ws_scope = self._tag
        key = self.graph_key(image_d.shape, self._im_info)
        cur = torch.cuda.current_stream(sess.device)
        with self.shape_scope(sess, image_d.shape, self._im_info):
            if not use_graph or sess.profile is not None:
                sess.flops_last_forward = 0
                self._build_network(self._mode == "TRAIN")
                return self._predictions
            if key not in sess.graphs:
                with torch.cuda.stream(sess.stream):
                    sess.stream.wait_stream(cur)
                    sess.flops_last_forward = 0
                    self._build_network(False)
                    sess.stream.synchronize()
                    flops = sess.flops_last_forward
                    g = ops.Graph().capture(lambda: self._build_network(False))
                    sess.stream.synchronize()
                sess.graphs[key] = (g, dict(self._predictions), self._num_rois, flops, self._rois_per_image, image_d)
            g, preds, num, flops, per, captured = sess.graphs[key]
            self._predictions, self._num_rois, sess.flops_last_forward, self._rois_per_image = dict(preds), num, flops, per
            if captured.data_ptr() != image_d.data_ptr():
                captured.copy_(image_d, non_blocking=True)
            g.launch()
        return self._predictions

    def extract_head(self, sess, image):
        self._sess = sess
        sess.prepared.wait_planes()
        shape = (int(image.shape[0]), int(image.shape[1]), int(image.shape[2]), 4)
        with sess.shape_scope(("extract_head", self._tag, shape), group=("head", self._tag), cap=int(cfg.HIP.GRAPH_CACHE_SHAPES)):
            self._image = self._stage_image(sess, image)
            self._h2_of, self._f32_missing = {}, set()
            ops.ws_scope = self._tag
            with self._plan_context(self, False):
                feat = self._image_to_head(False)
            return feat.cpu().numpy()

    def test_image(self, sess, image, im_info):
        img = self._stage_image(sess, image, im_info)
        p = self.forward_device(sess, img, im_info)
        assert img.shape[0] == 1, "test_image keeps the reference's single-image contract (network.py:388); use detect_device for batches"
        n = p["rois"].shape[0] if self._num_rois is None else int(self._num_rois.item())
        return (p["cls_score"][:n].cpu().numpy(), p["cls_prob"][:n].cpu().numpy(), p["bbox_pred"][:n].cpu().numpy(),
                p["rois"][:n].cpu().numpy())

    def _stage_train_inputs(self, sess, blobs):
        self._sess = sess
        info = blobs["im_info"]
        self._im_info = (float(info[0]), float(info[1]), float(info[2]))
        if "data" not in blobs:
            im = blobs["image"]
            im_scale, OH, OW = self._train_prep_shape(blobs)
            dev = sess.device
            G = int(blobs["boxes"].shape[0])
            cap = max(self.TRAIN_MAX_GT, (G + 63) // 64 * 64)
            self._image = sess.buf(self._tag + "/image", (1, OH, OW, 4), zero=True)
            buf = sess.buf(self._tag + "/gt_boxes", (cap, 5), zero=True)
            im_d = (im if torch.is_tensor(im) else torch.from_numpy(np.ascontiguousarray(im))).to(dev, non_blocking=True)
            boxes_d = torch.from_numpy(np.ascontiguousarray(blobs["boxes"], dtype=np.uint16)).to(dev, non_blocking=True) if G else None
            classes_d = torch.from_numpy(np.ascontiguousarray(blobs["gt_classes"], dtype=np.int32)).to(dev, non_blocking=True) if G else None
            ops.prep_train_image(im_d, bool(blobs["flipped"]), cfg.PIXEL_MEANS, im_scale, (OH, OW), out=self._image, out_c=4,
                                 boxes=boxes_d, classes=classes_d, gt_out=buf)
            self._gt_boxes = buf[:G]
            return
        self._image = self._stage_image(sess, blobs["data"])
        gt = blobs["gt_boxes"]
        gt = gt if torch.is_tensor(gt) else torch.from_numpy(np.ascontiguousarray(gt, dtype=np.float32))
        G = int(gt.shape[0])
        cap = max(self.TRAIN_MAX_GT, (G + 63) // 64 * 64)
        buf = sess.buf(self._tag + "/gt_boxes", (cap, 5), zero=True)
        buf[:G].copy_(gt, non_blocking=True)
        self._gt_boxes = buf[:G]

# ... 190 lines not shown
```

### tf-faster-rcnn_amd/lib/nets/resnet_v1.py

```python
from frcnn_hip import ACT_NONE, ACT_RELU, ops
from model.config import cfg
from nets.network import Network

BN_EPS = 1e-5


def _same_pad(k, stride):
    total = k - 1
    beg = total // 2
    return (beg, total - beg, beg, total - beg)


class resnetv1(Network):
    _rgb_first_conv = "/conv1"
    _trainable_on_device = True
    def __init__(self, num_layers=50):
        Network.__init__(self)
        self._feat_stride = [16, ]
        self._feat_compress = [1. / float(self._feat_stride[0]), ]
        self._num_layers = num_layers
        self._scope = 'resnet_v1_%d' % num_layers
        self._decide_blocks()

    def _decide_blocks(self):
# ... 22 lines not shown
    def _head_channels(self):
        return self._blocks[2][1] * 4

    def _tail_channels(self):
        return self._blocks[3][1] * 4

    def _bottleneck(self, x, prefix, base, stride, mean_rows=0, emit_out=True, f32_out=True):
        depth = base * 4
        cin = x.shape[-1]
        if cin != depth:
            shortcut = self._conv(x, prefix + "/shortcut", 1, stride, act=ACT_NONE, bn_eps=BN_EPS)
            res_stride = 1
        else:
            shortcut, res_stride = x, stride
        r = self._conv(x, prefix + "/conv1", 1, 1, act=ACT_RELU, bn_eps=BN_EPS)
        pad = (1, 1, 1, 1) if stride == 1 else _same_pad(3, stride)
        N, H, W, _ = r.shape
        M3 = N * ops.conv_out_size(H, 3, stride, pad[0], pad[1]) * ops.conv_out_size(W, 3, stride, pad[2], pad[3])
        if mean_rows and res_stride == 1 and stride == 1 and self._mean_fusable(M3, depth, base, prefix + "/conv3", mean_rows):
            r = self._conv(r, prefix + "/conv2", 3, stride, pad, act=ACT_RELU, bn_eps=BN_EPS, emit_h2=True, want_f32=False)
            if self._h2_input(r) is not None:
                return self._conv1x1_mean(r, prefix + "/conv3", mean_rows, act=ACT_RELU, bn_eps=BN_EPS, residual=shortcut)
            x = self._conv(r, prefix + "/conv3", 1, 1, act=ACT_RELU, bn_eps=BN_EPS, residual=shortcut, res_stride=1)
            out = self._sess.buf(self._tag + "/fc7", (x.shape[0], x.shape[-1]))
            return self._sess.mark("op:spatial_mean", 0, lambda: ops.spatial_mean(x, out=out), nbytes=4 * (x.numel() + out.numel()))
        c3_h2 = res_stride == 1 and self._h2_eligible(M3, depth, base, 1, prefix + "/conv3")
        r = self._conv(r, prefix + "/conv2", 3, stride, pad, act=ACT_RELU, bn_eps=BN_EPS, emit_h2=c3_h2, want_f32=not c3_h2)
        return self._conv(r, prefix + "/conv3", 1, 1, act=ACT_RELU, bn_eps=BN_EPS, residual=shortcut, res_stride=res_stride,
                          emit_h2=emit_out, want_f32=f32_out)

    def _trunk_planes_only(self, rows, base, next_stride, next_prefix=None):
        depth = 4 * base
        return (bool(cfg.HIP.H2_TRUNK_PLANES) and next_stride == 1
                and self._h2_eligible(rows, base, depth, 1, None if next_prefix is None else next_prefix + "/conv1")
                and self._h2_eligible(rows, depth, base, 1, None if next_prefix is None else next_prefix + "/conv3"))

    def _run_blocks(self, x, blocks, emit_last=True):
        for bi, (name, base, n_units, stride) in enumerate(blocks):
            for u in range(1, n_units + 1):
                s_u = stride if u == n_units else 1
                N, H, W, _ = x.shape
                rows = N * ops.conv_out_size(H, 3, s_u, 1, 1) * ops.conv_out_size(W, 3, s_u, 1, 1) if s_u > 1 else N * H * W
                planes_only = u < n_units and self._trunk_planes_only(rows, base, stride if u + 1 == n_units else 1,
                                                                       "%s/%s/unit_%d/bottleneck_v1" % (self._scope, name, u + 1))
                x = self._bottleneck(x, "%s/%s/unit_%d/bottleneck_v1" % (self._scope, name, u), base, s_u,
                                     emit_out=emit_last or u < n_units or bi + 1 < len(blocks), f32_out=not planes_only)
        return x

    def _crop_pool_layer(self, bottom, rois, name):
        return self._crop_pool(bottom, rois, name, max_pool=bool(cfg.RESNET.MAX_POOL))

    def _build_base(self):
        net = self._conv(self._image, self._scope + "/conv1", 7, 2, _same_pad(7, 2), act=ACT_RELU, bn_eps=BN_EPS,
                         fold_w=True, real_cin=3)
        N, H, W, C = net.shape
        out = self._sess.buf(self._tag + "/pool1", (N, ops.conv_out_size(H, 3, 2, 1, 1), ops.conv_out_size(W, 3, 2, 1, 1), C))
        self._sess.mark("op:maxpool", 0, lambda: ops.maxpool(net, 3, 2, (1, 1, 1, 1), out=out), nbytes=4 * (net.numel() + out.numel()))
        return self._wrote(out)

    def _image_to_head(self, is_training, reuse=None):
        assert (0 <= cfg.RESNET.FIXED_BLOCKS <= 3)
        net_conv = self._run_blocks(self._build_base(), self._blocks[0:3])
        self._act_summaries.append(net_conv)
        self._layers['head'] = net_conv
        return net_conv

    def _fused_tail_maps(self, net_conv):
        name = self._blocks[-1][0]
        prefix = "%s/%s/unit_1/bottleneck_v1" % (self._scope, name)
        sc_map = self._conv(net_conv, prefix + "/shortcut", 1, 1, act=ACT_NONE, bn_eps=BN_EPS, no_bias=True)
        c1_map = self._conv(net_conv, prefix + "/conv1", 1, 1, act=ACT_NONE, bn_eps=BN_EPS, no_bias=True)
        return sc_map, c1_map

    def _fused_tail_entry(self, net_conv, rois):
        sess, P = self._sess, cfg.POOLING_SIZE
        name, base, n_units, stride = self._blocks[-1]
        prefix = "%s/%s/unit_1/bottleneck_v1" % (self._scope, name)
        R = rois.shape[0]
        sc_map, c1_map = self._fused_tail_maps(net_conv)
        b_sc = sess.conv_info[prefix + "/shortcut"]["b"]
        b_c1 = sess.conv_info[prefix + "/conv1"]["b"]
        fs = float(self._feat_stride[0])
        sc_out = sess.buf(self._tag + "/" + prefix + "/shortcut_crop", (R, P, P, sc_map.shape[-1]))
        c1_out = sess.buf(self._tag + "/" + prefix + "/conv1_crop", (R, P, P, c1_map.shape[-1]))
        shortcut = self._crop_images(sc_map, rois, sc_out, bias=b_sc, act=ACT_NONE)
        r = self._crop_images(c1_map, rois, c1_out, bias=b_c1, act=ACT_RELU)
        c3_h2 = self._h2_eligible(R * P * P, 4 * base, base, 1, prefix + "/conv3")
        r = self._conv(r, prefix + "/conv2", 3, 1, (1, 1, 1, 1), act=ACT_RELU, bn_eps=BN_EPS, emit_h2=c3_h2, want_f32=not c3_h2)
        x = self._conv(r, prefix + "/conv3", 1, 1, act=ACT_RELU, bn_eps=BN_EPS, residual=shortcut, res_stride=1, emit_h2=n_units >= 2,
                       want_f32=not (n_units >= 2 and self._trunk_planes_only(R * P * P, base, stride if n_units == 2 else 1,
                                                                              "%s/%s/unit_2/bottleneck_v1" % (self._scope, name))))
        fused = stride == 1 and n_units >= 2 and self._mean_fusable(R * P * P, 4 * base, base, "%s/%s/unit_%d/bottleneck_v1/conv3" % (self._scope, name, n_units), P * P)
        for u in range(2, n_units + 1):
            x = self._bottleneck(x, "%s/%s/unit_%d/bottleneck_v1" % (self._scope, name, u), base, stride if u == n_units else 1,
                                 mean_rows=P * P if (fused and u == n_units) else 0, emit_out=u < n_units,
                                 f32_out=not (u < n_units and self._trunk_planes_only(R * P * P, base, stride if u + 1 == n_units else 1,
                                                                                      "%s/%s/unit_%d/bottleneck_v1" % (self._scope, name, u + 1))))
        if fused:
            return x
        out = sess.buf(self._tag + "/fc7", (x.shape[0], x.shape[-1]))
        return sess.mark("op:spatial_mean", 0, lambda: ops.spatial_mean(x, out=out), nbytes=4 * (x.numel() + out.numel()))

    def _head_to_tail(self, pool5, is_training, reuse=None):
        name, base, n_units, stride = self._blocks[-1]
        if stride == 1 and self._mean_fusable(pool5.shape[0] * pool5.shape[1] * pool5.shape[2], 4 * base, base,
                                              "%s/%s/unit_%d/bottleneck_v1/conv3" % (self._scope, name, n_units), pool5.shape[1] * pool5.shape[2]):
            x = pool5
            hw = pool5.shape[1] * pool5.shape[2]
            for u in range(1, n_units + 1):
                x = self._bottleneck(x, "%s/%s/unit_%d/bottleneck_v1" % (self._scope, name, u), base, 1, mean_rows=hw if u == n_units else 0)
            return x
        fc7 = self._run_blocks(pool5, self._blocks[-1:], emit_last=False)
        out = self._sess.buf(self._tag + "/fc7", (fc7.shape[0], fc7.shape[-1]))
        res = self._sess.mark("op:spatial_mean", 0, lambda: ops.spatial_mean(fc7, out=out), nbytes=4 * (fc7.numel() + out.numel()))
        if self._mode == "TRAIN":
            self._tape.append(dict(kind="mean", x=fc7, y=res, name=self._scope + "/fc7_mean"))
            if fc7.data_ptr() in self._requires_grad:
                self._requires_grad.add(res.data_ptr())
        return res

    def trainable_scope(self, scope):
        fixed = ["/conv1"] + ["/block%d/" % b for b in range(1, cfg.RESNET.FIXED_BLOCKS + 1)]
        tail = scope[len(self._scope):]
        return not any(tail.startswith(f) for f in fixed)
```

Baseline: 546.7.

## Fuse ROI crop-and-resize into Winograd 7x7 input transform for tail conv2

Adds a kernel that samples the ROI crop (bilinear, bias, ReLU) straight from the conv1 feature map inside the Winograd F(7) input transform. The tail entry uses it when the route is eligible, so the intermediate R×7×7×C crop buffer is never written and read back. Separately, it gives the Winograd output transform its own row-kernel threshold and restricts the dual-epilogue GEMM config to K<=256. The fused kernel recomputes bilinear samples per tile and may have a different memory-access pattern, and the threshold changes could shift kernel selection for other shapes.

```diff
diff --git a/include/frcnn_hip.h b/include/frcnn_hip.h
--- a/include/frcnn_hip.h
+++ b/include/frcnn_hip.h
@@ -167,6 +167,9 @@
 int frcnn_winograd_output_transform_h2(const float* m_d, int N, int H, int W, int C, int m, const float* bias_d, int act, float* y_d,
                                        void* y_planes_d, float* y_inv_d, void* stream);
 int frcnn_winograd7_input_transform_h2(const float* x_d, int R, int C, void* v_planes_d, float* v_inv_d, void* stream);
+int frcnn_winograd7_input_transform_crop_h2(const float* feat_d, int NIMG, int H, int W, int C, const float* rois_d, int R,
+                                            float feat_stride, const float* bias_d, int act, void* v_planes_d, float* v_inv_d,
+                                            void* stream);
 int frcnn_winograd7_output_transform_h2(const float* m_d, int R, int C, const float* bias_d, int act, float* y_d, void* y_planes_d,
                                         float* y_inv_d, void* stream);
 int frcnn_pack_filter_hwio(const float* w_hwio, int KH, int KW, int Cin, int Cout, const float* scale, float* out);
diff --git a/scratch/tail_entry_bench.py b/scratch/tail_entry_bench.py
--- /dev/null
+++ b/scratch/tail_entry_bench.py
@@ -0,0 +1,54 @@
+import os, sys
+ROOT = os.path.abspath(sys.argv[1]) if len(sys.argv) > 1 else os.path.dirname(os.path.dirname(os.path.abspath(__file__)))
+sys.path[:0] = [os.path.join(ROOT, "tf-faster-rcnn_amd")]
+import numpy as np, torch
+import frcnn_hip
+from frcnn_hip import ops
+print("library:", frcnn_hip.LIB_PATH, flush=True)
+dev = torch.device("cuda:0")
+NIMG, H, W, C, PER = 8, 38, 63, 512, 300
+R = NIMG * PER
+torch.manual_seed(0)
+feat = torch.randn(NIMG, H, W, C, device=dev)
+bias = torch.randn(C, device=dev)
+rng = np.random.RandomState(0)
+rois = np.zeros((R, 5), np.float32)
+for i in range(NIMG):
+    cx, cy = rng.rand(PER) * 1000, rng.rand(PER) * 600
+    w, h = np.exp(rng.uniform(np.log(32), np.log(700), PER)), np.exp(rng.uniform(np.log(32), np.log(500), PER))
+    b = np.stack([cx - w / 2, cy - h / 2, cx + w / 2, cy + h / 2], 1)
+    b[:, 0::2] = b[:, 0::2].clip(0, 999); b[:, 1::2] = b[:, 1::2].clip(0, 599)
+    rois[i * PER:(i + 1) * PER, 0] = i; rois[i * PER:(i + 1) * PER, 1:] = b
+rois = torch.from_numpy(rois).to(dev)
+crop = torch.empty(R, 7, 7, C, device=dev)
+v1, v2 = ops.H2.empty(121 * R, C, dev), ops.H2.empty(121 * R, C, dev)
+for v in (v1, v2):
+    v.planes.zero_(); v.inv.zero_()
+has_fused = hasattr(ops, "winograd7_input_transform_crop_h2")
+
+def t_crop(): ops.crop_and_resize_bias_act(feat, rois, 16.0, 7, bias, 1, out=crop)
+def t_tr(): ops.winograd_input_transform_h2(crop, v1, 7)
+def t_pair(): t_crop(); t_tr()
+def t_fused(): ops.winograd7_input_transform_crop_h2(feat, rois, 16.0, bias, 1, v2)
+
+def bench(fn, groups=25, per=10):
+    for _ in range(5): fn()
+    torch.cuda.synchronize()
+    ts = []
+    for g in range(groups):
+        e0, e1 = torch.cuda.Event(enable_timing=True), torch.cuda.Event(enable_timing=True)
+        e0.record()
+        for _ in range(per): fn()
+        e1.record(); torch.cuda.synchronize()
+        ts.append(e0.elapsed_time(e1) * 1000.0 / per)
+    return float(np.median(ts)), min(ts), max(ts)
+
+rows = [("crop (bias, ReLU)", t_crop), ("k_wino7_input<true>", t_tr), ("crop + transform", t_pair)]
+if has_fused:
+    rows.append(("fused transform", t_fused))
+for rep in range(2):
+    for name, fn in rows:
+        print("round %d  %-22s median %7.1f us  min %7.1f  max %7.1f   (%d groups of %d launches)" % ((rep, name) + bench(fn) + (25, 10)), flush=True)
+if has_fused:
+    t_pair(); t_fused(); torch.cuda.synchronize()
+    print("bits: planes %s, scales %s" % (torch.equal(v1.planes, v2.planes), torch.equal(v1.inv.view(torch.int32), v2.inv.view(torch.int32))))
diff --git a/scratch/wino_bench.py b/scratch/wino_bench.py
--- a/scratch/wino_bench.py
+++ b/scratch/wino_bench.py
@@ -10,6 +10,8 @@
     "block3 conv2 x8": (8, 38, 63, 256, 4),
     "block3 conv2 x1": (1, 38, 63, 256, 4),
     "rpn 3x3 x8": (8, 38, 63, 1024, 4),
+    "rpn 3x3 x4": (4, 38, 63, 1024, 4),
+    "block3 conv2 x4 800x1333": (4, 50, 84, 256, 4),
     "block2 conv2 x8 (F2)": (8, 75, 125, 128, 2),
     "tail conv2 7x7 x8": (2400, 7, 7, 512, 7),
 }
diff --git a/tf-faster-rcnn_amd/csrc/conv_igemm.hip b/tf-faster-rcnn_amd/csrc/conv_igemm.hip
--- a/tf-faster-rcnn_amd/csrc/conv_igemm.hip
+++ b/tf-faster-rcnn_amd/csrc/conv_igemm.hip
@@ -554,9 +554,10 @@
 static thread_local int g_force_cfg = -1, g_stagger = 0, g_stream = 1, g_split_target = 640;
 static thread_local int g_plan_images = 0;
 static constexpr int PLAN_IMAGES = 4;
-extern thread_local int g_wino_rows_below;
+extern thread_local int g_wino_rows_below, g_wino_out_rows_below;
 extern "C" int frcnn_set_tuning(int key, int value) {
-  if (key == 9) { g_wino_rows_below = value > 0 ? value : 256; return FRCNN_OK; }
+  if (key == 9) { g_wino_rows_below = value > 0 ? value : 256; g_wino_out_rows_below = value > 0 ? value : 512; return FRCNN_OK; }
+  if (key == 10) { g_wino_out_rows_below = value > 0 ? value : 512; return FRCNN_OK; }
   if (key == 0) { g_force_cfg = value; return FRCNN_OK; }
   if (key == 5) { g_stagger = value; return FRCNN_OK; }
   if (key == 6) { g_stream = value; return FRCNN_OK; }
diff --git a/tf-faster-rcnn_amd/csrc/crop_sample.h b/tf-faster-rcnn_amd/csrc/crop_sample.h
--- /dev/null
+++ b/tf-faster-rcnn_amd/csrc/crop_sample.h
@@ -0,0 +1,77 @@
+#pragma once
+#include "common.h"
+
+__device__ __forceinline__ float4 crop_zero(const float4*) { return make_float4(0, 0, 0, 0); }
+__device__ __forceinline__ float2 crop_zero(const float2*) { return make_float2(0, 0); }
+__device__ __forceinline__ float4 crop_lerp(const float4 a, const float4 b, float t) {
+  return make_float4(a.x + (b.x - a.x) * t, a.y + (b.y - a.y) * t, a.z + (b.z - a.z) * t, a.w + (b.w - a.w) * t);
+}
+__device__ __forceinline__ float2 crop_lerp(const float2 a, const float2 b, float t) {
+  return make_float2(a.x + (b.x - a.x) * t, a.y + (b.y - a.y) * t);
+}
+
+__device__ __forceinline__ int crop_roi_image(const float* __restrict__ roi) { return (int)roi[0]; }
+struct CropGeom {
+  float x1, y1, hs, ws;
+};
+__device__ __forceinline__ CropGeom crop_geom(const float* __restrict__ roi, int H, int W, float stride, int P) {
+  const float height = ((float)H - 1.0f) * stride, width = ((float)W - 1.0f) * stride;
+  const float x1 = roi[1] / width, y1 = roi[2] / height, x2 = roi[3] / width, y2 = roi[4] / height;
+  CropGeom g;
+  g.x1 = x1; g.y1 = y1;
+  g.hs = (y2 - y1) * (float)(H - 1) / (float)(P - 1);
+  g.ws = (x2 - x1) * (float)(W - 1) / (float)(P - 1);
+  return g;
+}
+
+struct CropPos {
+  float in_y, in_x;
+  bool inside;
+};
+__device__ __forceinline__ CropPos crop_pos(int H, int W, float y1, float x1, float hs, float ws, int gy, int gx) {
+  CropPos p;
+  p.in_y = y1 * (float)(H - 1) + (float)gy * hs;
+  p.in_x = x1 * (float)(W - 1) + (float)gx * ws;
+  p.inside = !(p.in_y < 0 || p.in_y > (float)(H - 1) || p.in_x < 0 || p.in_x > (float)(W - 1));
+  return p;
+}
+struct CropTaps {
+  int top, bot, left, right;
+  float ly, lx;
+};
+__device__ __forceinline__ CropTaps crop_taps(const CropPos p) {
+  CropTaps t;
+  t.top = (int)floorf(p.in_y), t.bot = (int)ceilf(p.in_y);
+  t.left = (int)floorf(p.in_x), t.right = (int)ceilf(p.in_x);
+  t.ly = p.in_y - (float)t.top, t.lx = p.in_x - (float)t.left;
+  return t;
+}
+template <typename V>
+__device__ __forceinline__ V crop_blend(const V tl, const V tr, const V bl, const V br, float lx, float ly) {
+  return crop_lerp(crop_lerp(tl, tr, lx), crop_lerp(bl, br, lx), ly);
+}
+
+template <typename V>
+__device__ __forceinline__ V crop_sample(const V* __restrict__ feat, int H, int W, int CV, int c, float y1, float x1, float hs, float ws,
+                                         int gy, int gx) {
+  const CropPos p = crop_pos(H, W, y1, x1, hs, ws, gy, gx);
+  if (!p.inside) return crop_zero(feat);
+  const CropTaps t = crop_taps(p);
+  const V tl = feat[((size_t)t.top * W + t.left) * CV + c], tr = feat[((size_t)t.top * W + t.right) * CV + c];
+  const V bl = feat[((size_t)t.bot * W + t.left) * CV + c], br = feat[((size_t)t.bot * W + t.right) * CV + c];
+  return crop_blend(tl, tr, bl, br, t.lx, t.ly);
+}
+
+__device__ __forceinline__ float4 crop_bias_act(float4 v, const float4* __restrict__ bias, int c, int act) {
+  if (bias) {
+    const float4 bv = bias[c];
+    v.x += bv.x; v.y += bv.y; v.z += bv.z; v.w += bv.w;
+  }
+  if (act == FRCNN_ACT_RELU) v = act_relu(v);
+  return v;
+}
+__device__ __forceinline__ float2 crop_bias_act(float2 v, bool has_bias, const float2 bv, int act) {
+  if (has_bias) { v.x += bv.x; v.y += bv.y; }
+  if (act == FRCNN_ACT_RELU) v = act_relu(v);
+  return v;
+}
diff --git a/tf-faster-rcnn_amd/csrc/detect_kernels.hip b/tf-faster-rcnn_amd/csrc/detect_kernels.hip
--- a/tf-faster-rcnn_amd/csrc/detect_kernels.hip
+++ b/tf-faster-rcnn_amd/csrc/detect_kernels.hip
@@ -1,4 +1,5 @@
 #include "common.h"
+#include "crop_sample.h"
 
 extern "C" int frcnn_generate_anchors(int base_size, const double* ratios, int n_ratios, const double* scales,
                                       int n_scales, double* out_base) {
@@ -817,24 +818,8 @@
                                          nms_thresh, rois_d, scores_d, num_d, ws, ws_bytes, stream);
 }
 
-__device__ __forceinline__ float4 lerp4(const float4 a, const float4 b, float t) {
-  return make_float4(a.x + (b.x - a.x) * t, a.y + (b.y - a.y) * t, a.z + (b.z - a.z) * t, a.w + (b.w - a.w) * t);
-}
 __device__ __forceinline__ float4 max4(const float4 a, const float4 b) {
   return make_float4(fmaxf(a.x, b.x), fmaxf(a.y, b.y), fmaxf(a.z, b.z), fmaxf(a.w, b.w));
-}
-
-__device__ __forceinline__ float4 crop_sample(const float4* __restrict__ feat, int H, int W, int C4, int c4, float y1,
-                                              float x1, float hs, float ws, int gy, int gx) {
-  const float in_y = y1 * (float)(H - 1) + (float)gy * hs;
-  const float in_x = x1 * (float)(W - 1) + (float)gx * ws;
-  if (in_y < 0 || in_y > (float)(H - 1) || in_x < 0 || in_x > (float)(W - 1)) return make_float4(0, 0, 0, 0);
-  const int top = (int)floorf(in_y), bot = (int)ceilf(in_y);
-  const int left = (int)floorf(in_x), right = (int)ceilf(in_x);
-  const float ly = in_y - (float)top, lx = in_x - (float)left;
-  const float4 tl = feat[((size_t)top * W + left) * C4 + c4], tr = feat[((size_t)top * W + right) * C4 + c4];
-  const float4 bl = feat[((size_t)bot * W + left) * C4 + c4], br = feat[((size_t)bot * W + right) * C4 + c4];
-  return lerp4(lerp4(tl, tr, lx), lerp4(bl, br, lx), ly);
 }
 
 template <bool MAX2>
@@ -844,19 +829,16 @@
   const int slab = blockIdx.x % nslab, rp = blockIdx.x / nslab;
   const int r = rp / pool, py = rp % pool;
   const int SC4 = C4 / nslab, c40 = slab * SC4;
-  const float height = ((float)H - 1.0f) * stride, width = ((float)W - 1.0f) * stride;
   const float* roi = rois + 5 * (size_t)r;
-  const int img = (int)roi[0];
+  const int img = crop_roi_image(roi);
   float4* orow = out + ((size_t)r * pool + py) * pool * C4;
   if (img < 0 || img >= NIMG) {
     for (int t = threadIdx.x; t < pool * SC4; t += 256) orow[(size_t)(t / SC4) * C4 + c40 + t % SC4] = make_float4(0, 0, 0, 0);
     return;
   }
   const float4* feat = feat_all + (size_t)img * H * W * C4;
-  const float x1 = roi[1] / width, y1 = roi[2] / height, x2 = roi[3] / width, y2 = roi[4] / height;
-  const int P = MAX2 ? 2 * pool : pool;
-  const float hs = (y2 - y1) * (float)(H - 1) / (float)(P - 1);
-  const float ws = (x2 - x1) * (float)(W - 1) / (float)(P - 1);
+  const CropGeom g = crop_geom(roi, H, W, stride, MAX2 ? 2 * pool : pool);
+  const float x1 = g.x1, y1 = g.y1, hs = g.hs, ws = g.ws;
   for (int t = threadIdx.x; t < pool * SC4; t += 256) {
     const int px = t / SC4, c4 = c40 + t % SC4;
     float4 v;
@@ -868,11 +850,7 @@
     } else {
       v = crop_sample(feat, H, W, C4, c4, y1, x1, hs, ws, py, px);
     }
-    if (bias) {
-      const float4 bv = bias[c4];
-      v.x += bv.x; v.y += bv.y; v.z += bv.z; v.w += bv.w;
-    }
-    if (act == FRCNN_ACT_RELU) v = act_relu(v);
+    v = crop_bias_act(v, bias, c4, act);
     orow[(size_t)px * C4 + c4] = v;
   }
 }
@@ -883,9 +861,8 @@
                                                              const float4* __restrict__ bias, int act, float4* __restrict__ out) {
   const int slab = blockIdx.x % nslab, r = blockIdx.x / nslab;
   const int SC4 = C4 / nslab, c40 = slab * SC4;
-  const float height = ((float)H - 1.0f) * stride, width = ((float)W - 1.0f) * stride;
   const float* roi = rois + 5 * (size_t)r;
-  const int img = (int)roi[0];
+  const int img = crop_roi_image(roi);
   float4* obase = out + (size_t)r * pool * pool * C4;
   const int total = pool * pool * SC4;
   if (img < 0 || img >= NIMG) {
@@ -893,10 +870,8 @@
     return;
   }
   const float4* feat = feat_all + (size_t)img * H * W * C4;
-  const float x1 = roi[1] / width, y1 = roi[2] / height, x2 = roi[3] / width, y2 = roi[4] / height;
-  const int P = MAX2 ? 2 * pool : pool;
-  const float hs = (y2 - y1) * (float)(H - 1) / (float)(P - 1);
-  const float ws = (x2 - x1) * (float)(W - 1) / (float)(P - 1);
+  const CropGeom g = crop_geom(roi, H, W, stride, MAX2 ? 2 * pool : pool);
+  const float x1 = g.x1, y1 = g.y1, hs = g.hs, ws = g.ws;
   for (int t0 = threadIdx.x; t0 < total; t0 += 256 * ITEMS) {
     float4 v[ITEMS];
 #pragma unroll
@@ -919,13 +894,7 @@
       const int t = t0 + k * 256;
       if (t >= total) continue;
       const int pix = t / SC4, c4 = c40 + t % SC4;
-      float4 o = v[k];
-      if (bias) {
-        const float4 bv = bias[c4];
-        o.x += bv.x; o.y += bv.y; o.z += bv.z; o.w += bv.w;
-      }
-      if (act == FRCNN_ACT_RELU) o = act_relu(o);
-      obase[(size_t)pix * C4 + c4] = o;
+      obase[(size_t)pix * C4 + c4] = crop_bias_act(v[k], bias, c4, act);
     }
   }
 }
diff --git a/tf-faster-rcnn_amd/csrc/gemm_h2.hip b/tf-faster-rcnn_amd/csrc/gemm_h2.hip
--- a/tf-faster-rcnn_amd/csrc/gemm_h2.hip
+++ b/tf-faster-rcnn_amd/csrc/gemm_h2.hip
@@ -1134,7 +1134,7 @@
     const int pp_cfg = (cfg == -3 || cfg == -4 || (cfg == -6 && K < FRCNN_H2_PP_MIN_K)) ? 34 : 21;
     const bool pp = K >= pp_min_k && mt256 * 256 * 100 <= (long long)M * 104 && mt256 * (N / 128) * G >= 256;
     const bool tiny = (long long)((M + 127) / 128) * (N / 128) * G < 150;
-    const bool de = cfg != -2 && cfg != -7 && !p.mean_part && !p.mask && ((p.resp && p.yp && !p.y) || cfg == -8);
+    const bool de = cfg != -2 && cfg != -7 && !p.mean_part && !p.mask && ((p.resp && p.yp && !p.y && K <= 256) || cfg == -8);
     cfg = pp ? pp_cfg : tiny ? (cfg == -2 ? 12 : (de && cfg == -8) ? 41 : 33) : (cfg == -2 ? 9 : de ? 40 : 31);
   }
   if (p.mean_part && (cfg == 40 || cfg == 41)) cfg = cfg == 40 ? 31 : 33;
diff --git a/tf-faster-rcnn_amd/csrc/winograd.hip b/tf-faster-rcnn_amd/csrc/winograd.hip
--- a/tf-faster-rcnn_amd/csrc/winograd.hip
+++ b/tf-faster-rcnn_amd/csrc/winograd.hip
@@ -302,7 +302,9 @@
 }
 
 thread_local int g_wino_rows_below = 256;
+thread_local int g_wino_out_rows_below = 512;
 #define WINO_ROWS_BELOW g_wino_rows_below
+#define WINO_OUT_ROWS_BELOW g_wino_out_rows_below
 
 template <bool H2>
 static int wino_input_launch(const float* x_d, int N, int H, int W, int C, int m, const WinoSink<H2>& sink, hipStream_t st) {
@@ -380,7 +382,7 @@
                               hipStream_t st, const float* mask_d = nullptr) {
   const int TH = (H + m - 1) / m, TW = (W + m - 1) / m;
   const long long tot = (long long)N * TH * TW * (C / 4);
-  const bool rows = (tot + 255) / 256 < WINO_ROWS_BELOW;
+  const bool rows = (tot + 255) / 256 < WINO_OUT_ROWS_BELOW;
   if (m == 4 && mask_d && rows)
     hipLaunchKernelGGL((k_wino4_output_rows<H2, true>), dim3((unsigned)((tot * 4 + 255) / 256)), dim3(256), 0, st, (const float4*)m_d, N, H, W,
                        C / 4, TH, TW, (const float4*)bias_d, act, (const float4*)mask_d, sink);
diff --git a/tf-faster-rcnn_amd/csrc/winograd7.hip b/tf-faster-rcnn_amd/csrc/winograd7.hip
--- a/tf-faster-rcnn_amd/csrc/winograd7.hip
+++ b/tf-faster-rcnn_amd/csrc/winograd7.hip
@@ -1,4 +1,5 @@
 #include "h2_common.h"
+#include "crop_sample.h"
 
 namespace w7 {
 constexpr float BT[11][9] = {
@@ -91,6 +92,79 @@
   }
 }
 
+template <bool H2>
+__device__ __forceinline__ void wino7_input_points(const float2 (&d)[7][7], int r, int R, int c2, int C2, const Wino7Sink<H2>& V) {
+#pragma unroll
+  for (int xi = 0; xi < 11; ++xi) {
+    float2 t[7];
+#pragma unroll
+    for (int j = 0; j < 7; ++j) {
+      bool first = true;
+      t[j] = make_float2(0.f, 0.f);
+#pragma unroll
+      for (int i = 0; i < 7; ++i) acc_term(t[j], first, w7::BT[xi][i + 1], d[i][j]);
+    }
+    float2 o[11];
+    size_t rw[11];
+#pragma unroll
+    for (int nu = 0; nu < 11; ++nu) {
+      bool first = true;
+      float2 v = make_float2(0.f, 0.f);
+#pragma unroll
+      for (int j = 0; j < 7; ++j) acc_term(v, first, w7::BT[nu][j + 1], t[j]);
+      o[nu] = v;
+      rw[nu] = (size_t)(xi * 11 + nu) * R + r;
+    }
+    V.template putn<11>(rw, o, c2, C2);
+  }
+}
+
+__global__ void __launch_bounds__(256) k_wino7_input_crop(const float2* __restrict__ feat_all, int NIMG, int H, int W, int C2,
+                                                          const float* __restrict__ rois, int R, float stride, const float2* __restrict__ bias,
+                                                          int act, const Wino7Sink<true> V) {
+  const int nblk = C2 >> 6;
+  const int r = __builtin_amdgcn_readfirstlane((int)(blockIdx.x / nblk) * 4 + (int)(threadIdx.x >> 6));
+  if (r >= R) return;
+  const int c2 = (int)(blockIdx.x % nblk) * 64 + (int)(threadIdx.x & 63);
+  const float* roi = rois + 5 * (size_t)r;
+  const int img = crop_roi_image(roi);
+  float2 d[7][7];
+  if (img < 0 || img >= NIMG) {
+#pragma unroll
+    for (int i = 0; i < 7; ++i)
+#pragma unroll
+      for (int j = 0; j < 7; ++j) d[i][j] = make_float2(0.f, 0.f);
+  } else {
+    const float2* feat = feat_all + (size_t)img * H * W * C2 + c2;
+    const CropGeom g = crop_geom(roi, H, W, stride, 7);
+    const bool has_bias = bias != nullptr;
+    const float2 bv = has_bias ? bias[c2] : make_float2(0.f, 0.f);
+#pragma unroll
+    for (int i = 0; i < 7; ++i) {
+      bool inside[7];
+      float ly[7], lx[7];
+      float2 tl[7], tr[7], bl[7], br[7];
+#pragma unroll
+      for (int j = 0; j < 7; ++j) {
+        const CropPos p = crop_pos(H, W, g.y1, g.x1, g.hs, g.ws, i, j);
+        const CropTaps t = crop_taps(p);
+        inside[j] = p.inside, ly[j] = t.ly, lx[j] = t.lx;
+        const int top = p.inside ? t.top : 0, bot = p.inside ? t.bot : 0, left = p.inside ? t.left : 0, right = p.inside ? t.right : 0;
+        tl[j] = feat[((size_t)top * W + left) * C2], tr[j] = feat[((size_t)top * W + right) * C2];
+        bl[j] = feat[((size_t)bot * W + left) * C2], br[j] = feat[((size_t)bot * W + right) * C2];
+      }
+#pragma unroll
+      for (int j = 0; j < 7; ++j) {
+        const float2 smp = crop_blend(tl[j], tr[j], bl[j], br[j], lx[j], ly[j]);
+        d[i][j] = crop_bias_act(inside[j] ? smp : crop_zero(feat), has_bias, bv, act);
+      }
+#pragma unroll
+      for (int j = 0; j < 7; ++j) asm volatile("" : "+v"(d[i][j].x), "+v"(d[i][j].y));
+    }
+  }
+  wino7_input_points<true>(d, r, R, c2, C2, V);
+}
+
 template <int XI0, int NXI, int I0, int NI, bool H2, bool MASK>
 __device__ __forceinline__ void wino7_out_segment(const float2* __restrict__ in, size_t plane, float2 bv, int act, const Wino7Sink<H2>& y,
                                                   size_t row0, int c2, int C2, const float2* __restrict__ mask) {
@@ -219,6 +293,21 @@
   return FRCNN_OK;
 }
 
+extern "C" int frcnn_winograd7_input_transform_crop_h2(const float* feat_d, int NIMG, int H, int W, int C, const float* rois_d, int R,
+                                                       float feat_stride, const float* bias_d, int act, void* v_planes_d, float* v_inv_d,
+                                                       void* stream) {
+  if (!feat_d || !rois_d || !v_planes_d || !v_inv_d || NIMG <= 0 || H < 2 || W < 2 || C <= 0 || R <= 0) return FRCNN_E_ARG;
+  if (act != FRCNN_ACT_NONE && act != FRCNN_ACT_RELU) return FRCNN_E_ARG;
+  if (C % H2_KB) return FRCNN_E_UNSUPPORTED;
+  const long long blocks = (long long)((R + 3) / 4) * (C / H2_KB);
+  if (blocks >= (1ll << 31)) return FRCNN_E_UNSUPPORTED;
+  const Wino7Sink<true> sink{nullptr, (unsigned short*)v_planes_d, v_inv_d, (size_t)121 * R};
+  hipLaunchKernelGGL(k_wino7_input_crop, dim3((unsigned)blocks), dim3(256), 0, (hipStream_t)stream, (const float2*)feat_d, NIMG, H, W, C / 2, rois_d,
+                     R, feat_stride, (const float2*)bias_d, act, sink);
+  LAUNCH_CHECK();
+  return FRCNN_OK;
+}
+
 extern "C" int frcnn_winograd7_output_transform(const float* m_d, int R, int C, const float* bias_d, int act, float* y_d, void* stream) {
   if (!m_d || !y_d || R <= 0 || C <= 0) return FRCNN_E_ARG;
   if (C % 2 || (act != FRCNN_ACT_NONE && act != FRCNN_ACT_RELU)) return FRCNN_E_UNSUPPORTED;
diff --git a/tf-faster-rcnn_amd/frcnn_hip/__init__.py b/tf-faster-rcnn_amd/frcnn_hip/__init__.py
--- a/tf-faster-rcnn_amd/frcnn_hip/__init__.py
+++ b/tf-faster-rcnn_amd/frcnn_hip/__init__.py
@@ -87,6 +87,7 @@
     "frcnn_winograd_input_transform_h2": (c_int, [_P, c_int, c_int, c_int, c_int, c_int, _P, _P, _P]),
     "frcnn_winograd_output_transform_h2": (c_int, [_P, c_int, c_int, c_int, c_int, c_int, _P, c_int, _P, _P, _P, _P]),
     "frcnn_winograd7_input_transform_h2": (c_int, [_P, c_int, c_int, _P, _P, _P]),
+    "frcnn_winograd7_input_transform_crop_h2": (c_int, [_P, c_int, c_int, c_int, c_int, _P, c_int, c_float, _P, c_int, _P, _P, _P]),
     "frcnn_winograd7_output_transform_h2": (c_int, [_P, c_int, c_int, _P, c_int, _P, _P, _P, _P]),
     "frcnn_set_tuning": (c_int, [c_int, c_int]),
     "frcnn_pack_filter_hwio": (c_int, [_P, c_int, c_int, c_int, c_int, _P, _P]),
diff --git a/tf-faster-rcnn_amd/frcnn_hip/ops.py b/tf-faster-rcnn_amd/frcnn_hip/ops.py
--- a/tf-faster-rcnn_amd/frcnn_hip/ops.py
+++ b/tf-faster-rcnn_amd/frcnn_hip/ops.py
@@ -1003,6 +1003,16 @@
     return v
 
 
+def winograd7_input_transform_crop_h2(feat, rois, feat_stride, bias, act, v):
+    _chk(feat), _chk(rois)
+    N, H, W, C = feat.shape
+    R = rois.shape[0]
+    assert isinstance(v, H2) and v.K == C and v.rows == winograd_points(7) * R and rois.shape[1] == 5
+    call("frcnn_winograd7_input_transform_crop_h2", _ptr(feat), N, H, W, C, _ptr(rois), R, float(feat_stride), _ptr(bias), int(act),
+         _ptr(v.planes), _ptr(v.inv), _stream())
+    return v
+
+
 def winograd_output_transform_h2(mm, bias, act, shape, m, out_planes, out=None):
     _chk(mm)
     N, H, W, C = shape
diff --git a/tf-faster-rcnn_amd/lib/model/config.py b/tf-faster-rcnn_amd/lib/model/config.py
--- a/tf-faster-rcnn_amd/lib/model/config.py
+++ b/tf-faster-rcnn_amd/lib/model/config.py
@@ -53,7 +53,7 @@
     ANCHOR_SCALES=[8, 16, 32], ANCHOR_RATIOS=[0.5, 1, 2], RPN_CHANNELS=512,
     HIP=dict(WINOGRAD=True, WINOGRAD_MIN_CIN=64, WINOGRAD_M=4, WINOGRAD_F2_SCOPES=("block1", "block2"), WINOGRAD_DIRECT_SCOPES=(),
              WINOGRAD_TRAIN=True, WINOGRAD_DGRAD=True,
-             WINOGRAD_7X7=True, FUSE_TAIL_MEAN=True, MFMA_X3=True,
+             WINOGRAD_7X7=True, FUSE_TAIL_MEAN=True, FUSE_TAIL_CROP=True, MFMA_X3=True,
              MFMA_H2=True, H2_LAZY_SPLIT=True, H2_MIN_TILES=150, H2_TRAIN_MIN_TILES=320, H2_TRUNK_PLANES=True, H2_TILE_CFG=-1,
              X3_TILE_CFG=-1, H2_TRAIN=True, WGRAD_STREAM=2, WGRAD_TN=True, WGRAD_H2=True, PREP_STREAM=True, TRAIN_REPLAY=True, TRAIN_PICK_STREAMS=6,
              GRAPH_CACHE_SHAPES=4, TRAIN_CACHE_SHAPES=16, JPEG_DEVICE=False, TEST_BATCH_IMAGES=1))
diff --git a/tf-faster-rcnn_amd/lib/nets/network.py b/tf-faster-rcnn_amd/lib/nets/network.py
--- a/tf-faster-rcnn_amd/lib/nets/network.py
+++ b/tf-faster-rcnn_amd/lib/nets/network.py
@@ -185,10 +185,21 @@
         m = int(cfg.HIP.WINOGRAD_M)
         return 7 if (m == 4 and H == 7 and W == 7 and cfg.HIP.WINOGRAD_7X7) else m
 
-    def _conv_winograd(self, x, scope, act, bn_eps, emit_h2=False, want_f32=True):
+    def _wino7_h2_route(self, shape, scope, k=3, stride=1, pad=(1, 1, 1, 1), act=ACT_RELU):
+        N, H, W, Cin = shape
+        wino = (cfg.HIP.WINOGRAD and self._mode == "TEST" and k == 3 and stride == 1 and tuple(pad) == (1, 1, 1, 1)
+                and Cin % 32 == 0 and Cin >= cfg.HIP.WINOGRAD_MIN_CIN and act in (ACT_NONE, ACT_RELU)
+                and not any(tok in scope for tok in cfg.HIP.WINOGRAD_DIRECT_SCOPES))
+        if not wino or self._winograd_scheme(scope, H, W) != 7:
+            return False
+        Cout = self._var_specs[scope + "/weights"].shape[3]
+        return self._h2_eligible(ops.winograd_tiles(N, H, W, 7), Cout, Cin, ops.winograd_points(7), scope)
+
+    def _conv_winograd(self, x, scope, act, bn_eps, emit_h2=False, want_f32=True, crop_of=None):
         sess = self._sess
-        self._need_f32(x)
-        N, H, W, Cin = x.shape
+        self._need_f32(x if crop_of is None else crop_of[0])
+        N, H, W, Cin = x.shape if crop_of is None else crop_of[4]
+        x_numel = N * H * W * Cin
         m = self._winograd_scheme(scope, H, W)
         u, b = sess.winograd_params(scope, bn_eps=bn_eps, m=m)
         G, Cout = u.shape[0], u.shape[1]
@@ -198,11 +209,19 @@
         flops = 2 * G * T * Cout * Cin
         if self._h2_eligible(T, Cout, Cin, G, scope):
             vp, wp = sess.h2_buf(self._tag + "/wino_v", G * T, Cin), sess.h2_planes(u)
-            sess.mark("op:wino_in", 0, lambda: ops.winograd_input_transform_h2(x, vp, m), nbytes=4 * (x.numel() + G * T * Cin))
+            if crop_of is None:
+                sess.mark("op:wino_in", 0, lambda: ops.winograd_input_transform_h2(x, vp, m), nbytes=4 * (x_numel + G * T * Cin))
+            else:
+                feat, rois, c_bias, c_act = crop_of[:4]
+                assert m == 7 and T == rois.shape[0]
+                fs = float(self._feat_stride[0])
+                sess.mark("op:wino_in", 0, lambda: ops.winograd7_input_transform_crop_h2(feat, rois, fs, c_bias, c_act, vp),
+                          nbytes=4 * (feat.numel() + G * T * Cin))
             tcfg = int(cfg.HIP.H2_TILE_CFG)
             sess.mark("conv:h2:" + scope, flops, lambda: ops.gemm_h2(vp, wp, G, T, Cout, Cin, out=mm, cfg=tcfg),
                       nbytes=4 * (G * T * Cin + mm.numel()) + 4 * u.numel())
         else:
+            assert crop_of is None
             v = sess.buf(self._tag + "/wino_v", (G, T, Cin))
             sess.mark("op:wino_in", 0, lambda: ops.winograd_input_transform(x, v, m), nbytes=4 * (x.numel() + v.numel()))
             if self._x3_eligible(T, Cout, Cin, G):
@@ -575,7 +594,7 @@
                 bool(cfg.USE_GPU_NMS), tuple(int(v) for v in image_shape), (float(im_info[0]), float(im_info[1])), self._mode, cfg.TEST.MODE, self._fuse_tail_entry,
                 c.RPN_PRE_NMS_TOP_N, c.RPN_POST_NMS_TOP_N, c.RPN_NMS_THRESH, cfg.TEST.RPN_TOP_N, cfg.POOLING_SIZE,
                 bool(cfg.HIP.WINOGRAD), int(cfg.HIP.WINOGRAD_MIN_CIN), int(cfg.HIP.WINOGRAD_M), tuple(cfg.HIP.WINOGRAD_F2_SCOPES),
-                tuple(cfg.HIP.WINOGRAD_DIRECT_SCOPES), bool(cfg.HIP.WINOGRAD_7X7), bool(cfg.HIP.FUSE_TAIL_MEAN), bool(cfg.HIP.MFMA_X3), bool(cfg.USE_E2E_TF),
+                tuple(cfg.HIP.WINOGRAD_DIRECT_SCOPES), bool(cfg.HIP.WINOGRAD_7X7), bool(cfg.HIP.FUSE_TAIL_MEAN), bool(cfg.HIP.FUSE_TAIL_CROP), bool(cfg.HIP.MFMA_X3), bool(cfg.USE_E2E_TF),
                 bool(cfg.HIP.MFMA_H2), bool(cfg.HIP.H2_LAZY_SPLIT), int(cfg.HIP.H2_MIN_TILES), bool(cfg.HIP.H2_TRUNK_PLANES), int(cfg.HIP.H2_TILE_CFG), int(cfg.HIP.X3_TILE_CFG), bool(cfg.HIP.H2_TRAIN))
 
     def shape_scope(self, sess, image_shape, im_info):
diff --git a/tf-faster-rcnn_amd/lib/nets/resnet_v1.py b/tf-faster-rcnn_amd/lib/nets/resnet_v1.py
--- a/tf-faster-rcnn_amd/lib/nets/resnet_v1.py
+++ b/tf-faster-rcnn_amd/lib/nets/resnet_v1.py
@@ -128,11 +128,16 @@
         b_c1 = sess.conv_info[prefix + "/conv1"]["b"]
         fs = float(self._feat_stride[0])
         sc_out = sess.buf(self._tag + "/" + prefix + "/shortcut_crop", (R, P, P, sc_map.shape[-1]))
-        c1_out = sess.buf(self._tag + "/" + prefix + "/conv1_crop", (R, P, P, c1_map.shape[-1]))
         shortcut = self._crop_images(sc_map, rois, sc_out, bias=b_sc, act=ACT_NONE)
-        r = self._crop_images(c1_map, rois, c1_out, bias=b_c1, act=ACT_RELU)
         c3_h2 = self._h2_eligible(R * P * P, 4 * base, base, 1, prefix + "/conv3")
-        r = self._conv(r, prefix + "/conv2", 3, 1, (1, 1, 1, 1), act=ACT_RELU, bn_eps=BN_EPS, emit_h2=c3_h2, want_f32=not c3_h2)
+        c1_shape = (R, P, P, c1_map.shape[-1])
+        if cfg.HIP.FUSE_TAIL_CROP and cfg.HIP.H2_LAZY_SPLIT and self._wino7_h2_route(c1_shape, prefix + "/conv2"):
+            r = self._conv_winograd(None, prefix + "/conv2", ACT_RELU, BN_EPS, emit_h2=c3_h2, want_f32=not c3_h2,
+                                    crop_of=(c1_map, rois, b_c1, ACT_RELU, c1_shape))
+        else:
+            c1_out = sess.buf(self._tag + "/" + prefix + "/conv1_crop", c1_shape)
+            r = self._crop_images(c1_map, rois, c1_out, bias=b_c1, act=ACT_RELU)
+            r = self._conv(r, prefix + "/conv2", 3, 1, (1, 1, 1, 1), act=ACT_RELU, bn_eps=BN_EPS, emit_h2=c3_h2, want_f32=not c3_h2)
         x = self._conv(r, prefix + "/conv3", 1, 1, act=ACT_RELU, bn_eps=BN_EPS, residual=shortcut, res_stride=1, emit_h2=n_units >= 2,
                        want_f32=not (n_units >= 2 and self._trunk_planes_only(R * P * P, base, stride if n_units == 2 else 1,
                                                                               "%s/%s/unit_2/bottleneck_v1" % (self._scope, name))))
```

Result: no change. 549.1, median of 6 (+0.4%).
